# vpariza/open-hummingbird-eval

Hardware: AMD Instinct MI355X
Metric: query-patches/sec (higher is better)
Workload: dtype f32

## Files before the change

### include/hbird_hip.h

```cpp
#ifndef HBIRD_HIP_H
#define HBIRD_HIP_H
#include <stdint.h>
#ifdef __cplusplus
extern "C" {
#endif

typedef struct hb_index hb_index_t;

#define HB_METRIC_IP 0
#define HB_METRIC_L2 1
#define HB_MAX_K 2048
#define HB_MAX_K_AGGREGATE 256
#define HB_BIGK_MAX_PARTS 64

const char* hb_last_error(void);
int hb_device_count(int* n);

int hb_index_create(int d, int metric, int device, hb_index_t** out);
int hb_index_free(hb_index_t* ix);
int hb_index_set_stream(hb_index_t* ix, void* hip_stream);
int hb_index_reserve(hb_index_t* ix, int64_t n_rows);
int hb_index_add(hb_index_t* ix, const float* x, int64_t n, int x_on_device, int normalize);
int hb_index_add_labels(hb_index_t* ix, const float* labels, int64_t n, int c, int on_device);
int hb_index_set_label_denominator(hb_index_t* ix, int P);
// ... 36 lines not shown
int hb_bigk_aggregate(hb_index_t* ix, const float* q, int64_t nq, const int64_t* idx, const float* dist, int k,
                      int64_t id_base, float beta, float* out_label_hat, int io_on_device);
int hb_bigk_aggregate_partial(hb_index_t* ix, const float* q, int64_t nq, const int64_t* idx, const float* dist, int k,
                              int64_t id_base, float beta, const float* norms_all, int64_t n_all, float* out_partial);
int hb_bigk_merge_topk(const float* dist_parts, const int64_t* idx_parts, int parts, int64_t nq, int k, int metric,
                       int64_t* out_idx, float* out_dist, void* hip_stream);
int hb_bigk_merge_topk_packed(const void* packed_parts, int64_t part_bytes, int parts, int64_t nq, int k, int metric,
                              int64_t* out_idx, float* out_dist, void* hip_stream);

typedef struct hb_multi hb_multi_t;
int hb_multi_create(int d, int metric, const int* gpu_ids, int n_gpus, int shard, hb_multi_t** out);
int hb_multi_free(hb_multi_t* m);
int hb_multi_reserve(hb_multi_t* m, int64_t n_rows);
int hb_multi_add(hb_multi_t* m, const float* x, int64_t n, int normalize);
int64_t hb_multi_ntotal(const hb_multi_t* m);
int hb_multi_shard_rows(const hb_multi_t* m, int64_t* rows, int n);
int hb_multi_set_fp16(hb_multi_t* m, int enable);
int hb_multi_search(hb_multi_t* m, const float* q, int64_t nq, int k, int64_t* out_idx, float* out_dist);

int hb_normalize_rows(const float* x, int64_t n, int d, float* out, void* hip_stream);
int hb_patch_label_hist(const int64_t* y, int64_t B, int H, int W, int ps, int C, int map255, float* out,
                        void* hip_stream);
int hb_patch_scores(const float* label, int64_t B, int SS, int C, float* scores, int* nonempty, int* nz_count,
                    void* hip_stream);
int hb_patch_select(const float* scores, const int* nonempty, const float* r, const int64_t* r_off, int64_t B,
                    int SS, int K, int64_t* out_idx, float* out_scores, void* hip_stream);
int hb_gather_rows(const float* src, int64_t src_rows, int width, const int64_t* ids, int64_t n, float* out,
                   void* hip_stream);

int hb_upsample_argmax(const float* label_hat, int64_t B, int S, int C, int h, int w, int64_t* out,
                       void* hip_stream);
int hb_upsample_argmax_confusion(const float* label_hat, int64_t B, int S, int C, int h, int w, const int64_t* gt, int num_gt,
                                 int num_pred, int64_t ignore_index, int has_ignore, uint64_t* conf, int64_t* out_map_opt,
                                 void* hip_stream);
int hb_upsample_accumulate(const float* label_hat, int64_t B, int S, int C, int win_h, int win_w, float* acc, int H,
                           int W, int y0, int x0, void* hip_stream);
int hb_argmax_channels(const float* acc, int64_t n, int C, int64_t* out, void* hip_stream);
int hb_confusion_update(const int64_t* gt, const int64_t* pred, int64_t n, int num_gt, int num_pred,
                        int64_t ignore_index, int has_ignore, uint64_t* conf, void* hip_stream);

int hb_index_set_timing(hb_index_t* ix, int enable);
int hb_index_last_knn_ms(const hb_index_t* ix, double* ms);
int hb_index_set_tuning(hb_index_t* ix, int workgroups, int panel_tiles);
#define HB_FP16_AUTO 3
#define HB_PATH_FP32 0
#define HB_PATH_FP16_CHAIN 1
#define HB_PATH_FP16_WIDE 2
#define HB_WHY_EXPLICIT_FP32 0
#define HB_WHY_EXPLICIT_FP16 1
#define HB_WHY_AUTO 2
#define HB_WHY_K 3
#define HB_WHY_CEILING 4
#define HB_WHY_WORK 5
#define HB_WHY_SMALL 6
#define HB_WHY_PINNED 7
#define HB_WHY_ENV 8
#define HB_WHY_MEMORY 9
#define HB_WHY_OVERFLOW 10
#define HB_WHY_ADAPTIVE 11
int hb_index_set_fp16(hb_index_t* ix, int enable);
int hb_last_search_path(const hb_index_t* ix, int* path, int* reason);
int hb_exact_screen_replay(int setting, int pinned, int env_off, int k, int ceiling, int64_t rows, int64_t nq, int d, int64_t stages_per_wg,
                           int overflow, int have_copy, int declined, uint64_t free_bytes, uint64_t total_bytes, uint64_t bank_bytes,
                           uint64_t copy_bytes, int* why);
int hb_knn_plan_replay(const int64_t* in, int n_in, int64_t* out, int n_out);
int hb_index_last_fp16_fallbacks(const hb_index_t* ix, int64_t* n);
int hb_index_set_fp16_escalation(hb_index_t* ix, int mode);
int hb_index_last_fp16_escalated(const hb_index_t* ix, int64_t* n);
int hb_index_set_variant(hb_index_t* ix, int variant);
int hb_index_set_search_options(hb_index_t* ix, int phases, int64_t small_limit_stages);
int hb_index_set_xcd_weights(hb_index_t* ix, int mode, const double* w8);
int hb_index_xcd_weights(const hb_index_t* ix, int fp16_kernel, double* w8, int* rounds);
int hb_schedule_plan_weighted(int nqt, int nbt, int workgroups, int panel_tiles, int d, int cluster_q, int cluster_b, int shared,
                              const double* xcd_w8, int* segs_out, int64_t max_segs, int64_t stats[8]);
int hb_index_wg_stamps(hb_index_t* ix, uint32_t* out, int max_blocks, int* workgroups);
int hb_index_kernel_clock(hb_index_t* ix, double out[4]);
int hb_index_xcd_stats(const hb_index_t* ix, int fp16_kernel, double out[12]);
void* hb_calibration_new(int fp16_kernel);
void hb_calibration_free(void* h);
int hb_calibration_state(const void* h, double shares8[8], int64_t out[12]);
int hb_calibration_feed(void* h, const uint32_t* stamps, int G, const double run_shares8[8], const int key6[6], int auto_cluster, double frac);
int hb_f16_adapt_replay(int n, const double* f1, const double* f2, int64_t nq, int* out_how);
int hb_set_layout_form(int form);
int hb_index_set_rerank_copy(hb_index_t* ix, int mode);
int hb_index_rerank_copy_bytes(const hb_index_t* ix, int64_t* bytes);
int hb_index_schedule_info(const hb_index_t* ix, int64_t out[8]);
int hb_index_set_cluster(hb_index_t* ix, int cluster_q, int cluster_b, int sync_lag);
int hb_index_set_cluster_sharing(hb_index_t* ix, int mode);
int hb_index_cluster_stats(hb_index_t* ix, int64_t out[4]);

int hb_schedule_plan(int nqt, int nbt, int workgroups, int panel_tiles, int d, int cluster_q, int cluster_b, int* segs_out,
                     int64_t max_segs, int64_t stats[8]);
int hb_schedule_plan_phased(int nqt, int nbt, int workgroups, int panel_tiles, int d, int cluster_q, int cluster_b, int* segs_out,
                            int64_t max_segs, int64_t stats[8], int* clocks_out, int max_cuts, int* n_cuts, int* bounds_out);

int hb_schedule_plan_shared(int nqt, int nbt, int workgroups, int panel_tiles, int d, int cluster_q, int cluster_b, int phased,
                            int* segs_out, int64_t max_segs, int64_t stats[8]);

#include "hbird_hip_centre.h"
#include "hbird_hip_select.h"
#include "hbird_hip_grid.h"

#ifdef __cplusplus
}
#endif
#endif
```

### open-hummingbird-eval_amd/csrc/hbird_capi.hip

```cpp
#include "../../include/hbird_hip.h"
#include "hbird_internal.h"
#include <algorithm>
#include <cmath>
#include <cstdlib>
#include <cstring>
#include <dlfcn.h>
#include <mutex>
#include <set>
#include <utility>

static thread_local std::string g_err;
void hb_set_error(const std::string& msg) { g_err = msg; }
int hb_fail(const std::string& msg) { g_err = msg; return -1; }

namespace {
struct roctx_api {
    int (*push)(const char*) = nullptr;
    int (*pop)() = nullptr;
    roctx_api() {
        for (const char* lib : {"librocprofiler-sdk-roctx.so", "librocprofiler-sdk-roctx.so.1", "libroctx64.so", "libroctx64.so.4"}) {
            void* h = dlopen(lib, RTLD_LAZY | RTLD_GLOBAL);
            if (!h) continue;
            push = reinterpret_cast<int (*)(const char*)>(dlsym(h, "roctxRangePushA"));
            pop = reinterpret_cast<int (*)()>(dlsym(h, "roctxRangePop"));
// ... 116 lines not shown
    if (ix->f16_flag) HB_HIP(hipMemsetAsync(ix->f16_flag, 0, 4, ix->stream));
    hb_centre_drop(ix);
    ix->fp16_centre = on; ix->last_centred = 0;
    ix->f16_adapt = hb_f16_adapt();
    return 0;
}
extern "C" int hb_index_fp16_centre_info(const hb_index_t* ix, double out[8]) {
    if (!ix || !out) return hb_fail("hb_index_fp16_centre_info: NULL pointer");
    for (int i = 0; i < 8; ++i) out[i] = 0.0;
    const hb_centre_state& c = ix->centre;
    HB_HIP(hipSetDevice(ix->device));
    float sc[4] = {0, 0, 0, 0}, bmax = 0.0f;
    HB_HIP(hipStreamSynchronize(ix->stream));
    HB_HIP(hipMemcpy(&bmax, ix->bmax, 4, hipMemcpyDeviceToHost));
    const bool active = ix->fp16_centre && c.active && ix->tiles16 && c.sc;
    if (active) HB_HIP(hipMemcpy(sc, c.sc, 16, hipMemcpyDeviceToHost));
    out[0] = active ? 1.0 : 0.0; out[1] = sc[1]; out[2] = sc[0]; out[3] = bmax; out[4] = sc[3]; out[5] = active ? (double)c.rows : 0.0;
    out[6] = ix->fp16_centre; out[7] = ix->last_centred;
    return 0;
}
extern "C" int hb_last_search_path(const hb_index_t* ix, int* path, int* reason) {
    if (!ix || !path || !reason) return hb_fail("hb_last_search_path: NULL pointer");
    *path = ix->last_path; *reason = ix->last_reason;
    return 0;
}

extern "C" int hb_index_set_fp16_escalation(hb_index_t* ix, int mode) {
    if (!ix) return hb_fail("hb_index_set_fp16_escalation: NULL index handle");
    if (mode < 0 || mode > 1) return hb_fail("hb_index_set_fp16_escalation: mode must be 0 (second fp16 pass before the fp32 kernel) or 1 (straight to the fp32 kernel)");
    ix->fp16_escalation = mode;
    return 0;
}
extern "C" int hb_index_last_fp16_escalated(const hb_index_t* ix, int64_t* n) {
    if (!ix || !n) return hb_fail("hb_index_last_fp16_escalated: NULL pointer");
    *n = ix->last_fp16_escalated;
    return 0;
}
extern "C" int hb_index_last_fp16_fallbacks(const hb_index_t* ix, int64_t* n) {
    if (!ix || !n) return hb_fail("hb_index_last_fp16_fallbacks: NULL pointer");
    *n = ix->last_fp16_fallbacks;
    return 0;
}


extern "C" int hb_index_set_cluster_sharing(hb_index_t* ix, int mode) {
    if (!ix) return hb_fail("hb_index_set_cluster_sharing: NULL index handle");
    if (mode < 0 || mode > 2) return hb_fail("hb_index_set_cluster_sharing: mode must be 0 (automatic), 1 (off) or 2 (on)");
    ix->xcd_share = mode; ix->sched = hb_schedule(); ix->fp32_pinned = 1;
    return 0;
}

extern "C" int hb_index_cluster_stats(hb_index_t* ix, int64_t out[4]) {
    if (!ix || !out) return hb_fail("hb_index_cluster_stats: NULL pointer");
    out[0] = out[1] = out[2] = out[3] = 0;
    if (!ix->cl_stats_dev) return 0;
    HB_HIP(hipSetDevice(ix->device));
    int h[4] = {0, 0, 0, 0};
    HB_HIP(hipMemcpyAsync(h, ix->cl_stats_dev, sizeof(h), hipMemcpyDeviceToHost, ix->stream));
    HB_HIP(hipStreamSynchronize(ix->stream));
    out[0] = h[0]; out[1] = h[1]; out[2] = h[2]; out[3] = h[3];
    return 0;
}

extern "C" int hb_index_set_cluster(hb_index_t* ix, int cluster_q, int cluster_b, int sync_lag) {
    if (!ix) return hb_fail("hb_index_set_cluster: NULL index handle");
    if (cluster_q < 0 || cluster_b < 0 || cluster_q * cluster_b > HB_CLUSTER_MAX)
        return hb_fail("hb_index_set_cluster: cluster shape must be 0 x 0 (automatic), 1 x 1 (off) or q x b with q * b <= " + std::to_string(HB_CLUSTER_MAX));
    ix->force_cq = cluster_q; ix->force_cb = cluster_b; ix->sync_lag = sync_lag; ix->sched = hb_schedule();
    if (cluster_q != 0 || cluster_b != 0) ix->fp32_pinned = 1;
    return 0;
}

extern "C" int hb_index_set_variant(hb_index_t* ix, int variant) {
    if (!ix) return hb_fail("hb_index_set_variant: NULL index handle");
    if (variant < 0 || variant > 6) return hb_fail("hb_index_set_variant: unknown kernel variant");
    if (variant == 1 || variant == 2 || variant == 5)
        return hb_fail("hb_index_set_variant: variants 1 (4-wave fp32 kernel), 2 (first fp16 design) and 5 (16x16x32 fp16 kernel) were removed in round 4 (same bits, not faster)");
    ix->variant = variant; ix->fp32_pinned = 1;
    return 0;
}
extern "C" int hb_index_set_search_options(hb_index_t* ix, int phases, int64_t small_limit_stages) {
    if (!ix) return hb_fail("hb_index_set_search_options: NULL index handle");
    if (small_limit_stages < 0) return hb_fail("hb_index_set_search_options: negative limit");
    ix->phases_on = phases ? 1 : 0; ix->small_limit = small_limit_stages; ix->sched = hb_schedule(); ix->fp32_pinned = 1;
    return 0;
}
extern "C" int hb_index_set_xcd_weights(hb_index_t* ix, int mode, const double* w8) {
    if (!ix) return hb_fail("hb_index_set_xcd_weights: NULL index handle");
    if (mode < 0 || mode > 2) return hb_fail("hb_index_set_xcd_weights: mode must be 0 (calibrated), 1 (equal shares) or 2 (the given shares)");
    if (mode == 2 && !w8) return hb_fail("hb_index_set_xcd_weights: mode 2 needs eight shares");
    for (int x = 0; x < 8; ++x) {
        const double w = mode == 2 ? w8[x] : 1.0;
        if (!(w > 0.25 && w < 4.0)) return hb_fail("hb_index_set_xcd_weights: every share must lie in (0.25, 4)");
        ix->xcal[0].w[x] = w; ix->xcal[1].w[x] = w;
    }
    ix->xcd_balance = mode;
    if (mode != 0) ix->fp32_pinned = 1;
    for (auto& c : ix->xcal) { c.stamp_pending = 0; c.rounds = mode == 0 ? 0 : 1; c.locked = 0; c.cur_n = 0; c.best_span = 0.0; c.perm_moves = 0; }
    ix->sched = hb_schedule();
    return 0;
}
extern "C" int hb_index_xcd_weights(const hb_index_t* ix, int fp16_kernel, double* w8, int* rounds) {
    if (!ix || !w8) return hb_fail("hb_index_xcd_weights: NULL pointer");
    const hb_index::xcd_cal& c = ix->xcal[fp16_kernel ? 1 : 0];
    for (int x = 0; x < 8; ++x) w8[x] = c.w[x];
    if (rounds) *rounds = c.rounds;
    return 0;
}
extern "C" int hb_index_wg_stamps(hb_index_t* ix, uint32_t* out, int max_blocks, int* workgroups) {
    if (!ix || !out || !workgroups) return hb_fail("hb_index_wg_stamps: NULL pointer");
    *workgroups = 0;
    if (!ix->wg_stamp_dev) return 0;
    if (ix->wg_stamp_blocks > max_blocks) return hb_fail("hb_index_wg_stamps: the buffer is too small");
    HB_HIP(hipSetDevice(ix->device));
    std::vector<unsigned> h((size_t)ix->wg_stamp_blocks * 8);
    HB_HIP(hipMemcpyAsync(h.data(), ix->wg_stamp_dev, h.size() * 4, hipMemcpyDeviceToHost, ix->stream));
    HB_HIP(hipStreamSynchronize(ix->stream));
    for (int b = 0; b < ix->wg_stamp_blocks; ++b) { out[4 * b] = h[8 * b]; out[4 * b + 1] = h[8 * b + 4]; out[4 * b + 2] = h[8 * b + 1]; out[4 * b + 3] = 0; }
    *workgroups = ix->wg_stamp_blocks;
    return 0;
}
extern "C" int hb_index_kernel_clock(hb_index_t* ix, double out[4]) {
    if (!ix || !out) return hb_fail("hb_index_kernel_clock: NULL pointer");
    out[0] = out[1] = out[2] = out[3] = 0.0;
    if (!ix->wg_stamp_dev || ix->wg_stamp_blocks <= 0) return 0;
    HB_HIP(hipSetDevice(ix->device));
    const int G = ix->wg_stamp_blocks;
    std::vector<unsigned> h((size_t)G * 8);
    HB_HIP(hipMemcpyAsync(h.data(), ix->wg_stamp_dev, (size_t)G * 32, hipMemcpyDeviceToHost, ix->stream));
    HB_HIP(hipStreamSynchronize(ix->stream));
    std::vector<double> ghz;
    long long first = 0, last = 0;
    bool any = false;
    unsigned origin = 0;
    for (int b = 0; b < G; ++b) {
        const unsigned* sb = h.data() + 8 * (size_t)b;
        const unsigned t0 = sb[0], t1 = sb[4];
        if (t0 == 0u && t1 == 0u) continue;
        if (!any) origin = t0;
        const unsigned d = t1 - t0;
        const long long rs = (long long)(int)(t0 - origin), re = rs + (long long)d;
        if (!any) { first = rs; last = re; any = true; }
        first = std::min(first, rs); last = std::max(last, re);
        const unsigned long long c0 = ((unsigned long long)sb[3] << 32) | sb[2], c1 = ((unsigned long long)sb[7] << 32) | sb[6];
        if (c1 > c0 && d >= 100u && d < 0x7FFFFFFFu) ghz.push_back((double)(c1 - c0) / (double)d * 0.1);
    }
    if (ghz.empty()) return 0;
    std::sort(ghz.begin(), ghz.end());
    out[0] = ghz[ghz.size() / 2]; out[1] = ghz.front(); out[2] = ghz.back(); out[3] = (double)(last - first) * 1e-5;
    return 0;
}
extern "C" int hb_index_xcd_stats(const hb_index_t* ix, int fp16_kernel, double out[12]) {
    if (!ix || !out) return hb_fail("hb_index_xcd_stats: NULL pointer");
    const hb_index::xcd_cal& c = ix->xcal[fp16_kernel ? 1 : 0];
    out[0] = c.rounds; out[1] = c.locked; out[2] = c.reverts; out[3] = c.samples; out[4] = c.rejected;
    out[5] = c.best_span * 1e-5; out[6] = c.cur_span * 1e-5; out[7] = (double)ix->sched_builds;
    out[8] = c.perm_moves; out[9] = c.perm[0];
    out[10] = c.cl_state == 2 ? c.cl_choice : -1; out[11] = (c.cl_span_on - c.cl_span_off) * 1e-5;
    return 0;
}
extern "C" int hb_index_set_rerank_copy(hb_index_t* ix, int mode) {
    if (!ix) return hb_fail("hb_index_set_rerank_copy: NULL index handle");
    if (mode < 0 || mode > 2) return hb_fail("hb_index_set_rerank_copy: mode must be 0 (automatic), 1 (always) or 2 (never)");
    ix->rerank_copy = mode; ix->rows32_declined_cap = -1;
    if (mode == 2 && ix->rows32) {
        (void)hipSetDevice(ix->device);
        HB_HIP(hipStreamSynchronize(ix->stream));
        HB_HIP(hipFree(ix->rows32));
// ... 160 lines not shown
    }
    ix->c = c;
    const size_t esz = ix->label_P ? 2 : 4;
    const size_t ls = (size_t)ix->lab_stride();
    if (ix->nlabels + n > ix->lab_cap) {
        int64_t cap = std::max<int64_t>(ix->nlabels + n, std::max<int64_t>(ix->cap_rows, ix->lab_cap + ix->lab_cap / 2));
        char* nl = nullptr;
        char* old = ix->label_P ? (char*)ix->labels16 : (char*)ix->labels;
        HB_HIP(hipMalloc((void**)&nl, (size_t)cap * ls * esz));
        if (ix->nlabels > 0) HB_HIP(hipMemcpyAsync(nl, old, (size_t)ix->nlabels * ls * esz, hipMemcpyDeviceToDevice, ix->stream));
        HB_HIP(hipStreamSynchronize(ix->stream));
        if (old) HB_HIP(hipFree(old));
        if (ix->label_P) ix->labels16 = (uint16_t*)nl; else ix->labels = (float*)nl;
        ix->lab_cap = cap;
    }
    return 0;
}

extern "C" int hb_index_add_labels(hb_index_t* ix, const float* labels, int64_t n, int c, int on_device) {
    if (!ix) return hb_fail("hb_index_add_labels: NULL index handle");
    if (n < 0 || c <= 0) return hb_fail("hb_index_add_labels: bad shape");
    if (n == 0) return 0;
    HB_HIP(hipSetDevice(ix->device));
    if (ix->c != 0 && ix->c != c && ix->nlabels > 0) return hb_fail("hb_index_add_labels: class count changed");
    if (hb_labels_ensure(ix, c, n)) return -1;
    const size_t ls = (size_t)ix->lab_stride();
    if (ix->label_P) {
        if (!ix->lab_flag) { HB_HIP(hipMalloc((void**)&ix->lab_flag, 4)); HB_HIP(hipMemsetAsync(ix->lab_flag, 0, 4, ix->stream)); }
        const float* src = labels;
        if (!on_device) {
            if (grow((void**)&ix->tmp, &ix->tmp_bytes, (size_t)n * c * 4)) return -1;
            if (stage_in(ix, labels, (size_t)n * c * 4, 0)) return -1;
            src = (const float*)ix->tmp;
        }
        if (hb_launch_labels_to_counts(src, n, c, (int)ls, ix->label_P, ix->labels16 + ix->nlabels * (int64_t)ls, ix->lab_flag, ix->stream)) return -1;
        if (!on_device) HB_HIP(hipStreamSynchronize(ix->stream));
        ix->nlabels += n;
        return 0;
    }
    HB_HIP(hipMemcpyAsync(ix->labels + ix->nlabels * (int64_t)c, labels, (size_t)n * c * 4,
                          on_device ? hipMemcpyDeviceToDevice : hipMemcpyHostToDevice, ix->stream));
    if (!on_device) HB_HIP(hipStreamSynchronize(ix->stream));
    ix->nlabels += n;
    return 0;
}

static inline size_t al256(size_t x) { return (x + 255) / 256 * 256; }

static int search_impl(hb_index* ix, const float* q, int64_t nq, int k, int64_t id_base, float beta, float* out_lab,
                       int64_t* out_idx, float* out_dist, int io_on_device, bool aggregate, bool bigk = false, const hb_grid_spec* grid = nullptr) {
    if (nq < 0) return hb_fail("hb_index_search: negative query count");
    if (k < 1 || k > HB_MAX_K) return hb_fail("hb_index_search: k must be in [1, " + std::to_string(HB_MAX_K) + "] (faiss-gpu's own limit)");
    if (aggregate && !bigk && k > HB_MAX_K_AGGREGATE)
        return hb_fail("hb_index_search_aggregate: k must be in [1, " + std::to_string(HB_MAX_K_AGGREGATE) + "] (plain searches take k up to " + std::to_string(HB_MAX_K) + ")");
    if (nq == 0) return 0;
    if (!q) return hb_fail("hb_index_search: q is NULL");
    hb_range range(aggregate ? "hbird:search_aggregate" : "hbird:search");
    HB_HIP(hipSetDevice(ix->device));
    const int64_t nqp = (nq + HB_QT - 1) / HB_QT * HB_QT;
    if (grow((void**)&ix->q_tiles, &ix->q_tiles_bytes, (size_t)nqp * ix->dp * 4)) return -1;
    if (grow((void**)&ix->q_aux, &ix->q_aux_bytes, (size_t)nq * 2 * 4)) return -1;
    const size_t b_q = io_on_device ? 0 : al256((size_t)nq * ix->d * 4);
    const size_t b_idx = al256((size_t)nq * k * 8), b_dist = al256((size_t)nq * k * 4);
    const size_t lab_bytes = (size_t)nq * ix->c * 4 * (grid ? (size_t)grid->nk * grid->nb : 1);
    const size_t b_lab = (aggregate && !io_on_device) ? al256(lab_bytes) : 0;
    const bool t_idx = !io_on_device || !out_idx, t_dist = !io_on_device || !out_dist;
    const size_t need = b_q + (t_idx ? b_idx : 0) + (t_dist ? b_dist : 0) + b_lab;
    if (need && grow((void**)&ix->tmp, &ix->tmp_bytes, need)) return -1;
    char* cur = ix->tmp;
    const float* qd = q;
    if (!io_on_device) {
        HB_HIP(hipMemcpyAsync(cur, q, (size_t)nq * ix->d * 4, hipMemcpyHostToDevice, ix->stream));
        qd = (const float*)cur;
        cur += b_q;
    }
    int64_t* d_idx = out_idx;
    float* d_dist = out_dist;
    float* d_lab = out_lab;
    if (t_idx) { d_idx = (int64_t*)cur; cur += b_idx; }
    if (t_dist) { d_dist = (float*)cur; cur += b_dist; }
    if (b_lab) { d_lab = (float*)cur; cur += b_lab; }
    {
        hb_range r("hbird:query_tiles");
        if (hb_launch_rows_to_tiles(qd, nq, ix->d, ix->dp, 0, ix->q_tiles, nullptr, nullptr, ix->metric, 0, 0, ix->stream)) return -1;
        if (hb_launch_query_aux(qd, nq, ix->d, ix->q_aux, ix->q_aux + nq, ix->stream)) return -1;
    }
    {
        hb_range r("hbird:knn");
        if (hb_launch_knn(ix, qd, nq, k, id_base, d_idx, d_dist)) return -1;
    }
    if (aggregate) {
        hb_range r("hbird:aggregate");
        if (grid) {
            if (hb_launch_aggregate_grid(ix, ix->q_aux + nq, d_idx, d_dist, nq, k, id_base, *grid, d_lab, ix->stream)) return -1;
        } else if ((bigk ? hb_launch_aggregate_bigk : hb_launch_aggregate)(ix, ix->q_aux + nq, d_idx, d_dist, nq, k, id_base, beta, d_lab, ix->stream, nullptr, 0)) return -1;
    }
    if (!io_on_device) {
        if (out_idx) HB_HIP(hipMemcpyAsync(out_idx, d_idx, (size_t)nq * k * 8, hipMemcpyDeviceToHost, ix->stream));
        if (out_dist) HB_HIP(hipMemcpyAsync(out_dist, d_dist, (size_t)nq * k * 4, hipMemcpyDeviceToHost, ix->stream));
        if (aggregate) HB_HIP(hipMemcpyAsync(out_lab, d_lab, lab_bytes, hipMemcpyDeviceToHost, ix->stream));
        HB_HIP(hipStreamSynchronize(ix->stream));
    }
    return 0;
}

extern "C" int hb_index_search(hb_index_t* ix, const float* q, int64_t nq, int k, int64_t id_base, int64_t* out_idx,
                               float* out_dist, int io_on_device) {
    if (!ix) return hb_fail("hb_index_search: NULL index handle");
    if (nq > 0 && (!out_idx || !out_dist)) return hb_fail("hb_index_search: output pointers are NULL");
    return search_impl(ix, q, nq, k, id_base, 0.f, nullptr, out_idx, out_dist, io_on_device, false);
}

static bool labels_missing(const hb_index* ix) {
    return !ix->ext_labels && !ix->ext_labels16 && ((!ix->labels && !ix->labels16) || ix->nlabels < ix->ntotal);
}

template <typename Launch>
static int aggregate_on_lists(hb_index* ix, const char* range_name, const float* q, int64_t nq, float* zero_if_empty, Launch launch) {
    hb_range range(range_name);
    HB_HIP(hipSetDevice(ix->device));
    if (hb_labels_checked(ix)) return -1;
    if (zero_if_empty && ix->ntotal == 0) {
        HB_HIP(hipMemsetAsync(zero_if_empty, 0, (size_t)nq * ix->c * 4, ix->stream));
        return 0;
    }
    if (grow((void**)&ix->q_aux, &ix->q_aux_bytes, (size_t)nq * 2 * 4)) return -1;
    if (hb_launch_query_aux(q, nq, ix->d, ix->q_aux, ix->q_aux + nq, ix->stream)) return -1;
    return launch(ix->q_aux + nq);
}

extern "C" int hb_index_search_aggregate(hb_index_t* ix, const float* q, int64_t nq, int k, int64_t id_base, float beta,
                                         float* out_label_hat, int64_t* out_idx_opt, float* out_dist_opt,
                                         int io_on_device) {
    if (!ix) return hb_fail("hb_index_search_aggregate: NULL index handle");
    if (nq > 0 && !out_label_hat) return hb_fail("hb_index_search_aggregate: out_label_hat is NULL");
    if (!(beta > 0.f)) return hb_fail("hb_index_search_aggregate: beta must be positive");
    if (labels_missing(ix)) return hb_fail("hb_index_search_aggregate: label rows missing (hb_index_add_labels)");
    if (hb_labels_checked(ix)) return -1;
    return search_impl(ix, q, nq, k, id_base, beta, out_label_hat, out_idx_opt, out_dist_opt, io_on_device, true);
}

extern "C" int hb_index_aggregate(hb_index_t* ix, const float* q, int64_t nq, const int64_t* idx, const float* dist,
                                  int k, int64_t id_base, float beta, float* out_label_hat, int io_on_device) {
    if (!ix) return hb_fail("hb_index_aggregate: NULL index handle");
    if (nq < 0) return hb_fail("hb_index_aggregate: nq is negative");
    if (nq == 0) return 0;
    if (k < 1) return hb_fail("hb_index_aggregate: k must be positive");
    if (!io_on_device) return hb_fail("hb_index_aggregate: host pointers are not supported, pass device memory");
    if (!(beta > 0.f)) return hb_fail("hb_index_aggregate: beta must be positive");
    return aggregate_on_lists(ix, "hbird:aggregate", q, nq, nullptr, [&](const float* qnorm) {
        return hb_launch_aggregate(ix, qnorm, idx, dist, nq, k, id_base, beta, out_label_hat, ix->stream);
    });
}

extern "C" int hb_index_aggregate_grid(hb_index_t* ix, const float* q, int64_t nq, const int64_t* idx, const float* dist, int k_list,
                                       int64_t id_base, const int* ks, int nk, const float* betas, int nb, float* out, int io_on_device) {
    if (!ix) return hb_fail("hb_index_aggregate_grid: NULL index handle");
    if (nq < 0) return hb_fail("hb_index_aggregate_grid: nq is negative");
    hb_grid_spec gs;
    if (hb_grid_check("hb_index_aggregate_grid", ks, nk, betas, nb, k_list, &gs)) return -1;
    if (labels_missing(ix)) return hb_fail("hb_index_aggregate_grid: label rows missing (hb_index_add_labels)");
    if (nq == 0) return 0;
    if (!q || !idx || !dist || !out) return hb_fail("hb_index_aggregate_grid: NULL pointer");
    if (!io_on_device) return hb_fail("hb_index_aggregate_grid: host pointers are not supported, pass device memory");
    return aggregate_on_lists(ix, "hbird:aggregate_grid", q, nq, nullptr, [&](const float* qnorm) {
        return hb_launch_aggregate_grid(ix, qnorm, idx, dist, nq, k_list, id_base, gs, out, ix->stream);
    });
// ... 284 lines not shown
```

### open-hummingbird-eval_amd/csrc/hbird_internal.h

```cpp
#pragma once
#include <hip/hip_runtime.h>
#include <stdint.h>
#include <array>
#include <string>
#include <vector>
#include "hbird_schedule.h"
#include "hbird_calibrate.h"
#include "hbird_f16_centre.h"

#define HB_RT 32
#define HB_THREADS 512
#define HB_WAVES 8
#define HB_BLK 256

#define HB_STAGE_BYTES (16384 + 16384 + 1024)
#define HB_LDS_LISTS (2 * HB_STAGE_BYTES)
#define HB_LDS_SCRATCH (HB_LDS_LISTS + 2 * HB_QT * HB_KL * 4)
#define HB_LDS_TOTAL (HB_LDS_SCRATCH + HB_WAVES * 8 * 64 * 4)

#define HB_ID_NONE 0xFFFFFFFFu

struct hb_range {
    explicit hb_range(const char* name);
    ~hb_range();
// ... 12 lines not shown
    uint16_t* labels16 = nullptr;
    int label_P = 0;
    int* lab_flag = nullptr;
    int64_t lab_checked = 0;
    int c = 0;
    int64_t nlabels = 0, lab_cap = 0;
    int lab_stride() const { return label_P ? (c + 7) & ~7 : c; }
    int num_cu = 256;
    const float* ext_labels = nullptr; const float* ext_bnorm = nullptr; int64_t ext_n = 0, ext_base = 0;
    const uint16_t* ext_labels16 = nullptr; int ext_P = 0;
    float* q_tiles = nullptr; size_t q_tiles_bytes = 0;
    float* q_aux = nullptr; size_t q_aux_bytes = 0;
    char* state = nullptr; size_t state_bytes = 0;
    char* sched_dev = nullptr; size_t sched_bytes = 0;
    char* tmp = nullptr; size_t tmp_bytes = 0;
    hb_schedule sched;
    int force_G = 0, force_panel = 0;
    int force_cq = 0, force_cb = 0;
    int sync_lag = -1;
    int xcd_share = 0;
    struct xcd_cal : hb_xcd_state {
        unsigned* stamp_host = nullptr;
        hipEvent_t stamp_ev = nullptr;
        int stamp_pending = 0;
        double stamp_w[8] = {1, 1, 1, 1, 1, 1, 1, 1};
        double stamp_frac = 1.0;
        std::array<int, 6> stamp_key{{0, 0, 0, 0, 0, 0}};
        int stamp_auto_cluster = 0;
    } xcal[2];
    int64_t sched_builds = 0;
    int xcd_balance = 0;
    const int* cl_stats_dev = nullptr;
    int fp16 = HB_FP16_AUTO, dp16 = 0;
    int fp32_pinned = 0;
    int screen_env_off = 0;
    int64_t f16_declined_cap = -1;
    int last_path = 0, last_reason = 0;
    unsigned* stamp_keep = nullptr; int stamp_keep_blocks = 0;
    void* tiles16 = nullptr; int64_t f16_cap_rows = 0, f16_rows = 0;
    int* f16_flag = nullptr; int f16_overflow = 0;
    float* rows32 = nullptr; int64_t rows32_cap_rows = 0, rows32_rows = 0; int rows32_rs = 0;
    int rerank_copy = 0;
    int64_t rows32_declined_cap = -1;
    int fp16_centre = 0;
    int last_centred = 0;
    hb_centre_state centre;
    void* q16 = nullptr; size_t q16_bytes = 0;
    char* cand = nullptr; size_t cand_bytes = 0;
    float* bmax = nullptr;
    char* mtmp = nullptr; size_t mtmp_bytes = 0;
    char* fb = nullptr; size_t fb_bytes = 0;
    char* fb1 = nullptr; size_t fb1_bytes = 0;
    int64_t last_fp16_fallbacks = 0;
    int64_t last_fp16_escalated = 0;
    int fp16_escalation = 0;
    hb_f16_adapt f16_adapt;
    char* bigk = nullptr; size_t bigk_bytes = 0;
    hb_schedule sched_esc; char* sched_esc_dev = nullptr; size_t sched_esc_bytes = 0;
    int score_output = 0;
    int variant = 0;
    int phases_on = 1;
    const unsigned* wg_stamp_dev = nullptr; int wg_stamp_blocks = 0;
    long long small_limit = 0;
    double last_knn_ms = 0.0;
    hipEvent_t ev0 = nullptr, ev1 = nullptr;
    int time_kernels = 0;
};

void hb_set_error(const std::string& msg);
int hb_fail(const std::string& msg);
#define HB_HIP(call)                                                                         \
    do {                                                                                     \
        hipError_t _e = (call);                                                              \
        if (_e != hipSuccess)                                                                \
            return hb_fail(std::string(#call) + ": " + hipGetErrorString(_e));               \
    } while (0)

int hb_ensure_dyn_lds(const void* kernel, int bytes);

int hb_launch_rows_to_tiles(const float* src, int64_t n_rows, int d, int dp, int64_t row0, float* tiles,
                            float* binit, float* bnorm, int metric, int normalize, int is_bank, hipStream_t s);
int hb_launch_scores_to_l2(const float* qn2, int64_t nq, int k, float* dist_inout, hipStream_t s);
int hb_launch_query_aux(const float* q, int64_t nq, int d, float* qn2, float* qnorm, hipStream_t s);
int hb_launch_tiles_to_rows(const float* tiles, int g8, int d, const int64_t* ids, int64_t n, int64_t id_base, int64_t ntotal,
                            float* out, hipStream_t s);
int hb_launch_knn(hb_index* ix, const float* q_dev, int64_t nq, int k, int64_t id_base, int64_t* out_idx, float* out_dist);
int hb_launch_tiles_to_f16(const float* t32, int g8, _Float16* t16, int g16, int64_t n_row_tiles, int64_t rt0, int* overflow,
                           hipStream_t s);
int hb_launch_tiles_to_rows(const float* t32, int g8, float* rows, int rs, int64_t n_row_tiles, int64_t rt0, hipStream_t s);
int hb_launch_rerank_rows(const float* rows, int rs, const float* binit, int d, const float* q, const float* qn2,
                          const int64_t* cand, const float* cand_score, const float* qnorm, const float* bmax,
                          unsigned char* certified, int kc, int64_t nq, int k, int64_t id_base, int metric, int out_metric,
                          int64_t ntotal, int64_t* out_idx, float* out_dist, hipStream_t s, const float* seed_in = nullptr, float* kth_out = nullptr,
                          float* floor_out = nullptr, const hb_centre_view* cv = nullptr);
int hb_launch_rerank(const float* tiles, const float* binit, int g8, int d, const float* q, const float* qn2,
                     const int64_t* cand, const float* cand_score, const float* qnorm, const float* bmax,
                     unsigned char* certified, int kc, int64_t nq, int k, int64_t id_base, int metric, int out_metric, int64_t ntotal, int64_t* out_idx,
                     float* out_dist, hipStream_t s, const float* seed_in = nullptr, float* kth_out = nullptr, float* floor_out = nullptr,
                     const hb_centre_view* cv = nullptr);
int hb_launch_bnorm_max(const float* bnorm, int64_t n, float* bmax, hipStream_t s);
int hb_launch_scatter_rows(const int64_t* rows, int64_t n, int k, const int64_t* src_idx, const float* src_dist,
                           int64_t* out_idx, float* out_dist, hipStream_t s);
struct knn16_args;
int hb_knn_f16_launch(const knn16_args& args, int grid, hipStream_t s);
int hb_launch_labels_to_counts(const float* src, int64_t rows, int c, int dst_stride, int P, uint16_t* dst, int* flag, hipStream_t s);
int hb_launch_gather_label_counts(const uint16_t* src, int64_t src_rows, int c, int src_stride, int P, const int64_t* ids, int64_t n, float* out, hipStream_t s);
int hb_labels_ensure(hb_index* ix, int c, int64_t n);
int hb_labels_checked(hb_index* ix);
struct hb_k5_table {
    const void* labels; bool u16; int P, ls; int64_t nlabels;
    const float* bnorm; int64_t norm_base, nnorm;
    int64_t id_base;
    int wide;
};
int hb_k5_table_choose(const hb_index* ix, int64_t id_base, const float* norms_all, int64_t n_all, const char* who, hb_k5_table* t);
int hb_launch_aggregate(const hb_index* ix, const float* qnorm, const int64_t* idx, const float* dist, int64_t nq,
                        int k, int64_t id_base, float beta, float* out, hipStream_t s, const float* norms_all = nullptr, int64_t n_all = 0);
int hb_launch_merge_parts(const float* dist_parts, const int64_t* idx_parts, int parts, int64_t nq, int k, int metric,
                          int64_t dist_stride, int64_t idx_stride, int64_t* out_idx, float* out_dist, hipStream_t s);
int hb_launch_aggregate_bigk(const hb_index* ix, const float* qnorm, const int64_t* idx, const float* dist, int64_t nq,
                             int k, int64_t id_base, float beta, float* out, hipStream_t s, const float* norms_all = nullptr, int64_t n_all = 0);
int hb_launch_merge_sorted_parts(const float* dist_parts, const int64_t* idx_parts, int parts, int64_t nq, int k, int metric,
                                 int64_t dist_stride, int64_t idx_stride, int64_t* out_idx, float* out_dist, hipStream_t s);
struct hb_grid_spec { int ks[16]; float betas[16]; int nk, nb; };
int hb_grid_check(const char* who, const int* ks, int nk, const float* betas, int nb, int k_list, hb_grid_spec* gs);
int hb_launch_aggregate_grid(const hb_index* ix, const float* qnorm, const int64_t* idx, const float* dist, int64_t nq, int k_list,
                             int64_t id_base, const hb_grid_spec& gs, float* out, hipStream_t s);
int hb_launch_patch_label_hist(const int64_t* y, int64_t B, int H, int W, int ps, int C, int map255, float* out,
                               hipStream_t s);
int hb_launch_normalize_rows(const float* x, int64_t n, int d, float* out, hipStream_t s);
int hb_launch_gather_rows(const float* src, int64_t src_rows, int width, const int64_t* ids, int64_t n, float* out,
                          hipStream_t s);
int hb_launch_upsample_argmax(const float* label_hat, int64_t B, int S, int C, int h, int w, int64_t* out,
                              hipStream_t s);
int hb_launch_upsample_argmax_confusion(const float* label_hat, int64_t B, int S, int C, int h, int w, int64_t* out, const int64_t* gt,
                                        int num_gt, int num_pred, int64_t ignore, int has_ignore, unsigned long long* conf, hipStream_t s);
int hb_launch_upsample_accumulate(const float* label_hat, int64_t B, int S, int C, int win_h, int win_w, float* acc, int H,
                                  int W, int y0, int x0, hipStream_t s);
int hb_launch_argmax_channels(const float* acc, int64_t n, int C, int64_t* out, hipStream_t s);
int hb_launch_confusion(const int64_t* gt, const int64_t* pred, int64_t n, int num_gt, int num_pred, int64_t ignore,
                        int has_ignore, unsigned long long* conf, hipStream_t s);
```

### open-hummingbird-eval_amd/csrc/hbird_knn.hip

```cpp
#include "hbird_internal.h"
#include "../../include/hbird_hip.h"
#include <algorithm>
#include <array>
#include <mutex>
#include <cstring>
#include <map>

#include "hbird_knn_dev.h"

#define KN_MFMA(T, FR, B, S) acc[T] = __builtin_amdgcn_mfma_f32_32x32x2f32(FR[(T) & 3][S], B[S], acc[T], 0, 0, 0);

template <bool COLD, bool WIDE, bool CL = false, bool CEIL = false>
__global__ __launch_bounds__(HB_THREADS, 2) void knn_fused_kernel(knn_args a) {
    extern __shared__ __attribute__((aligned(16))) char smem[];
    const int tid = threadIdx.x;
    const int lane = tid & 63;
    const int w = __builtin_amdgcn_readfirstlane(tid >> 6);
    const int h = lane >> 5;
    float* lst_s = reinterpret_cast<float*>(smem + KN_LISTS);
    unsigned* lst_i = reinterpret_cast<unsigned*>(smem + KN_LISTS + HB_QT * HB_KL * 4);
    float* sc = reinterpret_cast<float*>(smem + KN_SCRATCH) + w * 256;
    unsigned* qf = reinterpret_cast<unsigned*>(smem + KN_QF) + w * 512;
    int* pcnt = reinterpret_cast<int*>(smem + KN_LISTS);
    const int g8 = a.g8, k = a.k;
// ... 294 lines not shown
    if ((size_t)ng * k * 8 > lim) return hb_fail("hb_index_search: too many partial lists per query tile for the merge kernel");
    const size_t half = (size_t)nqt * ng * HB_QT * klw * 4;
    if (ensure_bytes(&ix->mtmp, &ix->mtmp_bytes, 2 * half)) return -1;
    float* ts = reinterpret_cast<float*>(ix->mtmp);
    unsigned* ti = reinterpret_cast<unsigned*>(ix->mtmp + half);
    knn_merge_kernel<<<dim3((unsigned)nq, (unsigned)ng), dim3(64), (size_t)grp * per * 8, s>>>(state_s, state_i, cnts, pthr, per, qt_off, qt_slots,
                                                                                                0, grp, ng, ts, ti, nq, k, klw, 0, 0,
                                                                                                nullptr, nullptr, nullptr);
    HB_HIP(hipGetLastError());
    knn_merge_kernel<<<dim3((unsigned)nq), dim3(64), (size_t)ng * k * 8, s>>>(ts, ti, nullptr, nullptr, k, nullptr, nullptr, ng, 0, 0, nullptr,
                                                                                nullptr, nq, k, klw, id_base, metric, qn2, out_idx,
                                                                                out_dist);
    HB_HIP(hipGetLastError());
    return 0;
}

__global__ __launch_bounds__(64) void merge_parts_kernel(const float* __restrict__ dist_parts,
                                                         const int64_t* __restrict__ idx_parts, int parts, int64_t nq,
                                                         int k, int metric, int64_t dist_stride, int64_t idx_stride,
                                                         int64_t* __restrict__ out_idx, float* __restrict__ out_dist) {
    extern __shared__ __attribute__((aligned(16))) char smem[];
    const int64_t q = blockIdx.x;
    const int n = parts * k;
    float* cs = reinterpret_cast<float*>(smem);
    int64_t* ci = reinterpret_cast<int64_t*>(smem + ((n * 4 + 15) / 16) * 16);
    const int lane = threadIdx.x;
    for (int c = lane; c < n; c += 64) {
        const size_t off = (size_t)q * k + (c % k);
        float d = dist_parts[(size_t)(c / k) * dist_stride + off];
        cs[c] = metric == 1 ? -d : d;
        ci[c] = idx_parts[(size_t)(c / k) * idx_stride + off];
    }
    __syncthreads();
    for (int c = lane; c < n; c += 64) {
        const float s = cs[c];
        const int64_t id = ci[c];
        int rank = 0;
        for (int j = 0; j < n; ++j) {
            const float sj = cs[j];
            const int64_t ij = ci[j];
            bool better;
            if (ij < 0 || id < 0) better = (ij >= 0 && id < 0) || (ij < 0 && id < 0 && j < c);
            else better = (sj > s) || (sj == s && (ij < id || (ij == id && j < c)));
            rank += better;
        }
        if (rank < k) {
            const int64_t o = q * (int64_t)k + rank;
            out_idx[o] = id < 0 ? -1 : id;
            out_dist[o] = id < 0 ? (metric == 1 ? INFINITY : -INFINITY) : (metric == 1 ? -s : s);
        }
    }
}

int hb_launch_merge_parts(const float* dist_parts, const int64_t* idx_parts, int parts, int64_t nq, int k, int metric,
                          int64_t dist_stride, int64_t idx_stride, int64_t* out_idx, float* out_dist, hipStream_t s) {
    if (nq == 0) return 0;
    const size_t n = (size_t)parts * k;
    const size_t sh = ((n * 4 + 15) / 16) * 16 + n * 8;
    if (sh > 60000) return hb_fail("hb_merge_topk: parts*k too large for the merge kernel");
    merge_parts_kernel<<<dim3((unsigned)nq), dim3(64), sh, s>>>(dist_parts, idx_parts, parts, nq, k, metric, dist_stride, idx_stride,
                                                                 out_idx, out_dist);
    HB_HIP(hipGetLastError());
    return 0;
}


__global__ __launch_bounds__(256) void seed_floors_kernel(const int64_t* __restrict__ idx, const float* __restrict__ score, int64_t nq, int kk,
                                                         unsigned* __restrict__ gthr) {
    const int64_t q = (int64_t)blockIdx.x * 256 + threadIdx.x;
    if (q >= nq) return;
    if (idx[q * kk + kk - 1] >= 0) atomicMax(gthr + q, pool_key(score[q * kk + kk - 1]));
}

__global__ __launch_bounds__(256) void seed_from_scores_kernel(const float* __restrict__ seed, int64_t nq, unsigned* __restrict__ gthr) {
    const int64_t q = (int64_t)blockIdx.x * 256 + threadIdx.x;
    if (q >= nq) return;
    const float v = seed[q];
    if (v > -INFINITY && v < INFINITY) atomicMax(gthr + q, pool_key(v));
}

__global__ __launch_bounds__(256) void pool_floor_kernel(const float* __restrict__ state_s, const int* __restrict__ cnts,
                                                        const float* __restrict__ pthr, const int* __restrict__ qt_off,
                                                        const int* __restrict__ qt_slots, int64_t nq, int kk, int klw, int per_wave,
                                                        unsigned* __restrict__ gthr) {
    extern __shared__ __attribute__((aligned(16))) char smem[];
    const int lane = threadIdx.x & 63, w = threadIdx.x >> 6;
    const int64_t q = (int64_t)blockIdx.x * 4 + w;
    if (q >= nq) return;
    pool_floor_query(state_s, cnts, pthr, qt_off, qt_slots, q, kk, klw, reinterpret_cast<float*>(smem) + (size_t)w * per_wave, gthr, lane);
}

static std::mutex g_xcd_mu;
static std::map<std::pair<int, int>, std::array<double, 8>> g_xcd_known;
static std::map<int, int> g_cl_known;
static void hb_xcd_calibrate(hb_index* ix, int fam) {
    hb_index::xcd_cal& c = ix->xcal[fam];
    if (c.rounds == 0 && !c.stamp_pending) {
        std::lock_guard<std::mutex> lock(g_xcd_mu);
        auto it = g_xcd_known.find({ix->device, fam});
        if (it != g_xcd_known.end()) {
            bool differs = false;
            for (int x = 0; x < 8; ++x) { differs = differs || c.w[x] != it->second[x]; c.w[x] = it->second[x]; }
            if (differs) ix->sched = hb_schedule();
            c.rounds = 1;
        }
        auto cl = g_cl_known.find(ix->device);
        if (fam == 0 && cl != g_cl_known.end() && c.cl_state != 2) { c.cl_state = 2; c.cl_choice = cl->second; ix->sched = hb_schedule(); }
    }
    if (!c.stamp_pending || !c.stamp_ev || !c.stamp_host || hipEventQuery(c.stamp_ev) != hipSuccess) { (void)hipGetLastError(); return; }
    const int G = c.stamp_pending;
    c.stamp_pending = 0;
    hb_stamp_set set;
    set.stamps = c.stamp_host; set.G = G; set.key = c.stamp_key; set.frac = c.stamp_frac; set.auto_cluster = c.stamp_auto_cluster;
    for (int x = 0; x < 8; ++x) set.run_shares[x] = c.stamp_w[x];
    const int flags = hb_xcd_step(c, fam, set);
    if (flags & HB_CAL_REBUILD) ix->sched = hb_schedule();
    if (flags & (HB_CAL_REMEMBER_SHARES | HB_CAL_REMEMBER_CLUSTERS)) {
        std::lock_guard<std::mutex> lock(g_xcd_mu);
        if (flags & HB_CAL_REMEMBER_SHARES) {
            std::array<double, 8> keep;
            for (int x = 0; x < 8; ++x) keep[x] = c.w[x];
            g_xcd_known[{ix->device, fam}] = keep;
        }
        if (flags & HB_CAL_REMEMBER_CLUSTERS) g_cl_known[ix->device] = c.cl_choice;
    }
}
static int hb_xcd_collect(hb_index* ix, int fam, const unsigned* stamps_dev, const hb_schedule& sc, const double* shares, int n_phases, int nqt, int nbt,
                          int k, hipStream_t s, bool auto_cluster = false) {
    hb_index::xcd_cal& c = ix->xcal[fam];
    if (!stamps_dev || sc.G > 1024 || c.stamp_pending) return 0;
    if (!c.stamp_ev) HB_HIP(hipEventCreateWithFlags(&c.stamp_ev, hipEventDisableTiming));
    if (!c.stamp_host) HB_HIP(hipHostMalloc((void**)&c.stamp_host, 1024 * 32, hipHostMallocDefault));
    HB_HIP(hipMemcpyAsync(c.stamp_host, stamps_dev, (size_t)sc.G * 32, hipMemcpyDeviceToHost, s));
    HB_HIP(hipEventRecord(c.stamp_ev, s));
    c.stamp_pending = sc.G;
    for (int x = 0; x < 8; ++x) c.stamp_w[x] = shares[x];
    c.stamp_key = {nqt, nbt, sc.G, n_phases, k, sc.cq * 16 + sc.cb};
    c.stamp_auto_cluster = auto_cluster ? 1 : 0;
    const double per_wg = (double)nqt * (double)nbt / std::max(1, sc.G);
    c.stamp_frac = n_phases > 1 && !sc.cuts_scaled && per_wg > 0.0 ? std::min(1.0, std::max(0.25, 1.0 - (double)sc.phase_clock.back() / per_wg)) : 1.0;
    return 0;
}

__global__ __launch_bounds__(256) void bigk_place_kernel(const int64_t* __restrict__ tmp_idx, const float* __restrict__ tmp_sc, int64_t nq, int kp, int k,
                                                         int col0, int64_t id_base, int out_metric, const float* __restrict__ qn2,
                                                         int64_t* __restrict__ out_idx, float* __restrict__ out_dist, float* __restrict__ ceil_s,
                                                         unsigned* __restrict__ ceil_i) {
    const int64_t t = (int64_t)blockIdx.x * 256 + threadIdx.x;
    if (t >= nq * kp) return;
    const int64_t q = t / kp;
    const int j = (int)(t % kp);
    const int64_t id = tmp_idx[t];
    const float s = tmp_sc[t];
    const int64_t o = q * (int64_t)k + col0 + j;
    if (id < 0) { out_idx[o] = -1; out_dist[o] = out_metric == 1 ? INFINITY : -INFINITY; }
    else {
        out_idx[o] = id + id_base;
        if (out_metric == 1) { const float d2 = fmaf(-2.0f, s, qn2[q]); out_dist[o] = d2 > 0.0f ? d2 : 0.0f; }
        else out_dist[o] = s;
    }
    if (j == kp - 1) {
        ceil_s[q] = id < 0 ? -INFINITY : s;
        ceil_i[q] = id < 0 ? 0xFFFFFFFFu : (unsigned)id;
    }
}

static inline size_t al256(size_t x) { return (x + 255) / 256 * 256; }

struct knn_call {
    int esc = 0;
    const float* seed = nullptr;
    const float* ceil_s = nullptr;
    const unsigned* ceil_i = nullptr;
    int fp16 = 0;
    bool timed = false;
    const float* q_aux = nullptr;
    bool score_out = false;
};
static int knn_search(hb_index* ix, const knn_call& c, const float* q_dev, int64_t nq, int k, int64_t id_base, int64_t* out_idx, float* out_dist);

static int hb_launch_knn_bigk(hb_index* ix, const knn_call& c, const float* q_dev, int64_t nq, int k, int64_t id_base, int64_t* out_idx, float* out_dist) {
    if (nq == 0) return 0;
    hipStream_t s = ix->stream;
    const int64_t nqp = (nq + HB_QT - 1) / HB_QT * HB_QT;
    const size_t o_sc = al256((size_t)nq * 256 * 8), o_cs = o_sc + al256((size_t)nq * 256 * 4), o_ci = o_cs + al256((size_t)nqp * 4), tot = o_ci + al256((size_t)nqp * 4);
    if (ensure_bytes(&ix->bigk, &ix->bigk_bytes, tot)) return -1;
    int64_t* tmp_idx = reinterpret_cast<int64_t*>(ix->bigk);
    float* tmp_sc = reinterpret_cast<float*>(ix->bigk + o_sc);
    float* ceil_s = reinterpret_cast<float*>(ix->bigk + o_cs);
    unsigned* ceil_i = reinterpret_cast<unsigned*>(ix->bigk + o_ci);
    HB_HIP(hipMemsetD32Async((hipDeviceptr_t)ceil_s, 0xFF800000u, (size_t)nqp, s));
    HB_HIP(hipMemsetD32Async((hipDeviceptr_t)ceil_i, 0xFFFFFFFFu, (size_t)nqp, s));
    const int out_metric = c.score_out ? 0 : ix->metric;
    double knn_ms = 0.0;
    int rc = 0;
    for (int col0 = 0; col0 < k && !rc; col0 += 256) {
        const int kp = std::min(256, k - col0);
        knn_call pass = c;
        pass.score_out = true;
        pass.ceil_s = col0 ? ceil_s : nullptr; pass.ceil_i = col0 ? ceil_i : nullptr;
        rc = knn_search(ix, pass, q_dev, nq, kp, 0, tmp_idx, tmp_sc);
        if (rc) break;
        if (c.timed) knn_ms += ix->last_knn_ms;
        bigk_place_kernel<<<dim3((unsigned)((nq * kp + 255) / 256)), dim3(256), 0, s>>>(tmp_idx, tmp_sc, nq, kp, k, col0, id_base, out_metric, c.q_aux,
                                                                                         out_idx, out_dist, ceil_s, ceil_i);
        HB_HIP(hipGetLastError());
    }
    if (c.timed) ix->last_knn_ms = knn_ms;
    return rc;
}

static int knn_drop_tiles16(hb_index* ix) {
    if (ix->tiles16) HB_HIP(hipFree(ix->tiles16));
    ix->tiles16 = nullptr; ix->f16_rows = 0; ix->f16_cap_rows = 0;
    return 0;
}

struct knn_path {
    bool f16 = false;
    int why = HB_WHY_EXPLICIT_FP32;
    bool automatic = false, wide_first = false;
    int how16 = HB_F16_CHAIN;
    bool centred = false;
};
static int knn_choose_path(hb_index* ix, const knn_call& c, int64_t nq, int k, knn_path* out) {
    knn_path& p = *out;
    const bool ceil = c.ceil_s != nullptr;
    const int esc = c.esc;
    hb_screen_in sin;
    sin.setting = c.fp16; sin.pinned = ix->fp32_pinned != 0; sin.env_off = ix->screen_env_off != 0; sin.k = k; sin.ceiling = ceil;
    sin.rows = ix->ntotal; sin.nq = nq; sin.d = ix->d; sin.overflow = ix->f16_overflow != 0;
    sin.stages_per_wg = hb_stages_per_wg((nq + HB_QT - 1) / HB_QT, (ix->ntotal + HB_BT - 1) / HB_BT, hb_knn_workgroups(ix->force_G, ix->num_cu), ix->g8);
    sin.have_copy = ix->tiles16 != nullptr && ix->f16_cap_rows == ix->cap_rows;
    sin.declined = ix->f16_declined_cap == ix->cap_rows;
    sin.bank_b = (uint64_t)ix->cap_rows * ix->dp * 4; sin.copy_b = (uint64_t)ix->cap_rows * ix->dp16 * 2;
    p.automatic = c.fp16 == HB_FP16_AUTO;
    p.f16 = hb_screen_choose(sin, &p.why);
    if (p.f16 && p.automatic && !sin.have_copy && nq > 0 && ix->ntotal > 0) {
        if (knn_drop_tiles16(ix)) return -1;
        size_t free_b = 0, total_b = 0;
        HB_HIP(hipMemGetInfo(&free_b, &total_b));
        sin.mem_known = true; sin.free_b = free_b; sin.total_b = total_b;
        p.f16 = hb_screen_choose(sin, &p.why);
        if (!p.f16) ix->f16_declined_cap = ix->cap_rows;
    }
    bool skipped = false;
    if (p.f16 && esc == 0 && (c.fp16 == 2 || p.automatic) && ix->fp16_escalation == 0) {
        p.how16 = hb_f16_choose(ix->f16_adapt);
        if (p.how16 == HB_F16_FP32) { p.f16 = false; skipped = true; p.why = HB_WHY_ADAPTIVE; }
        else if (p.how16 == HB_F16_WIDE_FIRST) p.wide_first = true;
    }
    if (!p.f16 && esc == 0) { ix->last_fp16_fallbacks = skipped ? nq : 0; ix->last_fp16_escalated = 0; }
    return 0;
}

static int knn_screen_upkeep(hb_index* ix, bool automatic, int esc, int64_t nq, hipStream_t s0, bool& f16, int& why) {
    if (!ix->f16_flag) { HB_HIP(hipMalloc((void**)&ix->f16_flag, 4)); HB_HIP(hipMemsetAsync(ix->f16_flag, 0, 4, s0)); }
    if (ix->f16_cap_rows != ix->cap_rows) {
        if (knn_drop_tiles16(ix)) return -1;
        if (!automatic) HB_HIP(hipMalloc(&ix->tiles16, (size_t)ix->cap_rows * ix->dp16 * 2));
        else if (hipMalloc(&ix->tiles16, (size_t)ix->cap_rows * ix->dp16 * 2) != hipSuccess) {
            (void)hipGetLastError();
            ix->tiles16 = nullptr; ix->f16_declined_cap = ix->cap_rows;
            f16 = false; why = HB_WHY_MEMORY;
            if (esc == 0) { ix->last_fp16_fallbacks = 0; ix->last_fp16_escalated = 0; }
        }
        if (ix->tiles16) {
            HB_HIP(hipMemsetAsync(ix->tiles16, 0, (size_t)ix->cap_rows * ix->dp16 * 2, s0));
            ix->f16_cap_rows = ix->cap_rows;
        }
    }
    if (f16 && ix->f16_rows < ix->ntotal) {
        const int64_t rt0 = ix->f16_rows / 32, need_rt = (ix->ntotal + 31) / 32;
        int centred = 0;
        if (ix->fp16_centre && hb_centre_convert(ix, s0, &centred)) return -1;
        if (!centred && hb_launch_tiles_to_f16(ix->tiles, ix->g8, (_Float16*)ix->tiles16, ix->dp16 / 16, need_rt - rt0, rt0, ix->f16_flag, s0)) return -1;
        ix->f16_rows = ix->ntotal;
        HB_HIP(hipMemcpyAsync(&ix->f16_overflow, ix->f16_flag, 4, hipMemcpyDeviceToHost, s0));
        HB_HIP(hipStreamSynchronize(s0));
    }
    if (f16 && ix->f16_overflow) {
        f16 = false; why = HB_WHY_OVERFLOW;
        if (esc == 0) { ix->last_fp16_fallbacks = nq; ix->last_fp16_escalated = 0; }
        if (automatic && knn_drop_tiles16(ix)) return -1;
    }
    if (f16 && ix->rerank_copy != 2) {
        const int rs = (ix->g8 * 8 + 31) / 32 * 32;
        if (ix->rows32 && (ix->rows32_cap_rows != ix->cap_rows || ix->rows32_rs != rs)) {
            HB_HIP(hipFree(ix->rows32));
            ix->rows32 = nullptr; ix->rows32_cap_rows = 0; ix->rows32_rows = 0;
        }
        if (!ix->rows32 && (ix->rerank_copy == 1 || ix->rows32_declined_cap != ix->cap_rows)) {
            const size_t need = (size_t)ix->cap_rows * rs * 4;
            size_t free_b = 0, total_b = 0;
            HB_HIP(hipMemGetInfo(&free_b, &total_b));
            ix->rows32_declined_cap = ix->cap_rows;
            const size_t bank_b = (size_t)ix->cap_rows * ix->dp * 4;
            if (ix->rerank_copy == 1 || (bank_b <= (size_t)16e9 && bank_b + bank_b / 2 + need <= total_b / 100 * 55 &&
                                         free_b > need + std::max<size_t>(total_b / 16, (size_t)2 << 30))) {
                if (hipMalloc((void**)&ix->rows32, need) == hipSuccess) { ix->rows32_cap_rows = ix->cap_rows; ix->rows32_rs = rs; ix->rows32_rows = 0; ix->rows32_declined_cap = -1; }
                else { (void)hipGetLastError(); ix->rows32 = nullptr; if (ix->rerank_copy == 1) return hb_fail("hb_index_search: no memory for the re-rank copy of the bank"); }
            }
        }
        if (ix->rows32 && ix->rows32_rows < ix->ntotal) {
            const int64_t rt0 = ix->rows32_rows / 32, need_rt = (ix->ntotal + 31) / 32;
            if (hb_launch_tiles_to_rows(ix->tiles, ix->g8, ix->rows32, rs, need_rt - rt0, rt0, s0)) return -1;
            ix->rows32_rows = ix->ntotal;
        }
    }
    return 0;
}

struct knn_work_list {
    const hb_schedule* sc = nullptr;
    double shares[8] = {1, 1, 1, 1, 1, 1, 1, 1};
    const hb_seg* segs = nullptr;
    const int *wg_off = nullptr, *qt_off = nullptr, *qt_slots = nullptr, *wg_member = nullptr, *phase_bounds = nullptr;
    int n_phases = 1;
    const int* phase_begin(int p) const { return p == 0 ? wg_off : phase_bounds + (size_t)(p - 1) * sc->G; }
    const int* phase_end(int p) const { return p == n_phases - 1 ? wg_off + 1 : phase_bounds + (size_t)p * sc->G; }
};
static int knn_get_work_list(hb_index* ix, int esc, const hb_knn_plan& p, hipStream_t s, knn_work_list* out) {
    knn_work_list& wl = *out;
    static const double equal_shares[8] = {1, 1, 1, 1, 1, 1, 1, 1};
    if (p.balance) {
        double shares_n[8];
        double mean = 0.0;
        bool uneven = false;
        const hb_index::xcd_cal& xc = ix->xcal[p.fam];
        for (int x = 0; x < 8; ++x) mean += xc.w[x] / 8.0;
        for (int g = 0; g < 8; ++g) { shares_n[g] = xc.w[ix->xcd_balance == 0 ? xc.perm[g] : g] / mean; uneven = uneven || std::fabs(shares_n[g] - 1.0) > 1e-9; }
        if (uneven) std::copy(shares_n, shares_n + 8, wl.shares);
    }
    const double* shares = wl.shares;
    hb_schedule& sc = esc == 0 ? ix->sched : ix->sched_esc;
    char*& sched_dev = esc == 0 ? ix->sched_dev : ix->sched_esc_dev;
    size_t& sched_bytes = esc == 0 ? ix->sched_bytes : ix->sched_esc_bytes;
    const int nqt = p.nqt, nbt = p.nbt, G = p.G;
    const bool rebuilt = !(sc.nqt == nqt && sc.nbt == nbt && sc.panel == p.panel && sc.cq == p.cq && sc.cb == p.cb && sc.phased == p.phased &&
                           sc.xcd_share == p.xs && (sc.G == G || (long long)nqt * nbt < G) &&
                           (sc.xcd_w.empty() ? std::equal(shares, shares + 8, equal_shares) : std::equal(shares, shares + 8, sc.xcd_w.begin())));
    if (rebuilt) { hb_build_schedule(nqt, nbt, G, p.panel, sc, p.cq, p.cb, p.phased, p.xs, shares); ++ix->sched_builds; }
    const struct { const void* data; size_t bytes; } part[6] = {{sc.segs.data(), sc.segs.size() * sizeof(hb_seg)}, {sc.wg_off.data(), sc.wg_off.size() * 4},
        {sc.qt_off.data(), sc.qt_off.size() * 4}, {sc.qt_slots.data(), sc.qt_slots.size() * 4}, {sc.wg_member.data(), sc.wg_member.size() * 4},
        {sc.phase_bounds.data(), sc.phase_bounds.size() * 4}};
    size_t off[7] = {0};
    for (int i = 0; i < 6; ++i) off[i + 1] = off[i] + al256(part[i].bytes);
    const bool need_upload = rebuilt || sched_bytes < off[6];
    if (ensure_bytes(&sched_dev, &sched_bytes, off[6])) return -1;
    if (need_upload) {
        for (int i = 0; i < 6; ++i) HB_HIP(hipMemcpyAsync(sched_dev + off[i], part[i].data, part[i].bytes, hipMemcpyHostToDevice, s));
        HB_HIP(hipStreamSynchronize(s));
    }
    auto ints = [&](int i) { return reinterpret_cast<const int*>(sched_dev + off[i]); };
    wl.sc = &sc; wl.segs = reinterpret_cast<const hb_seg*>(sched_dev);
    wl.wg_off = ints(1); wl.qt_off = ints(2); wl.qt_slots = ints(3); wl.wg_member = ints(4); wl.phase_bounds = ints(5);
    wl.n_phases = (int)sc.phase_clock.size() + 1;
    return 0;
}

struct knn_workspace {
    knn_args a;
    size_t state_aux = 0;
    size_t prog_bytes = 0, stamp_bytes = 0;
};
static int knn_carve_workspace(hb_index* ix, const knn_call& c, const hb_knn_plan& p, const knn_work_list& wl, int64_t nq, int k, hipStream_t s,
                               knn_workspace* out) {
    const hb_schedule& sc = *wl.sc;
    const int nqt = p.nqt, klw = p.klw, esc = c.esc;
    const size_t state_half = (size_t)sc.n_slots * HB_QT * klw * 4;
    const size_t state_aux = p.wide ? (size_t)sc.n_slots * HB_QT * 4 : 0;
    const size_t floor_bytes = (size_t)nqt * HB_QT * 4 * 17;
    const size_t prog_bytes = ((size_t)std::max(1, sc.n_clusters) * HB_CLUSTER_MAX + 1) * HB_CLUSTER_LINE * 4;
    const size_t stamp_bytes = (size_t)sc.G * 32;
    if (ensure_bytes(&ix->state, &ix->state_bytes, 2 * state_half + 2 * state_aux + floor_bytes + prog_bytes + stamp_bytes)) return -1;
    out->state_aux = state_aux; out->prog_bytes = prog_bytes; out->stamp_bytes = stamp_bytes;
    char* const floors = ix->state + 2 * state_half + 2 * state_aux;
    knn_args& a = out->a;
    a.wg_stamp = esc == 0 && (c.timed || p.calibrated) ? reinterpret_cast<unsigned*>(floors + floor_bytes + prog_bytes) : nullptr;
    if (esc == 0) { ix->wg_stamp_dev = a.wg_stamp; ix->wg_stamp_blocks = sc.G; }
    if (a.wg_stamp) HB_HIP(hipMemsetAsync(a.wg_stamp, 0, stamp_bytes, s));
    a.bank_tiles = ix->tiles; a.binit = ix->binit; a.q_tiles = ix->q_tiles;
    a.ceil_s = c.ceil_s; a.ceil_i = c.ceil_i; a.segs = wl.segs; a.wg_off = wl.wg_off; a.wg_end = a.wg_off + 1;
    a.state_s = reinterpret_cast<float*>(ix->state);
    a.state_i = reinterpret_cast<unsigned*>(ix->state + state_half);
    a.g8 = ix->g8; a.k = k; a.klw = klw;
    a.state_cnt = reinterpret_cast<int*>(ix->state + 2 * state_half);
    a.state_thr = reinterpret_cast<float*>(ix->state + 2 * state_half + state_aux);
    a.gthr = reinterpret_cast<unsigned*>(floors);
    a.qfl = a.gthr + (size_t)nqt * HB_QT;
    HB_HIP(hipMemsetD32Async((hipDeviceptr_t)a.gthr, 0x007FFFFF, (size_t)nqt * HB_QT * 17, s));
    if (nq < (int64_t)nqt * HB_QT) HB_HIP(hipMemsetD32Async((hipDeviceptr_t)(a.gthr + nq), 0xFF800000u, (size_t)((int64_t)nqt * HB_QT - nq), s));
    if (esc != 0 && c.seed) {
        seed_from_scores_kernel<<<dim3((unsigned)((nq + 255) / 256)), dim3(256), 0, s>>>(c.seed, nq, a.gthr);
        HB_HIP(hipGetLastError());
    }
    a.wg_member = wl.wg_member; a.prog = reinterpret_cast<int*>(floors + floor_bytes);
    a.cl = sc.cq * sc.cb; a.lag = p.lag;
    a.cl_stats = a.prog + (size_t)std::max(1, sc.n_clusters) * HB_CLUSTER_MAX * HB_CLUSTER_LINE;
    ix->cl_stats_dev = a.cl > 1 ? a.cl_stats : nullptr;
    if (a.cl > 1) HB_HIP(hipMemsetAsync(a.prog, 0, prog_bytes, s));
    return 0;
}

static int knn_seed_floors(hb_index* ix, const knn_args& a, const knn_work_list& wl, int nqt, int klw, int64_t nq, int kk, int64_t* scratch_idx,
                           float* scratch_dist, hipStream_t s) {
    const hb_schedule& sc = *wl.sc;
    const size_t per_wave = (size_t)sc.max_slots_per_qt * klw;
    if (per_wave * 16 <= 144 * 1024) {
        if (per_wave * 16 > 48 * 1024 && hb_ensure_dyn_lds((const void*)pool_floor_kernel, 144 * 1024)) return -1;
        pool_floor_kernel<<<dim3((unsigned)((nq + 3) / 4)), dim3(256), per_wave * 16, s>>>(a.state_s, a.state_cnt, a.state_thr, wl.qt_off, wl.qt_slots, nq, kk,
                                                                                           klw, (int)per_wave, a.gthr);
        HB_HIP(hipGetLastError());
        return 0;
    }
    if (launch_merge(ix, a.state_s, a.state_i, a.state_cnt, a.state_thr, wl.qt_off, wl.qt_slots, sc.max_slots_per_qt, nqt, nq, kk, klw, 0, 0, nullptr,
                     scratch_idx, scratch_dist, s)) return -1;
    seed_floors_kernel<<<dim3((unsigned)((nq + 255) / 256)), dim3(256), 0, s>>>(scratch_idx, scratch_dist, nq, kk, a.gthr);
    HB_HIP(hipGetLastError());
    return 0;
}

template <class Launch>
static int knn_run_phases(hb_index* ix, const knn_call& c, const hb_knn_plan& p, const knn_work_list& wl, const knn_workspace& ws, int64_t nq, int kk,
                          int64_t* scratch_idx, float* scratch_dist, hipStream_t s, Launch launch) {
    const knn_args& a = ws.a;
    if (c.timed) HB_HIP(hipEventRecord(ix->ev0, s));
    if (wl.n_phases > 1) {
        HB_HIP(hipMemsetAsync(a.state_cnt, 0, ws.state_aux, s));
        HB_HIP(hipMemsetD32Async((hipDeviceptr_t)a.state_thr, 0xFF800000u, ws.state_aux / 4, s));
    }
    for (int ph = 0; ph < wl.n_phases; ++ph) {
        if (launch(wl.phase_begin(ph), wl.phase_end(ph))) return -1;
        if (ph + 1 < wl.n_phases) {
            if (knn_seed_floors(ix, a, wl, p.nqt, p.klw, nq, kk, scratch_idx, scratch_dist, s)) return -1;
            if (a.cl > 1) HB_HIP(hipMemsetAsync(a.prog, 0, ws.prog_bytes - HB_CLUSTER_LINE * 4, s));
        }
    }
    if (c.timed) HB_HIP(hipEventRecord(ix->ev1, s));
    if (p.calibrated && c.esc == 0 && hb_xcd_collect(ix, p.fam, a.wg_stamp, *wl.sc, wl.shares, wl.n_phases, p.nqt, p.nbt, kk, s, p.auto_cluster)) return -1;
    return 0;
}
static int knn_read_time(hb_index* ix, const knn_call& c) {
    if (!c.timed) return 0;
    HB_HIP(hipEventSynchronize(ix->ev1));
    float ms = 0.f;
    HB_HIP(hipEventElapsedTime(&ms, ix->ev0, ix->ev1));
    ix->last_knn_ms = ms;
    return 0;
}

struct knn_level_buf {
    char*& buf; size_t& bytes;
    size_t o_kth, o_flo, o_rows;
    knn_level_buf(hb_index* ix, int esc, int64_t nq) : buf(esc == 0 ? ix->fb : ix->fb1), bytes(esc == 0 ? ix->fb_bytes : ix->fb1_bytes), o_kth(al256((size_t)nq + 64)),
                                                       o_flo(o_kth + al256((size_t)nq * 4)), o_rows(o_flo + al256((size_t)nq * 4)) {}
    float* kth() const { return reinterpret_cast<float*>(buf + o_kth); }
    float* flo() const { return reinterpret_cast<float*>(buf + o_flo); }
};

static int knn_research_failures(hb_index* ix, const knn_call& c, const knn_path& path, const hb_knn_plan& p, const knn_work_list& wl, const knn_workspace& ws,
                                 const std::vector<int64_t>& bad, const float* q_dev, int64_t nq, int k, int64_t id_base, int64_t* out_idx, float* out_dist,
                                 hipStream_t s) {
    const int esc = c.esc;
    const int64_t nf = (int64_t)bad.size();
    const knn_level_buf lv(ix, esc, nq);
    char*& fbuf = lv.buf;
    size_t& fbuf_bytes = lv.bytes;
    const size_t o_rows = lv.o_rows;
    const bool again16 = esc == 0 && ix->fp16_escalation == 0 && p.kc < 256 && ix->ntotal >= 4096;
    const size_t o_q = o_rows + al256((size_t)nf * 8), o_aux = o_q + al256((size_t)nf * ix->d * 4), o_seed = o_aux + al256((size_t)nf * 8),
                 o_idx = o_seed + al256((size_t)nf * 4), o_dist = o_idx + al256((size_t)nf * k * 8), tot2 = o_dist + al256((size_t)nf * k * 4);
    if (fbuf_bytes < tot2) {
        char* nb = nullptr;
        HB_HIP(hipMalloc((void**)&nb, tot2 + tot2 / 4));
        HB_HIP(hipMemcpyAsync(nb, fbuf, o_rows, hipMemcpyDeviceToDevice, s));
        HB_HIP(hipStreamSynchronize(s));
        HB_HIP(hipFree(fbuf));
        fbuf = nb; fbuf_bytes = tot2 + tot2 / 4;
    }
    const float *kth = lv.kth(), *flo = lv.flo();
    int64_t* d_rows = reinterpret_cast<int64_t*>(fbuf + o_rows);
    float* d_q = reinterpret_cast<float*>(fbuf + o_q);
    float* d_aux = reinterpret_cast<float*>(fbuf + o_aux);
    float* d_seed = reinterpret_cast<float*>(fbuf + o_seed);
    int64_t* d_fi = reinterpret_cast<int64_t*>(fbuf + o_idx);
    float* d_fd = reinterpret_cast<float*>(fbuf + o_dist);
    HB_HIP(hipMemcpyAsync(d_rows, bad.data(), (size_t)nf * 8, hipMemcpyHostToDevice, s));
    if (hb_launch_gather_rows(q_dev, nq, ix->d, d_rows, nf, d_q, s)) return -1;
    if (hb_launch_gather_rows(again16 ? flo : kth, nq, 1, d_rows, nf, d_seed, s)) return -1;
    if (hb_launch_rows_to_tiles(d_q, nf, ix->d, ix->dp, 0, ix->q_tiles, nullptr, nullptr, ix->metric, 0, 0, s)) return -1;
    if (esc == 0 && ws.a.wg_stamp) {
        const hb_schedule& sc = *wl.sc;
        const size_t stamp_bytes = ws.stamp_bytes;
        if (ix->stamp_keep_blocks < sc.G) {
            if (ix->stamp_keep) HB_HIP(hipFree(ix->stamp_keep));
            ix->stamp_keep = nullptr; ix->stamp_keep_blocks = 0;
            HB_HIP(hipMalloc((void**)&ix->stamp_keep, stamp_bytes));
            ix->stamp_keep_blocks = sc.G;
        }
        HB_HIP(hipMemcpyAsync(ix->stamp_keep, ws.a.wg_stamp, ws.stamp_bytes, hipMemcpyDeviceToDevice, s));
        ix->wg_stamp_dev = ix->stamp_keep;
    }
    int rc = hb_launch_query_aux(d_q, nf, ix->d, d_aux, d_aux + nf, s);
    knn_call nested;
    nested.esc = again16 ? 1 : 2; nested.seed = d_seed;
    nested.fp16 = again16 ? 1 : 0; nested.timed = false; nested.q_aux = d_aux; nested.score_out = c.score_out;
    if (!again16) ix->last_fp16_fallbacks = nf;
    if (!rc) rc = knn_search(ix, nested, d_q, nf, k, id_base, d_fi, d_fd);
    if (esc == 0) { ix->last_fp16_escalated = nf; hb_f16_observe(ix->f16_adapt, path.how16, nq, nf, ix->last_fp16_fallbacks); }
    if (rc) return -1;
    if (hb_launch_scatter_rows(d_rows, nf, k, d_fi, d_fd, out_idx, out_dist, s)) return -1;
    HB_HIP(hipStreamSynchronize(s));
    return 0;
}

static int knn_search_f16(hb_index* ix, const knn_call& c, const knn_path& path, const hb_knn_plan& p, const knn_work_list& wl, const knn_workspace& ws,
                          const float* q_dev, int64_t nq, int k, int64_t id_base, int out_metric, int64_t* out_idx, float* out_dist,
                          hipStream_t s) {
    const knn_args& a = ws.a;
    const hb_schedule& sc = *wl.sc;
    const int esc = c.esc, kc = p.kc, klw = p.klw, nqt = p.nqt;
    const bool centred = path.centred;
    const int64_t nqp = (int64_t)nqt * HB_QT;
    if (ensure_bytes((char**)&ix->q16, &ix->q16_bytes, (size_t)nqp * ix->dp16 * 2)) return -1;
    hb_centre_view cview{nullptr, nullptr, nullptr};
    if (centred) { if (hb_centre_queries(ix, nq, esc == 0, (_Float16*)ix->q16, &cview, s)) return -1; }
    else if (hb_launch_tiles_to_f16(ix->q_tiles, ix->g8, (_Float16*)ix->q16, ix->dp16 / 16, nqp / 32, 0, nullptr, s)) return -1;
    const hb_centre_view* cv = centred ? &cview : nullptr;
    if (ensure_bytes(&ix->cand, &ix->cand_bytes, (size_t)nq * kc * 12)) return -1;
    int64_t* cand_idx = reinterpret_cast<int64_t*>(ix->cand);
    float* cand_dist = reinterpret_cast<float*>(ix->cand + (size_t)nq * kc * 8);
    knn16_args h;
    h.wg_stamp = a.wg_stamp;
    h.bank16 = reinterpret_cast<const _Float16*>(ix->tiles16); h.binit = centred ? ix->centre.init16 : ix->binit; h.q16 = reinterpret_cast<const _Float16*>(ix->q16); h.segs = a.segs; h.wg_off = a.wg_off; h.wg_end = a.wg_end;
    h.state_s = a.state_s; h.state_i = a.state_i; h.g16 = ix->dp16 / 16; h.k = kc; h.klw = klw;
    h.state_cnt = a.state_cnt; h.state_thr = a.state_thr; h.gthr = a.gthr;
    h.wg_member = a.wg_member; h.prog = a.prog; h.cl = a.cl; h.lag = a.lag; h.cl_stats = a.cl_stats;
    if (knn_run_phases(ix, c, p, wl, ws, nq, kc, cand_idx, cand_dist, s, [&](const int* begin, const int* end) {
            h.wg_off = begin; h.wg_end = end;
            return hb_knn_f16_launch(h, sc.G, s);
        })) return -1;
    if (launch_merge(ix, a.state_s, a.state_i, a.state_cnt, a.state_thr, wl.qt_off, wl.qt_slots, sc.max_slots_per_qt, nqt, nq, kc, klw, 0, 0, nullptr,
                     cand_idx, cand_dist, s)) return -1;
    const knn_level_buf lv(ix, esc, nq);
    if (ensure_bytes(&lv.buf, &lv.bytes, lv.o_rows)) return -1;
    unsigned char* cert = reinterpret_cast<unsigned char*>(lv.buf);
    float *kth = lv.kth(), *flo = lv.flo();
    HB_HIP(hipMemsetD32Async((hipDeviceptr_t)kth, 0xFF800000u, (lv.o_rows - lv.o_kth) / 4, s));
    const float* seed_in = esc == 1 ? c.seed : nullptr;
    const float* q_aux = c.q_aux;
    if (ix->rows32 && ix->rerank_copy != 2 && ix->rows32_rows >= ix->ntotal) {
        if (hb_launch_rerank_rows(ix->rows32, ix->rows32_rs, ix->binit, ix->d, q_dev, q_aux, cand_idx, cand_dist, q_aux + nq, ix->bmax,
                                  cert, kc, nq, k, id_base, ix->metric, out_metric, ix->ntotal, out_idx, out_dist, s, seed_in, kth, flo, cv)) return -1;
    } else if (hb_launch_rerank(ix->tiles, ix->binit, ix->g8, ix->d, q_dev, q_aux, cand_idx, cand_dist, q_aux + nq, ix->bmax,
                                cert, kc, nq, k, id_base, ix->metric, out_metric, ix->ntotal, out_idx, out_dist, s, seed_in, kth, flo, cv)) return -1;
    if (knn_read_time(ix, c)) return -1;
    std::vector<unsigned char> hc((size_t)nq);
    HB_HIP(hipMemcpyAsync(hc.data(), cert, (size_t)nq, hipMemcpyDeviceToHost, s));
    HB_HIP(hipStreamSynchronize(s));
    std::vector<int64_t> bad;
    for (int64_t i = 0; i < nq; ++i) if (!hc[i]) bad.push_back(i);
    const int64_t nf = (int64_t)bad.size();
    if (esc == 0) { ix->last_fp16_escalated = 0; ix->last_fp16_fallbacks = 0; }
    if (esc == 0 && nf == 0) hb_f16_observe(ix->f16_adapt, path.how16, nq, 0, 0);
    if (nf > 0 && knn_research_failures(ix, c, path, p, wl, ws, bad, q_dev, nq, k, id_base, out_idx, out_dist, s)) return -1;
    return 0;
}

static int knn_search_f32(hb_index* ix, const knn_call& c, const hb_knn_plan& p, const knn_work_list& wl, const knn_workspace& ws, int64_t nq, int k,
                          int64_t id_base, int out_metric, int64_t* out_idx, float* out_dist, hipStream_t s) {
    const hb_schedule& sc = *wl.sc;
    typedef void (*knn_fn)(knn_args);
    knn_fn fn = nullptr;
    int lds_bytes = KN_LDS_TOTAL;
    switch (p.kernel) {
        case HB_KERNEL_LISTS: fn = knn_fused_kernel<false, false>; break;
        case HB_KERNEL_LISTS_COLD: fn = knn_fused_kernel<true, false>; lds_bytes = KN_LDS_TOTAL_COLD; break;
        case HB_KERNEL_POOLS: fn = knn_fused_kernel<false, true>; break;
        case HB_KERNEL_LISTS_CL: fn = knn_fused_kernel<false, false, true>; break;
        case HB_KERNEL_POOLS_CL: fn = knn_fused_kernel<false, true, true>; break;
        case HB_KERNEL_CEIL: fn = knn_fused_kernel<false, true, false, true>; break;
        default:
            fn = hb_knn_bd_kernel(p.wide, ws.a.cl > 1, p.small);
            lds_bytes = hb_knn_bd_lds_bytes(p.small && !p.wide);
    }
    if (hb_ensure_dyn_lds((const void*)fn, lds_bytes)) return -1;
    knn_args a = ws.a;
    if (knn_run_phases(ix, c, p, wl, ws, nq, k, out_idx, out_dist, s, [&](const int* begin, const int* end) {
            a.wg_off = begin; a.wg_end = end;
            fn<<<dim3((unsigned)sc.G), dim3(HB_THREADS), lds_bytes, s>>>(a);
            HB_HIP(hipGetLastError());
            return 0;
        })) return -1;
    const float* qn2 = c.q_aux;
    const int* pool_cnt = p.wide ? a.state_cnt : nullptr;
    if (launch_merge(ix, a.state_s, a.state_i, pool_cnt, pool_cnt ? a.state_thr : nullptr, wl.qt_off, wl.qt_slots, sc.max_slots_per_qt, p.nqt, nq, k, p.klw,
                     id_base, out_metric, qn2, out_idx, out_dist, s)) return -1;
    return knn_read_time(ix, c);
}

static int knn_search(hb_index* ix, const knn_call& c, const float* q_dev, int64_t nq, int k, int64_t id_base, int64_t* out_idx, float* out_dist) {
    if (k < 1 || k > HB_MAX_K) return hb_fail("hb_index_search: k must be in [1, " + std::to_string(HB_MAX_K) + "] (faiss-gpu's limit, search_faiss.py:84-85)");
    if (k > 256) return hb_launch_knn_bigk(ix, c, q_dev, nq, k, id_base, out_idx, out_dist);
    hipStream_t s = ix->stream;
    const int esc = c.esc;
    knn_path path;
    if (knn_choose_path(ix, c, nq, k, &path)) return -1;
    if (path.f16 && nq > 0 && ix->ntotal > 0 && knn_screen_upkeep(ix, path.automatic, esc, nq, s, path.f16, path.why)) return -1;
    path.centred = path.f16 && ix->fp16_centre && ix->centre.active;
    if (esc == 0) { ix->last_path = !path.f16 ? HB_PATH_FP32 : path.wide_first ? HB_PATH_FP16_WIDE : HB_PATH_FP16_CHAIN; ix->last_reason = path.why; ix->last_centred = path.centred ? 1 : 0; }
    if (nq == 0) return 0;
    const int out_metric = c.score_out ? 0 : ix->metric;
    if (ix->ntotal == 0) {
        std::vector<int64_t> hi((size_t)nq * k, -1);
        std::vector<float> hd((size_t)nq * k, out_metric == 1 ? INFINITY : -INFINITY);
        HB_HIP(hipMemcpyAsync(out_idx, hi.data(), hi.size() * 8, hipMemcpyHostToDevice, s));
        HB_HIP(hipMemcpyAsync(out_dist, hd.data(), hd.size() * 4, hipMemcpyHostToDevice, s));
        HB_HIP(hipStreamSynchronize(s));
        return 0;
    }
    hb_knn_plan_in pin;
    pin.f16 = path.f16; pin.wide_first = path.wide_first; pin.esc = esc; pin.ceil = c.ceil_s != nullptr;
    pin.k = k; pin.nq = nq; pin.ntotal = ix->ntotal; pin.g8 = ix->g8; pin.dp = ix->dp; pin.dp16 = ix->dp16; pin.num_cu = ix->num_cu;
    pin.force_G = ix->force_G; pin.force_panel = ix->force_panel; pin.force_cq = ix->force_cq; pin.force_cb = ix->force_cb; pin.variant = ix->variant;
    pin.small_limit = ix->small_limit; pin.phases_on = ix->phases_on; pin.xcd_balance = ix->xcd_balance; pin.xcd_share = ix->xcd_share; pin.sync_lag = ix->sync_lag;
    hb_knn_plan p;
    hb_knn_plan_shape(pin, p);
    if (p.calibrated && esc == 0) hb_xcd_calibrate(ix, p.fam);
    pin.cl_state = ix->xcal[0].cl_state; pin.cl_choice = ix->xcal[0].cl_choice;
    hb_knn_plan_clusters(pin, p);
    knn_work_list wl;
    if (knn_get_work_list(ix, esc, p, s, &wl)) return -1;
    hb_knn_plan_kernel(pin, wl.sc->G, p);
    knn_workspace ws;
    if (knn_carve_workspace(ix, c, p, wl, nq, k, s, &ws)) return -1;
    if (path.f16) return knn_search_f16(ix, c, path, p, wl, ws, q_dev, nq, k, id_base, out_metric, out_idx, out_dist, s);
    return knn_search_f32(ix, c, p, wl, ws, nq, k, id_base, out_metric, out_idx, out_dist, s);
}

int hb_launch_knn(hb_index* ix, const float* q_dev, int64_t nq, int k, int64_t id_base, int64_t* out_idx, float* out_dist) {
    knn_call c;
    c.fp16 = ix->fp16; c.timed = ix->time_kernels != 0; c.q_aux = ix->q_aux; c.score_out = ix->score_output != 0;
    return knn_search(ix, c, q_dev, nq, k, id_base, out_idx, out_dist);
}
```

### open-hummingbird-eval_amd/csrc/hbird_knn_f16.hip

```cpp
#include "hbird_knn_dev.h"
#include <algorithm>

typedef _Float16 f16x8 __attribute__((ext_vector_type(8)));


__global__ __launch_bounds__(256) void tiles_to_f16_kernel(const float* __restrict__ t32, int g8, _Float16* __restrict__ t16,
                                                           int g16, int64_t n_row_tiles, int64_t rt0, int* __restrict__ overflow) {
    const int64_t gid = (int64_t)blockIdx.x * 256 + threadIdx.x;
    const int64_t total = n_row_tiles * g16 * 64;
    if (gid >= total) return;
    const int i = (int)(gid & 31), h = (int)((gid >> 5) & 1);
    const int64_t blk = gid >> 6;
    const int g = (int)(blk % g16);
    const int64_t rt = rt0 + blk / g16;
    f16x8 out;
#pragma unroll
    for (int j = 0; j < 8; ++j) {
        const int k = 16 * g + 8 * h + j;
        const int gg = k >> 3, kk = k & 7;
        float v = 0.0f;
        if (gg < g8) v = t32[((rt * g8) + gg) * HB_BLK + ((kk & 1) * 32 + i) * 4 + (kk >> 1)];
        out[j] = (_Float16)v;
        if (overflow && fabsf(v) > 65504.0f && fabsf(v) < INFINITY) *overflow = 1;
    }
// ... 95 lines not shown
            _Pragma("unroll") for (int t = 0; t < 8; ++t)                                                                    \
                _Pragma("unroll") for (int g = 0; g < 4; ++g) {                                                              \
                    const f32x4 v = bi_[8 * t + 2 * g + h];                                                                  \
                    acc[t][4 * g + 0] = v[0]; acc[t][4 * g + 1] = v[1]; acc[t][4 * g + 2] = v[2]; acc[t][4 * g + 3] = v[3]; \
                }                                                                                                            \
        }
        {
            const f16x8* A = reinterpret_cast<const f16x8*>(smem) + lane;
#pragma unroll
            for (int t = 0; t < 8; ++t) fa[t] = A[(t * 2) * 64];
        }
        F2_INIT_TILE()
#define F2_MM(T, B) acc[T] = __builtin_amdgcn_mfma_f32_32x32x16_f16(fa[T], B, acc[T], 0, 0, 0);
#define F2_STAGE(U)                                                                                                          \
        {                                                                                                                    \
            const f16x8* Ac = reinterpret_cast<const f16x8*>(smem + slot_c) + lane;                                          \
            const unsigned slot_n = (slot_c + F2_SLOT) & (F2_RING * F2_SLOT - 1);                                            \
            const f16x8* An = reinterpret_cast<const f16x8*>(smem + slot_n) + lane;                                          \
                                       \
            KN_FENCE F2_MM(0, bq[U][0]) KN_FENCE fa[0] = Ac[(0 * 2 + 1) * 64]; F2_REQ_B1((U + 3) & 3)                           \
            KN_FENCE F2_MM(1, bq[U][0]) KN_FENCE fa[1] = Ac[(1 * 2 + 1) * 64];                                                  \
            KN_FENCE F2_MM(2, bq[U][0]) KN_FENCE fa[2] = Ac[(2 * 2 + 1) * 64];                                                  \
            KN_FENCE F2_MM(3, bq[U][0]) KN_FENCE fa[3] = Ac[(3 * 2 + 1) * 64];                                                  \
            KN_FENCE F2_MM(4, bq[U][0]) KN_FENCE fa[4] = Ac[(4 * 2 + 1) * 64];                                                  \
            KN_FENCE F2_MM(5, bq[U][0]) KN_FENCE fa[5] = Ac[(5 * 2 + 1) * 64];                                                  \
            KN_FENCE F2_MM(6, bq[U][0]) KN_FENCE fa[6] = Ac[(6 * 2 + 1) * 64];                                                  \
            KN_FENCE F2_MM(7, bq[U][0]) KN_FENCE fa[7] = Ac[(7 * 2 + 1) * 64];                                                  \
            KN_FENCE                                                                                                         \
                                \
            asm volatile("s_waitcnt vmcnt(8)" : "+v"(bq[(U + 1) & 3][0]), "+v"(bq[(U + 1) & 3][1]), "+v"(bq[U][1]) :: "memory"); \
            __builtin_amdgcn_s_barrier();      \
                 \
            if ((U) == 0 && w == 0) cl_tick(cs, clock0 + st, lane);    \
            KN_FENCE F2_MM(0, bq[U][1]) KN_FENCE fa[0] = An[(0 * 2) * 64]; F2_REQ_B0(U)                                         \
            KN_FENCE F2_MM(1, bq[U][1]) KN_FENCE fa[1] = An[(1 * 2) * 64];                                                      \
            KN_FENCE F2_MM(2, bq[U][1]) KN_FENCE fa[2] = An[(2 * 2) * 64]; F2_REQ_C(0)                                          \
            KN_FENCE F2_MM(3, bq[U][1]) KN_FENCE fa[3] = An[(3 * 2) * 64];                                                      \
            KN_FENCE F2_MM(4, bq[U][1]) KN_FENCE fa[4] = An[(4 * 2) * 64]; F2_REQ_C(1)                                          \
            KN_FENCE F2_MM(5, bq[U][1]) KN_FENCE fa[5] = An[(5 * 2) * 64];                                                      \
            KN_FENCE F2_MM(6, bq[U][1]) KN_FENCE fa[6] = An[(6 * 2) * 64];                                                      \
            KN_FENCE F2_MM(7, bq[U][1]) KN_FENCE fa[7] = An[(7 * 2) * 64];                                                      \
            KN_FENCE                                                                                                         \
            F2_ADVANCE()                                                                                                     \
            KN_FENCE                                                                                                         \
            slot_c = slot_n;                                                                                                 \
        }
        for (int st = 0; st < total; st += 4) {
            F2_STAGE(0) F2_STAGE(1) F2_STAGE(2) F2_STAGE(3)
            ks += 4;
            if (ks == NS) {
                if (seg.first && bt == seg.b_tile0 && cold_start_needed(thr)) thr = fmaxf(thr, cold_start_threshold(acc, k));
                pool_epilogue_scan<EMAX>(acc, thr, wl_s, wl_i, sc, w * 32, lane, k, (unsigned)bt, klw, pcnt, bulk);
                ks = 0; bt += seg.stride; cpar ^= 1;
                F2_INIT_TILE()
                {
                    const f16x8* A = reinterpret_cast<const f16x8*>(smem + slot_c) + lane;
#pragma unroll
                    for (int t = 0; t < 8; ++t) fa[t] = A[(t * 2) * 64];
                }
            }
        }
        asm volatile("s_waitcnt vmcnt(0)" : "+v"(bq[0][0]), "+v"(bq[0][1]), "+v"(bq[1][0]), "+v"(bq[1][1]), "+v"(bq[2][0]), "+v"(bq[2][1]),
                     "+v"(bq[3][0]), "+v"(bq[3][1]) :: "memory");
#undef F2_STAGE
#undef F2_MM
#undef F2_INIT_TILE
#undef F2_ADVANCE
#undef F2_REQ_B0
#undef F2_REQ_B1
#undef F2_REQ_C
        if (w == 0) cl_publish(cs, seg.next_tile0 == 0x7FFFFFFF ? 0x7FFFFFFF : seg.next_tile0 * NS, lane);
        {
            const knn_args_pool_view pv{HB_KARG(knn16_args, state_cnt), HB_KARG(knn16_args, state_thr)};
            pool_end(pv, seg.slot, pcnt, thr, myq, lane);
        }
        if (lane < 32) floor_publish(HB_KARG(knn16_args, gthr), seg.q_tile * HB_QT + myq, thr);
        asm volatile("s_waitcnt vmcnt(0)" ::: "memory");
        __syncthreads();
    }
    cl_finish(cs, a.cl_stats, w == 0, lane);
    wg_stamp<knn16_args>(1);
}

struct hb_rerank_seeds { const float* seed_in; float* kth_out; float* floor_out; };
template <bool CENTRED>
__device__ __forceinline__ bool hb_rerank_finish(const hb_rerank_seeds& sd, int64_t qi, bool ok, bool list_not_full, bool have_kth, float s, float E, float cq) {
    if (sd.seed_in && list_not_full && have_kth && !ok) ok = CENTRED ? s > sd.seed_in[qi] + cq + E : s > sd.seed_in[qi] + E;
    if (sd.kth_out) {
        const bool fin = have_kth && E < INFINITY && fabsf(s) < INFINITY && (!CENTRED || fabsf(cq) < INFINITY);
        float f = CENTRED ? s - cq - 1.001f * E : s - 1.001f * E;
        f = f - fabsf(f) * 2.4e-7f - 1e-37f;
        sd.kth_out[qi] = fin ? s : -INFINITY;
        sd.floor_out[qi] = fin ? f : -INFINITY;
    }
    return ok;
}

__device__ __forceinline__ float hb_centred_E(const hb_centre_view& cv, int64_t qi, float qn, float bmax, int d, int metric) {
    const float cmax = cv.sc[0], mun = cv.sc[1], at = fabsf(cv.sc[3]), qc = cv.qcn[qi];
    const float du = (float)(d + 4) * 1.2e-7f;
    return qc * cmax * (1.05f / 1024.0f + du)
           + du * (qn * bmax + qn * mun + 2.0f * at * mun * cmax + (metric == 1 ? bmax * bmax : 0.0f))
           + (qc + cmax) * sqrtf((float)d) * 6e-8f
           + 1e-30f;
}

template <bool CENTRED>
__global__ __launch_bounds__(256) void rerank_kernel(const float* __restrict__ tiles, const float* __restrict__ binit, int g8,
                                                     int d, const float* __restrict__ q, const float* __restrict__ qn2,
                                                     const int64_t* __restrict__ cand, const float* __restrict__ cand_score,
                                                     const float* __restrict__ qnorm, const float* __restrict__ bmax,
                                                     unsigned char* __restrict__ certified, int kc, int64_t nq, int k,
                                                     int64_t id_base, int metric, int out_metric, int64_t ntotal,
                                                     int64_t* __restrict__ out_idx, float* __restrict__ out_dist, hb_rerank_seeds sd, hb_centre_view cv) {
    __shared__ float s_sc[4][256];
    __shared__ int64_t s_id[4][256];
    const int lane = threadIdx.x & 63, wv = threadIdx.x >> 6;
    const int64_t qi = (int64_t)blockIdx.x * 4 + wv;
    if (qi >= nq) return;
    const float* qr = q + qi * (int64_t)d;
    const float E = CENTRED ? hb_centred_E(cv, qi, qnorm[qi], bmax[0], d, metric)
                            : qnorm[qi] * bmax[0] * (1.05f / 1024.0f + (float)d * 2.4e-7f)
                              + (qnorm[qi] + bmax[0]) * sqrtf((float)d) * 6e-8f
                              + (metric == 1 ? (float)d * 1.2e-7f * 0.5f * bmax[0] * bmax[0] : 0.0f)
                              + 1e-30f;
    const float cq = CENTRED ? cv.cq[qi] : 0.0f;
    const float cut = (k <= kc && cand[qi * (int64_t)kc + (k - 1)] >= 0) ? cand_score[qi * (int64_t)kc + (k - 1)] - 2.0f * E : -INFINITY;
    for (int c = lane; c < kc; c += 64) {
        const int64_t row = cand[qi * (int64_t)kc + c];
        float acc = -INFINITY;
        if (row >= 0 && !(c >= k && cand_score[qi * (int64_t)kc + c] < cut)) {
            acc = binit[row];
            const float* base = tiles + ((row >> 5) * (int64_t)g8) * HB_BLK + (int)(row & 31) * 4;
            for (int g = 0; g < g8; ++g) {
                const f32x4 e = *reinterpret_cast<const f32x4*>(base + (int64_t)g * HB_BLK);
                const f32x4 o = *reinterpret_cast<const f32x4*>(base + (int64_t)g * HB_BLK + 128);
                const int k0 = 8 * g;
#pragma unroll
                for (int j = 0; j < 4; ++j) {
                    if (k0 + 2 * j < d) acc = fmaf(qr[k0 + 2 * j], e[j], acc);
                    if (k0 + 2 * j + 1 < d) acc = fmaf(qr[k0 + 2 * j + 1], o[j], acc);
                }
            }
        }
        s_sc[wv][c] = acc;
        s_id[wv][c] = row;
    }
    __builtin_amdgcn_s_waitcnt(0xc07f);
    for (int c = lane; c < kc; c += 64) {
        const float s = s_sc[wv][c];
        const int64_t id = s_id[wv][c];
        int rank = 0;
        for (int j = 0; j < kc; ++j) {
            const float sj = s_sc[wv][j];
            const int64_t ij = s_id[wv][j];
            bool better;
            if (ij < 0 || id < 0) better = (ij >= 0 && id < 0) || (ij < 0 && id < 0 && j < c);
            else better = (sj > s) || (sj == s && (ij < id || (ij == id && j < c)));
            rank += better;
        }
        if (rank == k - 1) {
            const int64_t last = cand[qi * (int64_t)kc + kc - 1];
            const bool finite_q = CENTRED ? (cv.qcn[qi] <= 65504.0f && qnorm[qi] < INFINITY && fabsf(cq) < INFINITY) : qnorm[qi] <= 65504.0f;
            bool ok = last < 0 && ntotal < kc && finite_q;
            if (last >= 0 && id >= 0 && finite_q) {
                ok = CENTRED ? s > cand_score[qi * (int64_t)kc + kc - 1] + cq + E : s > cand_score[qi * (int64_t)kc + kc - 1] + E;
            }
            ok = hb_rerank_finish<CENTRED>(sd, qi, ok, last < 0, id >= 0 && finite_q, s, E, cq);
            certified[qi] = ok ? 1 : 0;
        }
        if (rank < k) {
            const int64_t o = qi * (int64_t)k + rank;
            if (id < 0) { out_idx[o] = -1; out_dist[o] = out_metric == 1 ? INFINITY : -INFINITY; }
            else {
                out_idx[o] = id + id_base;
                if (out_metric == 1) { const float d2 = fmaf(-2.0f, s, qn2[qi]); out_dist[o] = d2 > 0.0f ? d2 : 0.0f; }
                else out_dist[o] = s;
            }
        }
    }
}

int hb_launch_rerank(const float* tiles, const float* binit, int g8, int d, const float* q, const float* qn2,
                     const int64_t* cand, const float* cand_score, const float* qnorm, const float* bmax,
                     unsigned char* certified, int kc, int64_t nq, int k, int64_t id_base, int metric, int out_metric,
                     int64_t ntotal, int64_t* out_idx, float* out_dist, hipStream_t s, const float* seed_in, float* kth_out, float* floor_out,
                     const hb_centre_view* cv) {
    if (nq == 0) return 0;
    if (kc > 256) return hb_fail("hb_index_search: too many candidates for the re-rank kernel");
    auto fn = cv ? rerank_kernel<true> : rerank_kernel<false>;
    fn<<<dim3((unsigned)((nq + 3) / 4)), dim3(256), 0, s>>>(tiles, binit, g8, d, q, qn2, cand, cand_score, qnorm, bmax,
                                                          certified, kc, nq, k, id_base, metric, out_metric, ntotal, out_idx, out_dist,
                                                          hb_rerank_seeds{seed_in, kth_out, floor_out}, cv ? *cv : hb_centre_view{nullptr, nullptr, nullptr});
    HB_HIP(hipGetLastError());
    return 0;
}

__global__ __launch_bounds__(256) void tiles_to_rows_kernel(const float* __restrict__ t32, int g8, float* __restrict__ rows, int rs,
                                                            int64_t rt0) {
    __shared__ float s[4 * HB_BLK];
    const int64_t rt = rt0 + blockIdx.x;
    const int g0 = blockIdx.y * 4, ng = min(4, g8 - g0);
    const int t = threadIdx.x;
    if (t < ng * 64) reinterpret_cast<f32x4*>(s)[t] = reinterpret_cast<const f32x4*>(t32 + (rt * g8 + g0) * HB_BLK)[t];
    __syncthreads();
    const int i = t >> 3, c = t & 7;
    f32x4 out;
#pragma unroll
    for (int j = 0; j < 4; ++j) {
        const int kq = 4 * c + j, gl = kq >> 3, kk = kq & 7;
        out[j] = gl < ng ? s[gl * HB_BLK + ((kk & 1) * 32 + i) * 4 + (kk >> 1)] : 0.0f;
    }
    if (8 * g0 + 4 * c < rs) *reinterpret_cast<f32x4*>(rows + (rt * 32 + i) * (int64_t)rs + 8 * g0 + 4 * c) = out;
}

int hb_launch_tiles_to_rows(const float* t32, int g8, float* rows, int rs, int64_t n_row_tiles, int64_t rt0, hipStream_t s) {
    if (n_row_tiles <= 0) return 0;
    tiles_to_rows_kernel<<<dim3((unsigned)n_row_tiles, (unsigned)((rs / 8 + 3) / 4)), dim3(256), 0, s>>>(t32, g8, rows, rs, rt0);
    HB_HIP(hipGetLastError());
    return 0;
}

#define RRW_NONE 0xFFFFFFFFu
#define RRW_STRIDE 36
template <bool CENTRED>
__global__ __launch_bounds__(256) void rerank_rows_kernel(const float* __restrict__ rows, int rs, const float* __restrict__ binit,
                                                          int d, const float* __restrict__ q, const float* __restrict__ qn2,
                                                          const int64_t* __restrict__ cand, const float* __restrict__ cand_score,
                                                          const float* __restrict__ qnorm, const float* __restrict__ bmax,
                                                          unsigned char* __restrict__ certified, int kc, int64_t nq, int k,
                                                          int64_t id_base, int metric, int out_metric, int64_t ntotal,
                                                          int64_t* __restrict__ out_idx, float* __restrict__ out_dist, hb_rerank_seeds sd, hb_centre_view cv) {
    __shared__ float s_sc[4][256];
    __shared__ unsigned s_id[4][256];
    __shared__ int s_act[4][256];
    __shared__ __attribute__((aligned(16))) float s_img[4][66 * RRW_STRIDE];
    const int lane = threadIdx.x & 63, wv = threadIdx.x >> 6;
    const int64_t qi = (int64_t)blockIdx.x * 4 + wv;
    if (qi >= nq) return;
    const float* qr = q + qi * (int64_t)d;
    const float E = CENTRED ? hb_centred_E(cv, qi, qnorm[qi], bmax[0], d, metric)
                            : qnorm[qi] * bmax[0] * (1.05f / 1024.0f + (float)d * 2.4e-7f)
                              + (qnorm[qi] + bmax[0]) * sqrtf((float)d) * 6e-8f
                              + (metric == 1 ? (float)d * 1.2e-7f * 0.5f * bmax[0] * bmax[0] : 0.0f)
                              + 1e-30f;
    const float cq = CENTRED ? cv.cq[qi] : 0.0f;
    const float cut = (k <= kc && cand[qi * (int64_t)kc + (k - 1)] >= 0) ? cand_score[qi * (int64_t)kc + (k - 1)] - 2.0f * E : -INFINITY;
    int n_act = 0;
    for (int c0 = 0; c0 < kc; c0 += 64) {
        const int c = c0 + lane;
        int64_t row = -1;
        bool act = false;
        if (c < kc) {
            row = cand[qi * (int64_t)kc + c];
            act = row >= 0 && !(c >= k && cand_score[qi * (int64_t)kc + c] < cut);
            s_sc[wv][c] = -INFINITY;
            s_id[wv][c] = row >= 0 ? (unsigned)row : RRW_NONE;
        }
        const unsigned long long m = __ballot(act);
        if (act) s_act[wv][n_act + __popcll(m & ((1ull << lane) - 1ull))] = c;
        n_act += __popcll(m);
    }
    __builtin_amdgcn_s_waitcnt(0xc07f);
    __builtin_amdgcn_wave_barrier();
    float* img = s_img[wv];
    const int rr = lane >> 3, chn = lane & 7;
    const int nch = (d + 31) >> 5;
    for (int b0 = 0; b0 < n_act; b0 += 64) {
        const int nb = min(64, n_act - b0);
        const int nj = (nb + 1 + 7) >> 3;
        const int c = lane < nb ? s_act[wv][b0 + lane] : -1;
        float acc = c >= 0 ? binit[s_id[wv][c]] : 0.0f;
        const float* src[9];
#pragma unroll
        for (int j = 0; j < 9; ++j) {
            const int li = 8 * j + rr;
            src[j] = li < nb ? rows + (int64_t)s_id[wv][s_act[wv][b0 + li]] * rs + 4 * chn : (li == nb ? qr + 4 * chn : nullptr);
        }
        f32x4 R[9];
#define RRW_LOAD(CH)                                                                                                         \
        _Pragma("unroll") for (int j = 0; j < 9; ++j) {                                                                      \
            if (j < nj) {                                                                                                    \
                R[j] = f32x4{0.f, 0.f, 0.f, 0.f};                                                                            \
                if (src[j]) {                                                                                                \
                    const int k0 = 32 * (CH) + 4 * chn;                                                                      \
                    if (8 * j + rr < nb || k0 + 4 <= d) R[j] = *reinterpret_cast<const f32x4*>(src[j] + 32 * (CH));          \
                    else { _Pragma("unroll") for (int e = 0; e < 4; ++e) if (k0 + e < d) R[j][e] = src[j][32 * (CH) + e]; }   \
                }                                                                                                            \
            }                                                                                                                \
        }
        RRW_LOAD(0)
        for (int ch = 0; ch < nch; ++ch) {
#pragma unroll
            for (int j = 0; j < 9; ++j)
                if (j < nj && 8 * j + rr <= nb) *reinterpret_cast<f32x4*>(img + (8 * j + rr) * RRW_STRIDE + 4 * chn) = R[j];
            if (ch + 1 < nch) { RRW_LOAD(ch + 1) }
            __builtin_amdgcn_s_waitcnt(0xc07f);
            __builtin_amdgcn_wave_barrier();
            if (c >= 0) {
                const f32x4* xr = reinterpret_cast<const f32x4*>(img + lane * RRW_STRIDE);
                const f32x4* qv = reinterpret_cast<const f32x4*>(img + nb * RRW_STRIDE);
                if (32 * ch + 32 <= d) {
#pragma unroll
                    for (int i = 0; i < 8; ++i) {
                        const f32x4 x = xr[i], y = qv[i];
                        acc = fmaf(y[0], x[0], acc); acc = fmaf(y[1], x[1], acc); acc = fmaf(y[2], x[2], acc); acc = fmaf(y[3], x[3], acc);
                    }
                } else {
                    for (int i = 0; 32 * ch + i < d; ++i) acc = fmaf(img[nb * RRW_STRIDE + i], img[lane * RRW_STRIDE + i], acc);
                }
            }
            __builtin_amdgcn_wave_barrier();
        }
#undef RRW_LOAD
        if (c >= 0) s_sc[wv][c] = acc;
    }
    __builtin_amdgcn_s_waitcnt(0xc07f);
    __builtin_amdgcn_wave_barrier();
    for (int c = lane; c < kc; c += 64) {
        const float s = s_sc[wv][c];
        const int64_t id = s_id[wv][c] == RRW_NONE ? -1 : (int64_t)s_id[wv][c];
        int rank = 0;
        for (int j = 0; j < kc; ++j) {
            const float sj = s_sc[wv][j];
            const int64_t ij = s_id[wv][j] == RRW_NONE ? -1 : (int64_t)s_id[wv][j];
            bool better;
            if (ij < 0 || id < 0) better = (ij >= 0 && id < 0) || (ij < 0 && id < 0 && j < c);
            else better = (sj > s) || (sj == s && (ij < id || (ij == id && j < c)));
            rank += better;
        }
        if (rank == k - 1) {
            const int64_t last = cand[qi * (int64_t)kc + kc - 1];
            const bool finite_q = CENTRED ? (cv.qcn[qi] <= 65504.0f && qnorm[qi] < INFINITY && fabsf(cq) < INFINITY) : qnorm[qi] <= 65504.0f;
            bool ok = last < 0 && ntotal < kc && finite_q;
            if (last >= 0 && id >= 0 && finite_q) ok = CENTRED ? s > cand_score[qi * (int64_t)kc + kc - 1] + cq + E : s > cand_score[qi * (int64_t)kc + kc - 1] + E;
            ok = hb_rerank_finish<CENTRED>(sd, qi, ok, last < 0, id >= 0 && finite_q, s, E, cq);
            certified[qi] = ok ? 1 : 0;
        }
        if (rank < k) {
            const int64_t o = qi * (int64_t)k + rank;
            if (id < 0) { out_idx[o] = -1; out_dist[o] = out_metric == 1 ? INFINITY : -INFINITY; }
            else {
                out_idx[o] = id + id_base;
                if (out_metric == 1) { const float d2 = fmaf(-2.0f, s, qn2[qi]); out_dist[o] = d2 > 0.0f ? d2 : 0.0f; }
                else out_dist[o] = s;
            }
        }
    }
}

int hb_launch_rerank_rows(const float* rows, int rs, const float* binit, int d, const float* q, const float* qn2,
                          const int64_t* cand, const float* cand_score, const float* qnorm, const float* bmax,
                          unsigned char* certified, int kc, int64_t nq, int k, int64_t id_base, int metric, int out_metric,
                          int64_t ntotal, int64_t* out_idx, float* out_dist, hipStream_t s, const float* seed_in, float* kth_out, float* floor_out,
                          const hb_centre_view* cv) {
    if (nq == 0) return 0;
    if (kc > 256) return hb_fail("hb_index_search: too many candidates for the re-rank kernel");
    auto fn = cv ? rerank_rows_kernel<true> : rerank_rows_kernel<false>;
    fn<<<dim3((unsigned)((nq + 3) / 4)), dim3(256), 0, s>>>(rows, rs, binit, d, q, qn2, cand, cand_score, qnorm, bmax,
                                                          certified, kc, nq, k, id_base, metric, out_metric, ntotal, out_idx, out_dist,
                                                          hb_rerank_seeds{seed_in, kth_out, floor_out}, cv ? *cv : hb_centre_view{nullptr, nullptr, nullptr});
    HB_HIP(hipGetLastError());
    return 0;
}

int hb_knn_f16_launch(const knn16_args& args, int grid, hipStream_t s) {
    void (*fn)(knn16_args) = args.klw <= 256 ? knn_f16v2_kernel<4> : knn_f16v2_kernel<8>;
    if (args.klw > 512) return hb_fail("hb_index_search: candidate pools beyond 512 entries");
    if (hb_ensure_dyn_lds((const void*)fn, F2_LDS_TOTAL)) return -1;
    fn<<<dim3((unsigned)grid), dim3(HB_THREADS), F2_LDS_TOTAL, s>>>(args);
    HB_HIP(hipGetLastError());
    return 0;
}

__global__ __launch_bounds__(256) void bnorm_max_kernel(const float* __restrict__ bnorm, int64_t n, float* __restrict__ bmax) {
    float m = 0.0f;
    for (int64_t i = (int64_t)blockIdx.x * 256 + threadIdx.x; i < n; i += (int64_t)gridDim.x * 256) m = fmaxf(m, bnorm[i]);
    for (int o = 32; o > 0; o >>= 1) m = fmaxf(m, __shfl_xor(m, o));
    if ((threadIdx.x & 63) == 0) atomicMax(reinterpret_cast<int*>(bmax), __float_as_int(m));
}

int hb_launch_bnorm_max(const float* bnorm, int64_t n, float* bmax, hipStream_t s) {
    if (n == 0) return 0;
    const int64_t blocks = std::min<int64_t>((n + 255) / 256, 1024);
    bnorm_max_kernel<<<dim3((unsigned)blocks), dim3(256), 0, s>>>(bnorm, n, bmax);
    HB_HIP(hipGetLastError());
    return 0;
}

__global__ __launch_bounds__(256) void scatter_rows_kernel(const int64_t* __restrict__ rows, int64_t n, int k,
                                                           const int64_t* __restrict__ src_idx, const float* __restrict__ src_dist,
                                                           int64_t* __restrict__ out_idx, float* __restrict__ out_dist) {
    const int64_t t = (int64_t)blockIdx.x * 256 + threadIdx.x;
    if (t >= n * k) return;
    const int64_t i = t / k;
    const int j = (int)(t % k);
    out_idx[rows[i] * k + j] = src_idx[t];
    out_dist[rows[i] * k + j] = src_dist[t];
}

int hb_launch_scatter_rows(const int64_t* rows, int64_t n, int k, const int64_t* src_idx, const float* src_dist,
                           int64_t* out_idx, float* out_dist, hipStream_t s) {
    if (n == 0) return 0;
    scatter_rows_kernel<<<dim3((unsigned)((n * k + 255) / 256)), dim3(256), 0, s>>>(rows, n, k, src_idx, src_dist, out_idx, out_dist);
    HB_HIP(hipGetLastError());
    return 0;
}
```

### open-hummingbird-eval_amd/csrc/hbird_layout.hip

```cpp
#include "hbird_internal.h"
#include <algorithm>

__device__ __forceinline__ double wave8_sum(double v) {
    v += __shfl_xor(v, 1);
    v += __shfl_xor(v, 2);
    v += __shfl_xor(v, 4);
    return v;
}

template <bool NORMALIZE, bool IS_BANK>
__global__ __launch_bounds__(256) void rows_to_tiles_kernel(const float* __restrict__ src, int64_t n_valid,
                                                            int64_t n_cover, int d, int dp, int64_t row0,
                                                            float* __restrict__ tiles, float* __restrict__ binit,
                                                            float* __restrict__ bnorm, int metric) {
    __shared__ float s_scale[32];
    const int tid = threadIdx.x;
    const int64_t r_base = (int64_t)blockIdx.x * 32;
    const int g8 = dp >> 3;

    {
        const int i = tid >> 3, sub = tid & 7;
        const int64_t r = r_base + i;
        double acc = 0.0;
        if ((NORMALIZE || IS_BANK) && r < n_valid) {
// ... 169 lines not shown

static int g_layout_form = 0;
static int g_layout_rows = 0;
extern "C" int hb_set_layout_form(int form) {
    if (form != 0 && form != 1 && form != 8 && form != 16 && form != 32) return hb_fail("hb_set_layout_form: 0 (automatic), 1 (the first form) or 8 / 16 / 32 (rows per workgroup of the LDS form)");
    g_layout_form = form == 1 ? 1 : 0;
    g_layout_rows = form > 1 ? form : 0;
    return 0;
}

int hb_launch_rows_to_tiles(const float* src, int64_t n_rows, int d, int dp, int64_t row0, float* tiles, float* binit,
                            float* bnorm, int metric, int normalize, int is_bank, hipStream_t s) {
    int64_t n_cover = is_bank ? n_rows : ((n_rows + HB_QT - 1) / HB_QT) * HB_QT;
    if (n_cover == 0) return 0;
    dim3 grid((unsigned)((n_cover + 31) / 32)), block(256);
    if (g_layout_form == 0 && d % 16 == 0 && d == dp && d <= K1L_MAX_D && (reinterpret_cast<uintptr_t>(src) & 15) == 0) {
        const int rows = g_layout_rows > 0 ? g_layout_rows : (d <= 192 ? 32 : d <= 828 ? 16 : 8);
        const int lds = rows * (d + 4) * 4;
        typedef void (*k1_fn)(const float*, int64_t, int64_t, int, int64_t, float*, float*, float*, int);
        k1_fn fn;
        if (rows == 32) fn = is_bank ? (normalize ? (k1_fn)rows_to_tiles_lds_kernel<true, true, 32> : (k1_fn)rows_to_tiles_lds_kernel<false, true, 32>) : (k1_fn)rows_to_tiles_lds_kernel<false, false, 32>;
        else if (rows == 16) fn = is_bank ? (normalize ? (k1_fn)rows_to_tiles_lds_kernel<true, true, 16> : (k1_fn)rows_to_tiles_lds_kernel<false, true, 16>) : (k1_fn)rows_to_tiles_lds_kernel<false, false, 16>;
        else fn = is_bank ? (normalize ? (k1_fn)rows_to_tiles_lds_kernel<true, true, 8> : (k1_fn)rows_to_tiles_lds_kernel<false, true, 8>) : (k1_fn)rows_to_tiles_lds_kernel<false, false, 8>;
        if (hb_ensure_dyn_lds((const void*)fn, lds)) return -1;
        fn<<<dim3((unsigned)((n_cover + rows - 1) / rows)), block, lds, s>>>(src, n_rows, n_cover, d, row0, tiles, binit, bnorm, metric);
        HB_HIP(hipGetLastError());
        return 0;
    }
    if (is_bank) {
        if (normalize) rows_to_tiles_kernel<true, true><<<grid, block, 0, s>>>(src, n_rows, n_cover, d, dp, row0, tiles, binit, bnorm, metric);
        else rows_to_tiles_kernel<false, true><<<grid, block, 0, s>>>(src, n_rows, n_cover, d, dp, row0, tiles, binit, bnorm, metric);
    } else {
        rows_to_tiles_kernel<false, false><<<grid, block, 0, s>>>(src, n_rows, n_cover, d, dp, row0, tiles, nullptr, nullptr, metric);
    }
    HB_HIP(hipGetLastError());
    return 0;
}

__global__ __launch_bounds__(64) void query_aux_kernel(const float* __restrict__ q, int64_t nq, int d,
                                                       float* __restrict__ qn2, float* __restrict__ qnorm) {
    const int64_t r = (int64_t)blockIdx.x * 64 + threadIdx.x;
    if (r >= nq) return;
    const float* row = q + r * (int64_t)d;
    float acc = 0.0f;
    double a2 = 0.0;
    int k = 0;
    if ((d & 3) == 0 && (reinterpret_cast<uintptr_t>(q) & 15) == 0) {
#pragma unroll 4
        for (; k < d; k += 4) {
            const float4 v4 = *reinterpret_cast<const float4*>(row + k); const float v[4] = {v4.x, v4.y, v4.z, v4.w};
#pragma unroll
            for (int j = 0; j < 4; ++j) { acc = fmaf(v[j], v[j], acc); a2 += (double)v[j] * v[j]; }
        }
    }
    for (; k < d; ++k) { const float v = row[k]; acc = fmaf(v, v, acc); a2 += (double)v * v; }
    qn2[r] = acc;
    qnorm[r] = (float)sqrt(a2);
}

__global__ __launch_bounds__(256) void scores_to_l2_kernel(const float* __restrict__ qn2, int64_t n, int k, float* __restrict__ dist) {
    const int64_t i = (int64_t)blockIdx.x * 256 + threadIdx.x;
    if (i >= n) return;
    const float s = dist[i];
    if (s == -INFINITY) { dist[i] = INFINITY; return; }
    const float d2 = fmaf(-2.0f, s, qn2[i / k]);
    dist[i] = d2 > 0.0f ? d2 : 0.0f;
}

int hb_launch_scores_to_l2(const float* qn2, int64_t nq, int k, float* dist_inout, hipStream_t s) {
    const int64_t n = nq * k;
    if (n == 0) return 0;
    scores_to_l2_kernel<<<dim3((unsigned)((n + 255) / 256)), dim3(256), 0, s>>>(qn2, n, k, dist_inout);
    HB_HIP(hipGetLastError());
    return 0;
}

int hb_launch_query_aux(const float* q, int64_t nq, int d, float* qn2, float* qnorm, hipStream_t s) {
    if (nq == 0) return 0;
    query_aux_kernel<<<dim3((unsigned)((nq + 63) / 64)), dim3(64), 0, s>>>(q, nq, d, qn2, qnorm);
    HB_HIP(hipGetLastError());
    return 0;
}

__global__ __launch_bounds__(256) void tiles_to_rows_kernel(const float* __restrict__ tiles, int g8, int d,
                                                            const int64_t* __restrict__ ids, int64_t n,
                                                            int64_t id_base, int64_t ntotal, float* __restrict__ out) {
    const int lane = threadIdx.x & 63;
    const int64_t o = (int64_t)blockIdx.x * 4 + (threadIdx.x >> 6);
    if (o >= n) return;
    const int64_t gid = ids[o];
    float* dst = out + o * (int64_t)d;
    if (gid < 0 || gid < id_base || (uint64_t)gid - (uint64_t)id_base >= (uint64_t)ntotal) { for (int k = lane; k < d; k += 64) dst[k] = 0.0f; return; }
    const int64_t r = (int64_t)((uint64_t)gid - (uint64_t)id_base);
    const float* base = tiles + ((r >> 5) * (int64_t)g8) * HB_BLK;
    const int i = (int)(r & 31);
    for (int k = lane; k < d; k += 64) {
        const int g = k >> 3, kk = k & 7;
        dst[k] = base[(int64_t)g * HB_BLK + ((kk & 1) * 32 + i) * 4 + (kk >> 1)];
    }
}

int hb_launch_tiles_to_rows(const float* tiles, int g8, int d, const int64_t* ids, int64_t n, int64_t id_base, int64_t ntotal,
                            float* out, hipStream_t s) {
    if (n == 0) return 0;
    tiles_to_rows_kernel<<<dim3((unsigned)((n + 3) / 4)), dim3(256), 0, s>>>(tiles, g8, d, ids, n, id_base, ntotal, out);
    HB_HIP(hipGetLastError());
    return 0;
}

__global__ __launch_bounds__(256) void normalize_rows_kernel(const float* __restrict__ x, int64_t n, int d,
                                                             float* __restrict__ out) {
    const int lane = threadIdx.x & 63;
    const int64_t r = (int64_t)blockIdx.x * 4 + (threadIdx.x >> 6);
    if (r >= n) return;
    const float* row = x + r * (int64_t)d;
    double acc = 0.0;
    for (int k = lane; k < d; k += 64) { float v = row[k]; acc += (double)v * v; }
    for (int o = 32; o > 0; o >>= 1) acc += __shfl_xor(acc, o);
    const float nrm = (float)sqrt(acc);
    for (int k = lane; k < d; k += 64) out[r * (int64_t)d + k] = row[k] / nrm;
}

int hb_launch_normalize_rows(const float* x, int64_t n, int d, float* out, hipStream_t s) {
    if (n == 0) return 0;
    normalize_rows_kernel<<<dim3((unsigned)((n + 3) / 4)), dim3(256), 0, s>>>(x, n, d, out);
    HB_HIP(hipGetLastError());
    return 0;
}

__global__ __launch_bounds__(256) void gather_rows_kernel(const float* __restrict__ src, int64_t src_rows, int width,
                                                          const int64_t* __restrict__ ids, int64_t n,
                                                          float* __restrict__ out) {
    const int lane = threadIdx.x & 63;
    const int64_t o = (int64_t)blockIdx.x * 4 + (threadIdx.x >> 6);
    if (o >= n) return;
    const int64_t r = ids[o];
    const bool ok = r >= 0 && r < src_rows;
    for (int c = lane; c < width; c += 64) out[o * (int64_t)width + c] = ok ? src[r * (int64_t)width + c] : 0.0f;
}

int hb_launch_gather_rows(const float* src, int64_t src_rows, int width, const int64_t* ids, int64_t n, float* out,
                          hipStream_t s) {
    if (n == 0) return 0;
    gather_rows_kernel<<<dim3((unsigned)((n + 3) / 4)), dim3(256), 0, s>>>(src, src_rows, width, ids, n, out);
    HB_HIP(hipGetLastError());
    return 0;
}
```

### open-hummingbird-eval_amd/csrc/hbird_schedule.cpp

```cpp
#include "hbird_schedule.h"
#include <algorithm>
#include <cmath>
#include <map>

#ifdef HB_PLAN_STANDALONE
static thread_local std::string g_plan_err;
int hb_fail(const std::string& msg) { g_plan_err = msg; return -1; }
extern "C" const char* hb_last_error(void) { return g_plan_err.c_str(); }
#endif

static int hb_gcd(int x, int y) { while (y) { int t = x % y; x = y; y = t; } return x; }

int hb_default_panel(int nqt, int G, size_t tile_bytes, int cq, int cb) {
    int p0;
    if (cq * cb > 1) {
        const int NC = std::max(1, G / (cq * cb)), NQG = (nqt + cq - 1) / cq;
        p0 = cb * (NC / hb_gcd(NQG, NC));
    } else p0 = G / hb_gcd(nqt, G);
    size_t budget = (size_t)96 << 20;
    int j = (int)std::max<size_t>(1, budget / (tile_bytes * (size_t)p0));
    return p0 * j;
}

void hb_default_cluster(int nqt, int nbt, int G, bool fp32_kernel, int* cq, int* cb) {
// ... 88 lines not shown
    return cum;
}
static long long hb_share_bound(long long W, const std::vector<double>& cum, int i, int workers, int panel_index) {
    if (i <= 0) return 0;
    if (i >= workers) return W;
    const double phi = std::fmod(0.5 + 0.6180339887498949 * panel_index, 1.0);
    return std::min<long long>(W, std::max<long long>(0, (long long)std::floor((double)W * cum[i] + phi)));
}

static void hb_build_clustered(int nqt, int nbt, int G, int panel, int cq, int cb, hb_schedule& out, bool xcd_share) {
    const int CS = cq * cb, NC = G / CS, NQG = (nqt + cq - 1) / cq;
    out.cq = cq; out.cb = cb; out.n_clusters = NC; out.xcd_share = xcd_share;
    std::vector<std::vector<hb_seg>> per_wg(G);
    std::vector<int> slot_of((size_t)G * nqt, -1);
    std::vector<std::vector<int>> slots_of_qt(nqt);
    std::vector<int> clock(NC, 0);
    auto deal = [&](int c, int b0, int pp, int qg, int j0, int cnt) {
        for (int m = 0; m < CS; ++m) {
            const int ia = m / cb, ib = m % cb, q = qg * cq + ia, w = c * CS + m;
            int n = cnt;
            if ((j0 + cnt - 1) * cb + ib >= pp) --n;
            if (q >= nqt || n <= 0) continue;
            hb_seg sg;
            sg.q_tile = q; sg.b_tile0 = b0 + j0 * cb + ib; sg.n_tiles = n; sg.stride = cb; sg.tile0 = clock[c]; sg.next_tile0 = 0;
            int& known = slot_of[(size_t)w * nqt + q];
            if (known < 0) {
                sg.slot = out.n_slots++; sg.first = 1;
                known = sg.slot;
                slots_of_qt[q].push_back(sg.slot);
            } else { sg.slot = known; sg.first = 0; }
            per_wg[w].push_back(sg);
        }
        clock[c] += cnt;
    };
    const int per_xcd_c = NC / 8;
    int rot = 0;
    const std::vector<double> cum = (!out.xcd_w.empty() && !xcd_share && NC % 8 == 0) ? hb_cum_shares(NC, NC / 8, out.xcd_w) : std::vector<double>();
    const std::vector<double> cumx = (!out.xcd_w.empty() && xcd_share) ? hb_cum_shares(8, 1, out.xcd_w) : std::vector<double>();
    for (int b0 = 0; b0 < nbt; b0 += panel) {
        const int pp = std::min(panel, nbt - b0);
        const int UB = (pp + cb - 1) / cb;
        const long long U = (long long)NQG * UB;
        if (xcd_share) {
            for (int x = 0; x < 8; ++x) {
                long long e = (U * x) / 8;
                long long e1 = (U * (x + 1)) / 8;
                if (!cumx.empty()) { e = hb_share_bound(U, cumx, x, 8, b0 / panel); e1 = hb_share_bound(U, cumx, x + 1, 8, b0 / panel); }
                while (e < e1) {
                    const int qg = (int)(e / UB), j0 = (int)(e % UB);
                    const int L = (int)std::min<long long>(UB - j0, e1 - e);
                    for (int i = 0; i < per_xcd_c; ++i) {
                        const int a0 = (int)((long long)L * i / per_xcd_c), a1 = (int)((long long)L * (i + 1) / per_xcd_c);
                        if (a1 > a0) deal(x * per_xcd_c + (i + rot) % per_xcd_c, b0, pp, qg, j0 + a0, a1 - a0);
                    }
                    ++rot;
                    e += L;
                }
            }
            continue;
        }
        for (int c = 0; c < NC; ++c) {
            long long e0 = (U * c) / NC, e1 = (U * (c + 1)) / NC;
            if (!cum.empty()) { e0 = hb_share_bound(U, cum, c, NC, b0 / panel); e1 = hb_share_bound(U, cum, c + 1, NC, b0 / panel); }
            while (e0 < e1) {
                const int qg = (int)(e0 / UB), j0 = (int)(e0 % UB);
                const int cnt = (int)std::min<long long>(UB - j0, e1 - e0);
                deal(c, b0, pp, qg, j0, cnt);
                e0 += cnt;
            }
        }
    }
    std::vector<int> logical_of_block(G);
    out.wg_member.assign(G, -1);
    const int per_xcd = NC / 8;
    for (int c = 0; c < NC; ++c)
        for (int m = 0; m < CS; ++m) {
            const int block = c / per_xcd + 8 * ((c % per_xcd) * CS + m);
            logical_of_block[block] = c * CS + m;
            out.wg_member[block] = c * HB_CLUSTER_LINE + m;
        }
    hb_finish_schedule(out, per_wg, logical_of_block, slots_of_qt);
}

void hb_build_schedule(int nqt, int nbt, int G, int panel, hb_schedule& out, int cq, int cb, bool phased, bool xcd_share, const double* xcd_w) {
    out = hb_schedule();
    out.nqt = nqt; out.nbt = nbt; out.panel = panel; out.phased = phased;
    if (xcd_w) {
        bool ok = true, equal = true;
        for (int x = 0; x < 8; ++x) { ok = ok && xcd_w[x] > 0.25 && xcd_w[x] < 4.0; equal = equal && xcd_w[x] == xcd_w[0]; }
        if (ok && !equal) out.xcd_w.assign(xcd_w, xcd_w + 8);
    }
    const long long total_pairs = (long long)nqt * nbt;
    if (total_pairs < G) G = (int)std::max<long long>(1, total_pairs);
    out.G = G;
    if (phased) {
        const long long per_wg_tiles = total_pairs / G;
        long long t = 0, step = 1;
        while (out.phase_clock.size() < HB_PHASE_CUTS) {
            t += step;
            if (t * 2 > per_wg_tiles) break;
            out.phase_clock.push_back((int)t);
            step = std::max<long long>(step + 1, per_wg_tiles <= 64 ? step * 3 : step < 128 ? step * 3 / 2 : step * 2);
        }
    }
    if (cq < 1 || cb < 1 || cq * cb > HB_CLUSTER_MAX || G % (8 * cq * cb) != 0) { cq = 1; cb = 1; }
    if (cq * cb > 1) { hb_build_clustered(nqt, nbt, G, panel, cq, cb, out, xcd_share); return; }
    std::vector<std::vector<hb_seg>> per_wg(G);
    std::vector<int> slot_of((size_t)G * nqt, -1);
    std::vector<std::vector<int>> slots_of_qt(nqt);
    std::vector<int> clock(G, 0);
    const std::vector<double> cum = (!out.xcd_w.empty() && G % 8 == 0) ? hb_cum_shares(G, G / 8, out.xcd_w) : std::vector<double>();
    for (int b0 = 0; b0 < nbt; b0 += panel) {
        const int pp = std::min(panel, nbt - b0);
        const long long W = (long long)nqt * pp;
        for (int w = 0; w < G; ++w) {
            long long e0 = (W * w) / G, e1 = (W * (w + 1)) / G;
            if (!cum.empty()) { e0 = hb_share_bound(W, cum, w, G, b0 / panel); e1 = hb_share_bound(W, cum, w + 1, G, b0 / panel); }
            while (e0 < e1) {
                const int q = (int)(e0 / pp), b = (int)(e0 % pp);
                const int cnt = (int)std::min<long long>(pp - b, e1 - e0);
                int& known = slot_of[(size_t)w * nqt + q];
                hb_seg sg;
                sg.q_tile = q; sg.b_tile0 = b0 + b; sg.n_tiles = cnt; sg.stride = 1; sg.tile0 = clock[w]; sg.next_tile0 = 0;
                clock[w] += cnt;
                if (known < 0) {
                    sg.slot = out.n_slots++; sg.first = 1;
                    known = sg.slot;
                    slots_of_qt[q].push_back(sg.slot);
                } else { sg.slot = known; sg.first = 0; }
                if (!per_wg[w].empty()) {
                    hb_seg& pv = per_wg[w].back();
                    if (pv.slot == sg.slot && pv.b_tile0 + pv.n_tiles == sg.b_tile0) { pv.n_tiles += cnt; e0 += cnt; continue; }
                }
                per_wg[w].push_back(sg);
                e0 += cnt;
            }
        }
    }
    std::vector<int> logical_of_block(G);
    for (int b = 0; b < G; ++b) {
        if (G % 8 == 0) logical_of_block[b] = (b % 8) * (G / 8) + b / 8;
        else {
            const int q = G / 8, r = G % 8, x = b % 8;
            logical_of_block[b] = (x < r ? x * (q + 1) : r * (q + 1) + (x - r) * q) + b / 8;
        }
    }
    out.wg_member.assign(G, -1);
    hb_finish_schedule(out, per_wg, logical_of_block, slots_of_qt);
}


static int schedule_plan(int nqt, int nbt, int workgroups, int panel_tiles, int d, int cluster_q, int cluster_b, bool phased,
                         int* segs_out, int64_t max_segs, int64_t stats[8], hb_schedule& sc, bool xcd_share = false, const double* xcd_w = nullptr) {
    if (!stats) return hb_fail("hb_schedule_plan: stats is NULL");
    if (nqt <= 0 || nbt <= 0 || workgroups <= 0 || d <= 0) return hb_fail("hb_schedule_plan: bad arguments");
    const int dp = (d + HB_KC - 1) / HB_KC * HB_KC;
    const int G = (int)std::min<long long>(workgroups, (long long)nqt * nbt);
    int cq = cluster_q, cb = cluster_b;
    if (cq < 0 || cb < 0) hb_default_cluster(nqt, nbt, G, cq == -2, &cq, &cb);
    if (cq < 1 || cb < 1 || (long long)nqt * nbt < workgroups || cq * cb > HB_CLUSTER_MAX || G % (8 * cq * cb) != 0) { cq = 1; cb = 1; }
    const int panel = panel_tiles > 0 ? panel_tiles : hb_default_panel(nqt, G, (size_t)HB_BT * dp * 4, cq, cb);
    hb_build_schedule(nqt, nbt, workgroups, panel, sc, cq, cb, phased, xcd_share && cq * cb > 1, xcd_w);
    stats[0] = sc.G; stats[1] = (int64_t)sc.segs.size(); stats[2] = sc.n_slots; stats[3] = sc.panel;
    stats[4] = sc.max_slots_per_qt; stats[5] = sc.nqt; stats[6] = sc.nbt; stats[7] = sc.cq * 16 + sc.cb;
    if (segs_out) {
        int64_t n = 0;
        for (int b = 0; b < sc.G; ++b)
            for (int i = sc.wg_off[b]; i < sc.wg_off[b + 1] && n < max_segs; ++i, ++n) {
                const hb_seg& g = sc.segs[i];
                int* o = segs_out + n * 10;
                o[0] = b; o[1] = g.q_tile; o[2] = g.b_tile0; o[3] = g.n_tiles; o[4] = g.slot; o[5] = g.first;
                o[6] = g.stride; o[7] = g.tile0; o[8] = g.next_tile0; o[9] = sc.wg_member[b];
            }
    }
    return 0;
}

extern "C" int hb_schedule_plan(int nqt, int nbt, int workgroups, int panel_tiles, int d, int cluster_q, int cluster_b,
                                int* segs_out, int64_t max_segs, int64_t stats[8]) {
    hb_schedule sc;
    return schedule_plan(nqt, nbt, workgroups, panel_tiles, d, cluster_q, cluster_b, false, segs_out, max_segs, stats, sc);
}

extern "C" int hb_schedule_plan_phased(int nqt, int nbt, int workgroups, int panel_tiles, int d, int cluster_q, int cluster_b,
                                       int* segs_out, int64_t max_segs, int64_t stats[8], int* clocks_out, int max_cuts, int* n_cuts,
                                       int* bounds_out) {
    if (!n_cuts) return hb_fail("hb_schedule_plan_phased: n_cuts is NULL");
    hb_schedule sc;
    if (schedule_plan(nqt, nbt, workgroups, panel_tiles, d, cluster_q, cluster_b, true, segs_out, max_segs, stats, sc)) return -1;
    *n_cuts = (int)sc.phase_clock.size();
    for (int p = 0; p < *n_cuts && p < max_cuts; ++p) {
        if (clocks_out) clocks_out[p] = sc.phase_clock[p];
        if (bounds_out)
            for (int b = 0; b < sc.G; ++b) bounds_out[(size_t)p * sc.G + b] = sc.phase_bounds[(size_t)p * sc.G + b] - sc.wg_off[b];
    }
    return 0;
}

extern "C" int hb_schedule_plan_weighted(int nqt, int nbt, int workgroups, int panel_tiles, int d, int cluster_q, int cluster_b, int shared,
                                         const double* xcd_w8, int* segs_out, int64_t max_segs, int64_t stats[8]) {
    hb_schedule sc;
    return schedule_plan(nqt, nbt, workgroups, panel_tiles, d, cluster_q, cluster_b, (shared & 2) != 0, segs_out, max_segs, stats, sc, (shared & 1) != 0, xcd_w8);
}

extern "C" int hb_schedule_plan_shared(int nqt, int nbt, int workgroups, int panel_tiles, int d, int cluster_q, int cluster_b, int phased,
                                       int* segs_out, int64_t max_segs, int64_t stats[8]) {
    hb_schedule sc;
    return schedule_plan(nqt, nbt, workgroups, panel_tiles, d, cluster_q, cluster_b, phased != 0, segs_out, max_segs, stats, sc, true);
}
```

### open-hummingbird-eval_amd/csrc/hbird_schedule.h

```cpp
#pragma once
#include <stddef.h>
#include <stdint.h>
#include <string>
#include <vector>

#define HB_QT 256
#define HB_BT 256
#define HB_KC 16

struct hb_seg {
    int q_tile;
    int b_tile0;
    int n_tiles;
    int slot;
    int first;
    int stride;
    int tile0;
    int next_tile0;
    int ord;
    int nsl;
};

#define HB_PHASE_CUTS 24
#define HB_CLUSTER_MAX 8
#define HB_CLUSTER_LINE 32

struct hb_schedule {
    int nqt = 0, nbt = 0, G = 0, panel = 0;
    int cq = 1, cb = 1;
    bool xcd_share = false;
    std::vector<double> xcd_w;
    std::vector<hb_seg> segs;
    std::vector<int> wg_off;
    std::vector<int> wg_member;
    bool phased = false;
    std::vector<int> phase_clock;
    bool cuts_scaled = false;
    std::vector<int> phase_bounds;
    std::vector<int> qt_off;
    std::vector<int> qt_slots;
    int n_slots = 0;
    int max_slots_per_qt = 0;
    int n_clusters = 0;
};

void hb_build_schedule(int nqt, int nbt, int G, int panel_tiles, hb_schedule& out, int cq = 1, int cb = 1, bool phased = false,
                       bool xcd_share = false, const double* xcd_w = nullptr);
int hb_default_panel(int nqt, int G, size_t tile_bytes, int cq = 1, int cb = 1);
void hb_default_cluster(int nqt, int nbt, int G, bool fp32_kernel, int* cq, int* cb);

int hb_fail(const std::string& msg);
```

### open-hummingbird-eval_amd/hbird_mi/_lib.py

```python
from __future__ import annotations

import ctypes
import os
from ctypes import POINTER, c_char_p, c_double, c_float, c_int, c_int64, c_uint64, c_void_p

_PKG_ROOT = os.path.dirname(os.path.dirname(os.path.abspath(__file__)))
LIB_PATH = os.environ.get("HBIRD_HIP_LIB") or os.path.join(_PKG_ROOT, "lib", "libhbird_hip.so")
CSRC_DIR = os.path.join(_PKG_ROOT, "csrc")

_lib = None

SIGNATURES = {
    "hb_last_error": (c_char_p, []),
    "hb_device_count": (c_int, [POINTER(c_int)]),
    "hb_index_create": (c_int, [c_int, c_int, c_int, POINTER(c_void_p)]),
    "hb_index_free": (c_int, [c_void_p]),
    "hb_index_set_stream": (c_int, [c_void_p, c_void_p]),
    "hb_index_reserve": (c_int, [c_void_p, c_int64]),
    "hb_index_add": (c_int, [c_void_p, c_void_p, c_int64, c_int, c_int]),
    "hb_index_add_labels": (c_int, [c_void_p, c_void_p, c_int64, c_int, c_int]),
    "hb_index_ntotal": (c_int64, [c_void_p]),
    "hb_index_nlabels": (c_int64, [c_void_p]),
    "hb_index_reset": (c_int, [c_void_p]),
    "hb_index_search": (c_int, [c_void_p, c_void_p, c_int64, c_int, c_int64, c_void_p, c_void_p, c_int]),
    "hb_index_search_aggregate": (c_int, [c_void_p, c_void_p, c_int64, c_int, c_int64, c_float, c_void_p, c_void_p,
                                          c_void_p, c_int]),
    "hb_index_aggregate": (c_int, [c_void_p, c_void_p, c_int64, c_void_p, c_void_p, c_int, c_int64, c_float,
                                   c_void_p, c_int]),
    "hb_index_aggregate_partial": (c_int, [c_void_p, c_void_p, c_int64, c_void_p, c_void_p, c_int, c_int64, c_float, c_void_p, c_int64,
                                           c_void_p]),
    "hb_index_reconstruct": (c_int, [c_void_p, c_void_p, c_int64, c_int64, c_void_p, c_int]),
    "hb_index_gather_labels": (c_int, [c_void_p, c_void_p, c_int64, c_int64, c_void_p, c_int]),
    "hb_index_set_label_table": (c_int, [c_void_p, c_void_p, c_void_p, c_int64, c_int, c_int64]),
    "hb_index_copy_norms": (c_int, [c_void_p, c_void_p, c_int]),
    "hb_index_set_score_output": (c_int, [c_void_p, c_int]),
    "hb_index_distances_from_scores": (c_int, [c_void_p, c_void_p, c_int64, c_int, c_void_p]),
    "hb_merge_topk": (c_int, [c_void_p, c_void_p, c_int, c_int64, c_int, c_int, c_void_p, c_void_p, c_void_p]),
    "hb_packed_list_bytes": (c_int64, [c_int64, c_int]),
    "hb_merge_topk_packed": (c_int, [c_void_p, c_int64, c_int, c_int64, c_int, c_int, c_void_p, c_void_p, c_void_p]),
    "hb_bigk_search_aggregate": (c_int, [c_void_p, c_void_p, c_int64, c_int, c_int64, c_float, c_void_p, c_void_p,
                                         c_void_p, c_int]),
    "hb_bigk_aggregate": (c_int, [c_void_p, c_void_p, c_int64, c_void_p, c_void_p, c_int, c_int64, c_float,
                                  c_void_p, c_int]),
    "hb_bigk_aggregate_partial": (c_int, [c_void_p, c_void_p, c_int64, c_void_p, c_void_p, c_int, c_int64, c_float, c_void_p, c_int64,
                                          c_void_p]),
    "hb_bigk_merge_topk": (c_int, [c_void_p, c_void_p, c_int, c_int64, c_int, c_int, c_void_p, c_void_p, c_void_p]),
    "hb_bigk_merge_topk_packed": (c_int, [c_void_p, c_int64, c_int, c_int64, c_int, c_int, c_void_p, c_void_p, c_void_p]),
    "hb_multi_create": (c_int, [c_int, c_int, POINTER(c_int), c_int, c_int, POINTER(c_void_p)]),
    "hb_multi_free": (c_int, [c_void_p]),
    "hb_multi_reserve": (c_int, [c_void_p, c_int64]),
    "hb_multi_add": (c_int, [c_void_p, c_void_p, c_int64, c_int]),
    "hb_multi_ntotal": (c_int64, [c_void_p]),
    "hb_multi_shard_rows": (c_int, [c_void_p, POINTER(c_int64), c_int]),
    "hb_multi_set_fp16": (c_int, [c_void_p, c_int]),
    "hb_multi_search": (c_int, [c_void_p, c_void_p, c_int64, c_int, c_void_p, c_void_p]),
    "hb_normalize_rows": (c_int, [c_void_p, c_int64, c_int, c_void_p, c_void_p]),
    "hb_patch_label_hist": (c_int, [c_void_p, c_int64, c_int, c_int, c_int, c_int, c_int, c_void_p, c_void_p]),
    "hb_patch_scores": (c_int, [c_void_p, c_int64, c_int, c_int, c_void_p, c_void_p, c_void_p, c_void_p]),
    "hb_patch_select": (c_int, [c_void_p, c_void_p, c_void_p, c_void_p, c_int64, c_int, c_int, c_void_p, c_void_p,
                                c_void_p]),
    "hb_gather_rows": (c_int, [c_void_p, c_int64, c_int, c_void_p, c_int64, c_void_p, c_void_p]),
    "hb_upsample_argmax": (c_int, [c_void_p, c_int64, c_int, c_int, c_int, c_int, c_void_p, c_void_p]),
    "hb_upsample_argmax_confusion": (c_int, [c_void_p, c_int64, c_int, c_int, c_int, c_int, c_void_p, c_int, c_int, c_int64, c_int,
                                             c_void_p, c_void_p, c_void_p]),
    "hb_upsample_accumulate": (c_int, [c_void_p, c_int64, c_int, c_int, c_int, c_int, c_void_p, c_int, c_int, c_int, c_int,
                                       c_void_p]),
    "hb_argmax_channels": (c_int, [c_void_p, c_int64, c_int, c_void_p, c_void_p]),
    "hb_confusion_update": (c_int, [c_void_p, c_void_p, c_int64, c_int, c_int, c_int64, c_int, c_void_p, c_void_p]),
    "hb_index_set_timing": (c_int, [c_void_p, c_int]),
    "hb_index_last_knn_ms": (c_int, [c_void_p, POINTER(c_double)]),
    "hb_index_set_tuning": (c_int, [c_void_p, c_int, c_int]),
    "hb_index_set_fp16": (c_int, [c_void_p, c_int]),
    "hb_index_last_fp16_fallbacks": (c_int, [c_void_p, POINTER(c_int64)]),
    "hb_last_search_path": (c_int, [c_void_p, POINTER(c_int), POINTER(c_int)]),
    "hb_index_set_fp16_escalation": (c_int, [c_void_p, c_int]),
    "hb_index_last_fp16_escalated": (c_int, [c_void_p, POINTER(c_int64)]),
    "hb_schedule_plan": (c_int, [c_int, c_int, c_int, c_int, c_int, c_int, c_int, c_void_p, c_int64, POINTER(c_int64)]),
    "hb_schedule_plan_phased": (c_int, [c_int, c_int, c_int, c_int, c_int, c_int, c_int, c_void_p, c_int64, POINTER(c_int64),
                                        c_void_p, c_int, POINTER(c_int), c_void_p]),
    "hb_schedule_plan_shared": (c_int, [c_int, c_int, c_int, c_int, c_int, c_int, c_int, c_int, c_void_p, c_int64, POINTER(c_int64)]),
    "hb_index_set_cluster": (c_int, [c_void_p, c_int, c_int, c_int]),
    "hb_index_set_cluster_sharing": (c_int, [c_void_p, c_int]),
    "hb_index_set_label_denominator": (c_int, [c_void_p, c_int]),
    "hb_index_labels_to_fp32": (c_int, [c_void_p]),
    "hb_index_label_denominator": (c_int, [c_void_p, POINTER(c_int)]),
    "hb_index_copy_label_counts": (c_int, [c_void_p, c_void_p, c_int]),
    "hb_index_set_label_count_table": (c_int, [c_void_p, c_void_p, c_void_p, c_int64, c_int, c_int, c_int64]),
    "hb_index_cluster_stats": (c_int, [c_void_p, POINTER(c_int64)]),
    "hb_index_set_variant": (c_int, [c_void_p, c_int]),
    "hb_index_set_search_options": (c_int, [c_void_p, c_int, c_int64]),
    "hb_index_wg_stamps": (c_int, [c_void_p, c_void_p, c_int, POINTER(c_int)]),
    "hb_index_set_xcd_weights": (c_int, [c_void_p, c_int, POINTER(c_double)]),
    "hb_index_xcd_weights": (c_int, [c_void_p, c_int, POINTER(c_double), POINTER(c_int)]),
    "hb_schedule_plan_weighted": (c_int, [c_int, c_int, c_int, c_int, c_int, c_int, c_int, c_int, POINTER(c_double), c_void_p, c_int64, POINTER(c_int64)]),
    "hb_index_kernel_clock": (c_int, [c_void_p, POINTER(c_double)]),
    "hb_index_xcd_stats": (c_int, [c_void_p, c_int, POINTER(c_double)]),
    "hb_calibration_new": (c_void_p, [c_int]),
    "hb_calibration_free": (None, [c_void_p]),
    "hb_calibration_state": (c_int, [c_void_p, POINTER(c_double), POINTER(c_int64)]),
    "hb_calibration_feed": (c_int, [c_void_p, c_void_p, c_int, POINTER(c_double), POINTER(c_int), c_int, c_double]),
    "hb_f16_adapt_replay": (c_int, [c_int, POINTER(c_double), POINTER(c_double), c_int64, POINTER(c_int)]),
    "hb_exact_screen_replay": (c_int, [c_int, c_int, c_int, c_int, c_int, c_int64, c_int64, c_int, c_int64, c_int, c_int, c_int,
                                       c_uint64, c_uint64, c_uint64, c_uint64, POINTER(c_int)]),
    "hb_knn_plan_replay": (c_int, [POINTER(c_int64), c_int, POINTER(c_int64), c_int]),
    "hb_set_layout_form": (c_int, [c_int]),
    "hb_index_set_rerank_copy": (c_int, [c_void_p, c_int]),
    "hb_index_rerank_copy_bytes": (c_int, [c_void_p, POINTER(c_int64)]),
    "hb_index_schedule_info": (c_int, [c_void_p, POINTER(c_int64)]),
}

SIGNATURES_CENTRE = {
    "hb_index_set_fp16_centre": (c_int, [c_void_p, c_int]),
    "hb_index_fp16_centre_info": (c_int, [c_void_p, POINTER(c_double)]),
    "hb_multi_set_fp16_centre": (c_int, [c_void_p, c_int]),
}

SIGNATURES_SELECT = {
    "hb_index_add_from": (c_int, [c_void_p, c_void_p, c_void_p, c_int64, c_int]),
    "hb_index_select_rows": (c_int, [c_void_p, c_void_p, c_int64, c_int, POINTER(c_void_p)]),
}

GRID_MAX_CONFIGS = 16
SIGNATURES_GRID = {
    "hb_index_aggregate_grid": (c_int, [c_void_p, c_void_p, c_int64, c_void_p, c_void_p, c_int, c_int64, POINTER(c_int), c_int,
                                        POINTER(c_float), c_int, c_void_p, c_int]),
    "hb_index_search_aggregate_grid": (c_int, [c_void_p, c_void_p, c_int64, c_int64, POINTER(c_int), c_int, POINTER(c_float), c_int,
                                               c_void_p, c_void_p, c_void_p, c_int]),
}


class HbirdHipError(RuntimeError):
    pass


class HbirdClassRangeError(HbirdHipError, ValueError):
    """A mask holds a class id outside [0, num_classes): F.one_hot of the reference raises for it (hbird_eval.py:319)."""


def lib() -> ctypes.CDLL:
    global _lib
    if _lib is None:
        if not os.path.exists(LIB_PATH):
            raise HbirdHipError(
                f"{LIB_PATH} is missing: build the HIP extension first (python -c 'import __graft_entry__ as g; "
                f"g.build()' or make -C {CSRC_DIR}). There is no CPU fallback.")
        L = ctypes.CDLL(LIB_PATH)
        plan_only = os.environ.get("HBIRD_PLAN_ONLY") == "1"
        for name, (res, args) in list(SIGNATURES.items()) + list(SIGNATURES_CENTRE.items()) + list(SIGNATURES_SELECT.items()) + list(SIGNATURES_GRID.items()):
            if plan_only and not (name.startswith("hb_schedule_plan") or name.startswith("hb_calibration_") or name in ("hb_f16_adapt_replay", "hb_exact_screen_replay", "hb_knn_plan_replay") or name == "hb_last_error"):
                continue
            fn = getattr(L, name)
            fn.restype = res
            fn.argtypes = args
        _lib = L
    return _lib


def last_error() -> str:
    msg = lib().hb_last_error()
    return msg.decode() if msg else ""


def check(rc: int, exc=HbirdHipError):
    if rc != 0:
        raise exc(last_error() or f"libhbird_hip call failed with status {rc}")


def device_count() -> int:
    n = c_int(0)
    lib().hb_device_count(ctypes.byref(n))
    return int(n.value)
```

Baseline: 77880.

## Batch workspace memsets into one init kernel and fuse query f16 tiling

Several separate hipMemsetAsync/MemsetD32 calls on the search workspace (floors, stamps, progress counters, phase state, level buffers) are gathered into one range list and cleared by a single state-init launch. The progress reset between phases is folded into pool_floor_kernel. Query fp32 tiling moves into the kNN path so it runs only where it is needed, and a direct rows-to-f16-tiles kernel is added. This cuts launch and queue overhead per search, at the cost of more coupling between the workspace setup and the kernels. It also adds a first-clock option for phased schedules and a failure counter for rerank.

```diff
diff --git a/include/hbird_hip.h b/include/hbird_hip.h
--- a/include/hbird_hip.h
+++ b/include/hbird_hip.h
@@ -142,6 +142,7 @@
 int hb_calibration_feed(void* h, const uint32_t* stamps, int G, const double run_shares8[8], const int key6[6], int auto_cluster, double frac);
 int hb_f16_adapt_replay(int n, const double* f1, const double* f2, int64_t nq, int* out_how);
 int hb_set_layout_form(int form);
+int hb_query_tiles_f16(const float* q_dev, int64_t nq, int d, int direct, void* out_dev, int64_t out_bytes, void* stream);
 int hb_index_set_rerank_copy(hb_index_t* ix, int mode);
 int hb_index_rerank_copy_bytes(const hb_index_t* ix, int64_t* bytes);
 int hb_index_schedule_info(const hb_index_t* ix, int64_t out[8]);
@@ -154,6 +155,9 @@
 int hb_schedule_plan_phased(int nqt, int nbt, int workgroups, int panel_tiles, int d, int cluster_q, int cluster_b, int* segs_out,
                             int64_t max_segs, int64_t stats[8], int* clocks_out, int max_cuts, int* n_cuts, int* bounds_out);
 
+int hb_schedule_plan_phased_from(int nqt, int nbt, int workgroups, int panel_tiles, int d, int cluster_q, int cluster_b, int first_clock,
+                                 int* segs_out, int64_t max_segs, int64_t stats[8], int* clocks_out, int max_cuts, int* n_cuts, int* bounds_out);
+
 int hb_schedule_plan_shared(int nqt, int nbt, int workgroups, int panel_tiles, int d, int cluster_q, int cluster_b, int phased,
                             int* segs_out, int64_t max_segs, int64_t stats[8]);
 
diff --git a/open-hummingbird-eval_amd/csrc/hbird_capi.hip b/open-hummingbird-eval_amd/csrc/hbird_capi.hip
--- a/open-hummingbird-eval_amd/csrc/hbird_capi.hip
+++ b/open-hummingbird-eval_amd/csrc/hbird_capi.hip
@@ -222,8 +222,25 @@
 extern "C" int hb_index_set_search_options(hb_index_t* ix, int phases, int64_t small_limit_stages) {
     if (!ix) return hb_fail("hb_index_set_search_options: NULL index handle");
     if (small_limit_stages < 0) return hb_fail("hb_index_set_search_options: negative limit");
-    ix->phases_on = phases ? 1 : 0; ix->small_limit = small_limit_stages; ix->sched = hb_schedule(); ix->fp32_pinned = 1;
-    return 0;
+    if (phases < 0) return hb_fail("hb_index_set_search_options: phases must be 0 (off), 1 (on) or the first cut clock of an A/B run (> 1)");
+    ix->phases_on = phases; ix->small_limit = small_limit_stages; ix->sched = hb_schedule(); ix->fp32_pinned = 1;
+    return 0;
+}
+extern "C" int hb_query_tiles_f16(const float* q_dev, int64_t nq, int d, int direct, void* out_dev, int64_t out_bytes, void* stream) {
+    if (!q_dev || !out_dev || nq < 1 || d < 1) return hb_fail("hb_query_tiles_f16: bad arguments");
+    const int dp = (d + HB_KC - 1) / HB_KC * HB_KC, dp16 = (d + 127) / 128 * 128;
+    const int64_t nqp = (nq + HB_QT - 1) / HB_QT * HB_QT;
+    if (out_bytes < nqp * dp16 * 2) return hb_fail("hb_query_tiles_f16: the output holds fewer than ceil(nq / 256) * 256 rows of ceil(d / 128) * 128 halves");
+    hipStream_t s = (hipStream_t)stream;
+    if (direct) return hb_launch_rows_to_f16_tiles(q_dev, nq, d, (_Float16*)out_dev, dp16 / 16, s);
+    float* t32 = nullptr;
+    HB_HIP(hipMalloc((void**)&t32, (size_t)nqp * dp * 4));
+    int rc = hb_launch_rows_to_tiles(q_dev, nq, d, dp, 0, t32, nullptr, nullptr, 0, 0, 0, s);
+    if (!rc) rc = hb_launch_tiles_to_f16(t32, dp / 8, (_Float16*)out_dev, dp16 / 16, nqp / 32, 0, nullptr, s);
+    const hipError_t e = hipStreamSynchronize(s);
+    (void)hipFree(t32);
+    if (!rc && e != hipSuccess) return hb_fail(std::string("hb_query_tiles_f16: ") + hipGetErrorString(e));
+    return rc;
 }
 extern "C" int hb_index_set_xcd_weights(hb_index_t* ix, int mode, const double* w8) {
     if (!ix) return hb_fail("hb_index_set_xcd_weights: NULL index handle");
@@ -550,7 +567,6 @@
     if (b_lab) { d_lab = (float*)cur; cur += b_lab; }
     {
         hb_range r("hbird:query_tiles");
-        if (hb_launch_rows_to_tiles(qd, nq, ix->d, ix->dp, 0, ix->q_tiles, nullptr, nullptr, ix->metric, 0, 0, ix->stream)) return -1;
         if (hb_launch_query_aux(qd, nq, ix->d, ix->q_aux, ix->q_aux + nq, ix->stream)) return -1;
     }
     {
diff --git a/open-hummingbird-eval_amd/csrc/hbird_internal.h b/open-hummingbird-eval_amd/csrc/hbird_internal.h
--- a/open-hummingbird-eval_amd/csrc/hbird_internal.h
+++ b/open-hummingbird-eval_amd/csrc/hbird_internal.h
@@ -118,22 +118,33 @@
                             float* binit, float* bnorm, int metric, int normalize, int is_bank, hipStream_t s);
 int hb_launch_scores_to_l2(const float* qn2, int64_t nq, int k, float* dist_inout, hipStream_t s);
 int hb_launch_query_aux(const float* q, int64_t nq, int d, float* qn2, float* qnorm, hipStream_t s);
+#define HB_INIT_RANGES 10
+struct hb_init_ranges {
+    unsigned* p[HB_INIT_RANGES]; unsigned long long n[HB_INIT_RANGES]; unsigned v[HB_INIT_RANGES]; int count = 0, dropped = 0;
+    void add(void* ptr, size_t words, unsigned value) {
+        if (!words) return;
+        if (count == HB_INIT_RANGES) { ++dropped; return; }
+        p[count] = static_cast<unsigned*>(ptr); n[count] = words; v[count] = value; ++count;
+    }
+};
+int hb_launch_state_init(const hb_init_ranges& r, hipStream_t s);
 int hb_launch_tiles_to_rows(const float* tiles, int g8, int d, const int64_t* ids, int64_t n, int64_t id_base, int64_t ntotal,
                             float* out, hipStream_t s);
 int hb_launch_knn(hb_index* ix, const float* q_dev, int64_t nq, int k, int64_t id_base, int64_t* out_idx, float* out_dist);
 int hb_launch_tiles_to_f16(const float* t32, int g8, _Float16* t16, int g16, int64_t n_row_tiles, int64_t rt0, int* overflow,
                            hipStream_t s);
+int hb_launch_rows_to_f16_tiles(const float* src, int64_t n_rows, int d, _Float16* t16, int g16, hipStream_t s);
 int hb_launch_tiles_to_rows(const float* t32, int g8, float* rows, int rs, int64_t n_row_tiles, int64_t rt0, hipStream_t s);
 int hb_launch_rerank_rows(const float* rows, int rs, const float* binit, int d, const float* q, const float* qn2,
                           const int64_t* cand, const float* cand_score, const float* qnorm, const float* bmax,
                           unsigned char* certified, int kc, int64_t nq, int k, int64_t id_base, int metric, int out_metric,
                           int64_t ntotal, int64_t* out_idx, float* out_dist, hipStream_t s, const float* seed_in = nullptr, float* kth_out = nullptr,
-                          float* floor_out = nullptr, const hb_centre_view* cv = nullptr);
+                          float* floor_out = nullptr, const hb_centre_view* cv = nullptr, unsigned* n_failed = nullptr);
 int hb_launch_rerank(const float* tiles, const float* binit, int g8, int d, const float* q, const float* qn2,
                      const int64_t* cand, const float* cand_score, const float* qnorm, const float* bmax,
                      unsigned char* certified, int kc, int64_t nq, int k, int64_t id_base, int metric, int out_metric, int64_t ntotal, int64_t* out_idx,
                      float* out_dist, hipStream_t s, const float* seed_in = nullptr, float* kth_out = nullptr, float* floor_out = nullptr,
-                     const hb_centre_view* cv = nullptr);
+                     const hb_centre_view* cv = nullptr, unsigned* n_failed = nullptr);
 int hb_launch_bnorm_max(const float* bnorm, int64_t n, float* bmax, hipStream_t s);
 int hb_launch_scatter_rows(const int64_t* rows, int64_t n, int k, const int64_t* src_idx, const float* src_dist,
                            int64_t* out_idx, float* out_dist, hipStream_t s);
diff --git a/open-hummingbird-eval_amd/csrc/hbird_knn.hip b/open-hummingbird-eval_amd/csrc/hbird_knn.hip
--- a/open-hummingbird-eval_amd/csrc/hbird_knn.hip
+++ b/open-hummingbird-eval_amd/csrc/hbird_knn.hip
@@ -400,9 +400,10 @@
 __global__ __launch_bounds__(256) void pool_floor_kernel(const float* __restrict__ state_s, const int* __restrict__ cnts,
                                                         const float* __restrict__ pthr, const int* __restrict__ qt_off,
                                                         const int* __restrict__ qt_slots, int64_t nq, int kk, int klw, int per_wave,
-                                                        unsigned* __restrict__ gthr) {
+                                                        unsigned* __restrict__ gthr, int* __restrict__ prog, int prog_words) {
     extern __shared__ __attribute__((aligned(16))) char smem[];
     const int lane = threadIdx.x & 63, w = threadIdx.x >> 6;
+    if (prog) for (int64_t e = (int64_t)blockIdx.x * 256 + threadIdx.x; e < prog_words; e += (int64_t)gridDim.x * 256) prog[e] = 0;
     const int64_t q = (int64_t)blockIdx.x * 4 + w;
     if (q >= nq) return;
     pool_floor_query(state_s, cnts, pthr, qt_off, qt_slots, q, kk, klw, reinterpret_cast<float*>(smem) + (size_t)w * per_wave, gthr, lane);
@@ -494,6 +495,7 @@
     bool timed = false;
     const float* q_aux = nullptr;
     bool score_out = false;
+    bool q32_tiled = false;
 };
 static int knn_search(hb_index* ix, const knn_call& c, const float* q_dev, int64_t nq, int k, int64_t id_base, int64_t* out_idx, float* out_dist);
 
@@ -512,9 +514,11 @@
     const int out_metric = c.score_out ? 0 : ix->metric;
     double knn_ms = 0.0;
     int rc = 0;
+    if (!c.q32_tiled && hb_launch_rows_to_tiles(q_dev, nq, ix->d, ix->dp, 0, ix->q_tiles, nullptr, nullptr, ix->metric, 0, 0, s)) return -1;
     for (int col0 = 0; col0 < k && !rc; col0 += 256) {
         const int kp = std::min(256, k - col0);
         knn_call pass = c;
+        pass.q32_tiled = true;
         pass.score_out = true;
         pass.ceil_s = col0 ? ceil_s : nullptr; pass.ceil_i = col0 ? ceil_i : nullptr;
         rc = knn_search(ix, pass, q_dev, nq, kp, 0, tmp_idx, tmp_sc);
@@ -658,7 +662,7 @@
     const bool rebuilt = !(sc.nqt == nqt && sc.nbt == nbt && sc.panel == p.panel && sc.cq == p.cq && sc.cb == p.cb && sc.phased == p.phased &&
                            sc.xcd_share == p.xs && (sc.G == G || (long long)nqt * nbt < G) &&
                            (sc.xcd_w.empty() ? std::equal(shares, shares + 8, equal_shares) : std::equal(shares, shares + 8, sc.xcd_w.begin())));
-    if (rebuilt) { hb_build_schedule(nqt, nbt, G, p.panel, sc, p.cq, p.cb, p.phased, p.xs, shares); ++ix->sched_builds; }
+    if (rebuilt) { hb_build_schedule(nqt, nbt, G, p.panel, sc, p.cq, p.cb, p.phased, p.xs, shares, ix->phases_on > 1 ? ix->phases_on : 0); ++ix->sched_builds; }
     const struct { const void* data; size_t bytes; } part[6] = {{sc.segs.data(), sc.segs.size() * sizeof(hb_seg)}, {sc.wg_off.data(), sc.wg_off.size() * 4},
         {sc.qt_off.data(), sc.qt_off.size() * 4}, {sc.qt_slots.data(), sc.qt_slots.size() * 4}, {sc.wg_member.data(), sc.wg_member.size() * 4},
         {sc.phase_bounds.data(), sc.phase_bounds.size() * 4}};
@@ -683,7 +687,7 @@
     size_t prog_bytes = 0, stamp_bytes = 0;
 };
 static int knn_carve_workspace(hb_index* ix, const knn_call& c, const hb_knn_plan& p, const knn_work_list& wl, int64_t nq, int k, hipStream_t s,
-                               knn_workspace* out) {
+                               const hb_init_ranges& tail, knn_workspace* out) {
     const hb_schedule& sc = *wl.sc;
     const int nqt = p.nqt, klw = p.klw, esc = c.esc;
     const size_t state_half = (size_t)sc.n_slots * HB_QT * klw * 4;
@@ -697,7 +701,8 @@
     knn_args& a = out->a;
     a.wg_stamp = esc == 0 && (c.timed || p.calibrated) ? reinterpret_cast<unsigned*>(floors + floor_bytes + prog_bytes) : nullptr;
     if (esc == 0) { ix->wg_stamp_dev = a.wg_stamp; ix->wg_stamp_blocks = sc.G; }
-    if (a.wg_stamp) HB_HIP(hipMemsetAsync(a.wg_stamp, 0, stamp_bytes, s));
+    hb_init_ranges init = tail;
+    if (a.wg_stamp) init.add(a.wg_stamp, stamp_bytes / 4, 0u);
     a.bank_tiles = ix->tiles; a.binit = ix->binit; a.q_tiles = ix->q_tiles;
     a.ceil_s = c.ceil_s; a.ceil_i = c.ceil_i; a.segs = wl.segs; a.wg_off = wl.wg_off; a.wg_end = a.wg_off + 1;
     a.state_s = reinterpret_cast<float*>(ix->state);
@@ -707,31 +712,39 @@
     a.state_thr = reinterpret_cast<float*>(ix->state + 2 * state_half + state_aux);
     a.gthr = reinterpret_cast<unsigned*>(floors);
     a.qfl = a.gthr + (size_t)nqt * HB_QT;
-    HB_HIP(hipMemsetD32Async((hipDeviceptr_t)a.gthr, 0x007FFFFF, (size_t)nqt * HB_QT * 17, s));
-    if (nq < (int64_t)nqt * HB_QT) HB_HIP(hipMemsetD32Async((hipDeviceptr_t)(a.gthr + nq), 0xFF800000u, (size_t)((int64_t)nqt * HB_QT - nq), s));
-    if (esc != 0 && c.seed) {
-        seed_from_scores_kernel<<<dim3((unsigned)((nq + 255) / 256)), dim3(256), 0, s>>>(c.seed, nq, a.gthr);
-        HB_HIP(hipGetLastError());
-    }
+    const size_t nqp = (size_t)nqt * HB_QT;
+    init.add(a.gthr, (size_t)nq, 0x007FFFFFu);
+    init.add(a.gthr + nqp, nqp * 16, 0x007FFFFFu);
+    init.add(a.gthr + nq, nqp - (size_t)nq, 0xFF800000u);
     a.wg_member = wl.wg_member; a.prog = reinterpret_cast<int*>(floors + floor_bytes);
     a.cl = sc.cq * sc.cb; a.lag = p.lag;
     a.cl_stats = a.prog + (size_t)std::max(1, sc.n_clusters) * HB_CLUSTER_MAX * HB_CLUSTER_LINE;
     ix->cl_stats_dev = a.cl > 1 ? a.cl_stats : nullptr;
-    if (a.cl > 1) HB_HIP(hipMemsetAsync(a.prog, 0, prog_bytes, s));
+    if (a.cl > 1) init.add(a.prog, prog_bytes / 4, 0u);
+    if (wl.n_phases > 1) {
+        init.add(a.state_cnt, state_aux / 4, 0u);
+        init.add(a.state_thr, state_aux / 4, 0xFF800000u);
+    }
+    if (hb_launch_state_init(init, s)) return -1;
+    if (esc != 0 && c.seed) {
+        seed_from_scores_kernel<<<dim3((unsigned)((nq + 255) / 256)), dim3(256), 0, s>>>(c.seed, nq, a.gthr);
+        HB_HIP(hipGetLastError());
+    }
     return 0;
 }
 
 static int knn_seed_floors(hb_index* ix, const knn_args& a, const knn_work_list& wl, int nqt, int klw, int64_t nq, int kk, int64_t* scratch_idx,
-                           float* scratch_dist, hipStream_t s) {
+                           float* scratch_dist, int prog_words, hipStream_t s) {
     const hb_schedule& sc = *wl.sc;
     const size_t per_wave = (size_t)sc.max_slots_per_qt * klw;
     if (per_wave * 16 <= 144 * 1024) {
         if (per_wave * 16 > 48 * 1024 && hb_ensure_dyn_lds((const void*)pool_floor_kernel, 144 * 1024)) return -1;
         pool_floor_kernel<<<dim3((unsigned)((nq + 3) / 4)), dim3(256), per_wave * 16, s>>>(a.state_s, a.state_cnt, a.state_thr, wl.qt_off, wl.qt_slots, nq, kk,
-                                                                                           klw, (int)per_wave, a.gthr);
+                                                                                           klw, (int)per_wave, a.gthr, prog_words > 0 ? a.prog : nullptr, prog_words);
         HB_HIP(hipGetLastError());
         return 0;
     }
+    if (prog_words > 0) HB_HIP(hipMemsetAsync(a.prog, 0, (size_t)prog_words * 4, s));
     if (launch_merge(ix, a.state_s, a.state_i, a.state_cnt, a.state_thr, wl.qt_off, wl.qt_slots, sc.max_slots_per_qt, nqt, nq, kk, klw, 0, 0, nullptr,
                      scratch_idx, scratch_dist, s)) return -1;
     seed_floors_kernel<<<dim3((unsigned)((nq + 255) / 256)), dim3(256), 0, s>>>(scratch_idx, scratch_dist, nq, kk, a.gthr);
@@ -744,15 +757,10 @@
                           int64_t* scratch_idx, float* scratch_dist, hipStream_t s, Launch launch) {
     const knn_args& a = ws.a;
     if (c.timed) HB_HIP(hipEventRecord(ix->ev0, s));
-    if (wl.n_phases > 1) {
-        HB_HIP(hipMemsetAsync(a.state_cnt, 0, ws.state_aux, s));
-        HB_HIP(hipMemsetD32Async((hipDeviceptr_t)a.state_thr, 0xFF800000u, ws.state_aux / 4, s));
-    }
     for (int ph = 0; ph < wl.n_phases; ++ph) {
         if (launch(wl.phase_begin(ph), wl.phase_end(ph))) return -1;
         if (ph + 1 < wl.n_phases) {
-            if (knn_seed_floors(ix, a, wl, p.nqt, p.klw, nq, kk, scratch_idx, scratch_dist, s)) return -1;
-            if (a.cl > 1) HB_HIP(hipMemsetAsync(a.prog, 0, ws.prog_bytes - HB_CLUSTER_LINE * 4, s));
+            if (knn_seed_floors(ix, a, wl, p.nqt, p.klw, nq, kk, scratch_idx, scratch_dist, a.cl > 1 ? (int)(ws.prog_bytes / 4) - HB_CLUSTER_LINE : 0, s)) return -1;
         }
     }
     if (c.timed) HB_HIP(hipEventRecord(ix->ev1, s));
@@ -773,9 +781,18 @@
     size_t o_kth, o_flo, o_rows;
     knn_level_buf(hb_index* ix, int esc, int64_t nq) : buf(esc == 0 ? ix->fb : ix->fb1), bytes(esc == 0 ? ix->fb_bytes : ix->fb1_bytes), o_kth(al256((size_t)nq + 64)),
                                                        o_flo(o_kth + al256((size_t)nq * 4)), o_rows(o_flo + al256((size_t)nq * 4)) {}
+    unsigned* n_failed() const { return reinterpret_cast<unsigned*>(buf + o_kth - 64); }
     float* kth() const { return reinterpret_cast<float*>(buf + o_kth); }
     float* flo() const { return reinterpret_cast<float*>(buf + o_flo); }
 };
+
+static int knn_level_init(hb_index* ix, int esc, int64_t nq, hb_init_ranges* init) {
+    const knn_level_buf lv(ix, esc, nq);
+    if (ensure_bytes(&lv.buf, &lv.bytes, lv.o_rows)) return -1;
+    init->add(lv.kth(), (lv.o_rows - lv.o_kth) / 4, 0xFF800000u);
+    init->add(lv.n_failed(), 1, 0u);
+    return 0;
+}
 
 static int knn_research_failures(hb_index* ix, const knn_call& c, const knn_path& path, const hb_knn_plan& p, const knn_work_list& wl, const knn_workspace& ws,
                                  const std::vector<int64_t>& bad, const float* q_dev, int64_t nq, int k, int64_t id_base, int64_t* out_idx, float* out_dist,
@@ -807,7 +824,6 @@
     HB_HIP(hipMemcpyAsync(d_rows, bad.data(), (size_t)nf * 8, hipMemcpyHostToDevice, s));
     if (hb_launch_gather_rows(q_dev, nq, ix->d, d_rows, nf, d_q, s)) return -1;
     if (hb_launch_gather_rows(again16 ? flo : kth, nq, 1, d_rows, nf, d_seed, s)) return -1;
-    if (hb_launch_rows_to_tiles(d_q, nf, ix->d, ix->dp, 0, ix->q_tiles, nullptr, nullptr, ix->metric, 0, 0, s)) return -1;
     if (esc == 0 && ws.a.wg_stamp) {
         const hb_schedule& sc = *wl.sc;
         const size_t stamp_bytes = ws.stamp_bytes;
@@ -844,7 +860,7 @@
     if (ensure_bytes((char**)&ix->q16, &ix->q16_bytes, (size_t)nqp * ix->dp16 * 2)) return -1;
     hb_centre_view cview{nullptr, nullptr, nullptr};
     if (centred) { if (hb_centre_queries(ix, nq, esc == 0, (_Float16*)ix->q16, &cview, s)) return -1; }
-    else if (hb_launch_tiles_to_f16(ix->q_tiles, ix->g8, (_Float16*)ix->q16, ix->dp16 / 16, nqp / 32, 0, nullptr, s)) return -1;
+    else if (hb_launch_rows_to_f16_tiles(q_dev, nq, ix->d, (_Float16*)ix->q16, ix->dp16 / 16, s)) return -1;
     const hb_centre_view* cv = centred ? &cview : nullptr;
     if (ensure_bytes(&ix->cand, &ix->cand_bytes, (size_t)nq * kc * 12)) return -1;
     int64_t* cand_idx = reinterpret_cast<int64_t*>(ix->cand);
@@ -862,23 +878,26 @@
     if (launch_merge(ix, a.state_s, a.state_i, a.state_cnt, a.state_thr, wl.qt_off, wl.qt_slots, sc.max_slots_per_qt, nqt, nq, kc, klw, 0, 0, nullptr,
                      cand_idx, cand_dist, s)) return -1;
     const knn_level_buf lv(ix, esc, nq);
-    if (ensure_bytes(&lv.buf, &lv.bytes, lv.o_rows)) return -1;
     unsigned char* cert = reinterpret_cast<unsigned char*>(lv.buf);
     float *kth = lv.kth(), *flo = lv.flo();
-    HB_HIP(hipMemsetD32Async((hipDeviceptr_t)kth, 0xFF800000u, (lv.o_rows - lv.o_kth) / 4, s));
     const float* seed_in = esc == 1 ? c.seed : nullptr;
     const float* q_aux = c.q_aux;
     if (ix->rows32 && ix->rerank_copy != 2 && ix->rows32_rows >= ix->ntotal) {
         if (hb_launch_rerank_rows(ix->rows32, ix->rows32_rs, ix->binit, ix->d, q_dev, q_aux, cand_idx, cand_dist, q_aux + nq, ix->bmax,
-                                  cert, kc, nq, k, id_base, ix->metric, out_metric, ix->ntotal, out_idx, out_dist, s, seed_in, kth, flo, cv)) return -1;
+                                  cert, kc, nq, k, id_base, ix->metric, out_metric, ix->ntotal, out_idx, out_dist, s, seed_in, kth, flo, cv, lv.n_failed())) return -1;
     } else if (hb_launch_rerank(ix->tiles, ix->binit, ix->g8, ix->d, q_dev, q_aux, cand_idx, cand_dist, q_aux + nq, ix->bmax,
-                                cert, kc, nq, k, id_base, ix->metric, out_metric, ix->ntotal, out_idx, out_dist, s, seed_in, kth, flo, cv)) return -1;
+                                cert, kc, nq, k, id_base, ix->metric, out_metric, ix->ntotal, out_idx, out_dist, s, seed_in, kth, flo, cv, lv.n_failed())) return -1;
     if (knn_read_time(ix, c)) return -1;
-    std::vector<unsigned char> hc((size_t)nq);
-    HB_HIP(hipMemcpyAsync(hc.data(), cert, (size_t)nq, hipMemcpyDeviceToHost, s));
+    unsigned n_failed = 0;
+    HB_HIP(hipMemcpyAsync(&n_failed, lv.n_failed(), 4, hipMemcpyDeviceToHost, s));
     HB_HIP(hipStreamSynchronize(s));
     std::vector<int64_t> bad;
-    for (int64_t i = 0; i < nq; ++i) if (!hc[i]) bad.push_back(i);
+    if (n_failed) {
+        std::vector<unsigned char> hc((size_t)nq);
+        HB_HIP(hipMemcpyAsync(hc.data(), cert, (size_t)nq, hipMemcpyDeviceToHost, s));
+        HB_HIP(hipStreamSynchronize(s));
+        for (int64_t i = 0; i < nq; ++i) if (!hc[i]) bad.push_back(i);
+    }
     const int64_t nf = (int64_t)bad.size();
     if (esc == 0) { ix->last_fp16_escalated = 0; ix->last_fp16_fallbacks = 0; }
     if (esc == 0 && nf == 0) hb_f16_observe(ix->f16_adapt, path.how16, nq, 0, 0);
@@ -938,6 +957,8 @@
         HB_HIP(hipStreamSynchronize(s));
         return 0;
     }
+    if (!c.q32_tiled && (!path.f16 || path.centred) &&
+        hb_launch_rows_to_tiles(q_dev, nq, ix->d, ix->dp, 0, ix->q_tiles, nullptr, nullptr, ix->metric, 0, 0, s)) return -1;
     hb_knn_plan_in pin;
     pin.f16 = path.f16; pin.wide_first = path.wide_first; pin.esc = esc; pin.ceil = c.ceil_s != nullptr;
     pin.k = k; pin.nq = nq; pin.ntotal = ix->ntotal; pin.g8 = ix->g8; pin.dp = ix->dp; pin.dp16 = ix->dp16; pin.num_cu = ix->num_cu;
@@ -952,7 +973,9 @@
     if (knn_get_work_list(ix, esc, p, s, &wl)) return -1;
     hb_knn_plan_kernel(pin, wl.sc->G, p);
     knn_workspace ws;
-    if (knn_carve_workspace(ix, c, p, wl, nq, k, s, &ws)) return -1;
+    hb_init_ranges tail;
+    if (path.f16 && knn_level_init(ix, esc, nq, &tail)) return -1;
+    if (knn_carve_workspace(ix, c, p, wl, nq, k, s, tail, &ws)) return -1;
     if (path.f16) return knn_search_f16(ix, c, path, p, wl, ws, q_dev, nq, k, id_base, out_metric, out_idx, out_dist, s);
     return knn_search_f32(ix, c, p, wl, ws, nq, k, id_base, out_metric, out_idx, out_dist, s);
 }
diff --git a/open-hummingbird-eval_amd/csrc/hbird_knn_f16.hip b/open-hummingbird-eval_amd/csrc/hbird_knn_f16.hip
--- a/open-hummingbird-eval_amd/csrc/hbird_knn_f16.hip
+++ b/open-hummingbird-eval_amd/csrc/hbird_knn_f16.hip
@@ -201,7 +201,7 @@
     wg_stamp<knn16_args>(1);
 }
 
-struct hb_rerank_seeds { const float* seed_in; float* kth_out; float* floor_out; };
+struct hb_rerank_seeds { const float* seed_in; float* kth_out; float* floor_out; unsigned* n_failed; };
 template <bool CENTRED>
 __device__ __forceinline__ bool hb_rerank_finish(const hb_rerank_seeds& sd, int64_t qi, bool ok, bool list_not_full, bool have_kth, float s, float E, float cq) {
     if (sd.seed_in && list_not_full && have_kth && !ok) ok = CENTRED ? s > sd.seed_in[qi] + cq + E : s > sd.seed_in[qi] + E;
@@ -212,6 +212,7 @@
         sd.kth_out[qi] = fin ? s : -INFINITY;
         sd.floor_out[qi] = fin ? f : -INFINITY;
     }
+    if (sd.n_failed && !ok) atomicAdd(sd.n_failed, 1u);
     return ok;
 }
 
@@ -304,13 +305,13 @@
                      const int64_t* cand, const float* cand_score, const float* qnorm, const float* bmax,
                      unsigned char* certified, int kc, int64_t nq, int k, int64_t id_base, int metric, int out_metric,
                      int64_t ntotal, int64_t* out_idx, float* out_dist, hipStream_t s, const float* seed_in, float* kth_out, float* floor_out,
-                     const hb_centre_view* cv) {
+                     const hb_centre_view* cv, unsigned* n_failed) {
     if (nq == 0) return 0;
     if (kc > 256) return hb_fail("hb_index_search: too many candidates for the re-rank kernel");
     auto fn = cv ? rerank_kernel<true> : rerank_kernel<false>;
     fn<<<dim3((unsigned)((nq + 3) / 4)), dim3(256), 0, s>>>(tiles, binit, g8, d, q, qn2, cand, cand_score, qnorm, bmax,
                                                           certified, kc, nq, k, id_base, metric, out_metric, ntotal, out_idx, out_dist,
-                                                          hb_rerank_seeds{seed_in, kth_out, floor_out}, cv ? *cv : hb_centre_view{nullptr, nullptr, nullptr});
+                                                          hb_rerank_seeds{seed_in, kth_out, floor_out, n_failed}, cv ? *cv : hb_centre_view{nullptr, nullptr, nullptr});
     HB_HIP(hipGetLastError());
     return 0;
 }
@@ -472,13 +473,13 @@
                           const int64_t* cand, const float* cand_score, const float* qnorm, const float* bmax,
                           unsigned char* certified, int kc, int64_t nq, int k, int64_t id_base, int metric, int out_metric,
                           int64_t ntotal, int64_t* out_idx, float* out_dist, hipStream_t s, const float* seed_in, float* kth_out, float* floor_out,
-                          const hb_centre_view* cv) {
+                          const hb_centre_view* cv, unsigned* n_failed) {
     if (nq == 0) return 0;
     if (kc > 256) return hb_fail("hb_index_search: too many candidates for the re-rank kernel");
     auto fn = cv ? rerank_rows_kernel<true> : rerank_rows_kernel<false>;
     fn<<<dim3((unsigned)((nq + 3) / 4)), dim3(256), 0, s>>>(rows, rs, binit, d, q, qn2, cand, cand_score, qnorm, bmax,
                                                           certified, kc, nq, k, id_base, metric, out_metric, ntotal, out_idx, out_dist,
-                                                          hb_rerank_seeds{seed_in, kth_out, floor_out}, cv ? *cv : hb_centre_view{nullptr, nullptr, nullptr});
+                                                          hb_rerank_seeds{seed_in, kth_out, floor_out, n_failed}, cv ? *cv : hb_centre_view{nullptr, nullptr, nullptr});
     HB_HIP(hipGetLastError());
     return 0;
 }
diff --git a/open-hummingbird-eval_amd/csrc/hbird_layout.hip b/open-hummingbird-eval_amd/csrc/hbird_layout.hip
--- a/open-hummingbird-eval_amd/csrc/hbird_layout.hip
+++ b/open-hummingbird-eval_amd/csrc/hbird_layout.hip
@@ -275,6 +275,68 @@
     return 0;
 }
 
+__global__ __launch_bounds__(256) void search_state_init_kernel(hb_init_ranges r) {
+    const int g = blockIdx.y;
+    unsigned* const p = r.p[g];
+    const size_t n = r.n[g];
+    const unsigned v = r.v[g];
+    const size_t head = std::min<size_t>(n, ((16 - (reinterpret_cast<uintptr_t>(p) & 15)) & 15) / 4);
+    const size_t n4 = (n - head) / 4, tail0 = head + 4 * n4;
+    const size_t t = (size_t)blockIdx.x * 256 + threadIdx.x, stride = (size_t)gridDim.x * 256;
+    uint4* const p4 = reinterpret_cast<uint4*>(p + head);
+    for (size_t i = t; i < n4; i += stride) p4[i] = make_uint4(v, v, v, v);
+    if (t < head) p[t] = v;
+    if (t < n - tail0) p[tail0 + t] = v;
+}
+
+int hb_launch_state_init(const hb_init_ranges& r, hipStream_t s) {
+    if (r.dropped) return hb_fail("hb_launch_state_init: more than HB_INIT_RANGES ranges");
+    if (r.count == 0) return 0;
+    size_t most = 0;
+    for (int g = 0; g < r.count; ++g) most = std::max<size_t>(most, r.n[g]);
+    const unsigned bx = (unsigned)std::min<size_t>(512, std::max<size_t>(1, (most / 4 + 255) / 256));
+    search_state_init_kernel<<<dim3(bx, (unsigned)r.count), dim3(256), 0, s>>>(r);
+    HB_HIP(hipGetLastError());
+    return 0;
+}
+
+__global__ __launch_bounds__(256) void rows_to_f16_tiles_kernel(const float* __restrict__ src, int64_t n_valid, int d, _Float16* __restrict__ t16,
+                                                                int g16, int64_t n_row_tiles, int aligned) {
+    typedef _Float16 f16x8 __attribute__((ext_vector_type(8)));
+    const int64_t gid = (int64_t)blockIdx.x * 256 + threadIdx.x;
+    if (gid >= n_row_tiles * g16 * 64) return;
+    const int i = (int)(gid & 31), h = (int)((gid >> 5) & 1);
+    const int64_t blk = gid >> 6;
+    const int g = (int)(blk % g16);
+    const int64_t r = (blk / g16) * 32 + i;
+    const int k0 = 16 * g + 8 * h;
+    float v[8] = {0.f, 0.f, 0.f, 0.f, 0.f, 0.f, 0.f, 0.f};
+    if (r < n_valid) {
+        const float* row = src + r * (int64_t)d;
+        if (aligned && k0 + 8 <= d) {
+            const float4 a = *reinterpret_cast<const float4*>(row + k0), b = *reinterpret_cast<const float4*>(row + k0 + 4);
+            v[0] = a.x; v[1] = a.y; v[2] = a.z; v[3] = a.w; v[4] = b.x; v[5] = b.y; v[6] = b.z; v[7] = b.w;
+        } else {
+#pragma unroll
+            for (int j = 0; j < 8; ++j) if (k0 + j < d) v[j] = row[k0 + j];
+        }
+    }
+    f16x8 out;
+#pragma unroll
+    for (int j = 0; j < 8; ++j) out[j] = (_Float16)v[j];
+    reinterpret_cast<f16x8*>(t16)[gid] = out;
+}
+
+int hb_launch_rows_to_f16_tiles(const float* src, int64_t n_rows, int d, _Float16* t16, int g16, hipStream_t s) {
+    const int64_t n_row_tiles = (n_rows + HB_QT - 1) / HB_QT * (HB_QT / 32);
+    const int64_t total = n_row_tiles * g16 * 64;
+    if (total == 0) return 0;
+    const int aligned = (d & 3) == 0 && (reinterpret_cast<uintptr_t>(src) & 15) == 0;
+    rows_to_f16_tiles_kernel<<<dim3((unsigned)((total + 255) / 256)), dim3(256), 0, s>>>(src, n_rows, d, t16, g16, n_row_tiles, aligned);
+    HB_HIP(hipGetLastError());
+    return 0;
+}
+
 __global__ __launch_bounds__(256) void tiles_to_rows_kernel(const float* __restrict__ tiles, int g8, int d,
                                                             const int64_t* __restrict__ ids, int64_t n,
                                                             int64_t id_base, int64_t ntotal, float* __restrict__ out) {
diff --git a/open-hummingbird-eval_amd/csrc/hbird_schedule.cpp b/open-hummingbird-eval_amd/csrc/hbird_schedule.cpp
--- a/open-hummingbird-eval_amd/csrc/hbird_schedule.cpp
+++ b/open-hummingbird-eval_amd/csrc/hbird_schedule.cpp
@@ -194,7 +194,7 @@
     hb_finish_schedule(out, per_wg, logical_of_block, slots_of_qt);
 }
 
-void hb_build_schedule(int nqt, int nbt, int G, int panel, hb_schedule& out, int cq, int cb, bool phased, bool xcd_share, const double* xcd_w) {
+void hb_build_schedule(int nqt, int nbt, int G, int panel, hb_schedule& out, int cq, int cb, bool phased, bool xcd_share, const double* xcd_w, int first_clock) {
     out = hb_schedule();
     out.nqt = nqt; out.nbt = nbt; out.panel = panel; out.phased = phased;
     if (xcd_w) {
@@ -207,11 +207,12 @@
     out.G = G;
     if (phased) {
         const long long per_wg_tiles = total_pairs / G;
+        const long long first = std::max(1, first_clock);
         long long t = 0, step = 1;
-        while (out.phase_clock.size() < HB_PHASE_CUTS) {
+        for (int n = 0; n < HB_PHASE_CUTS; ++n) {
             t += step;
             if (t * 2 > per_wg_tiles) break;
-            out.phase_clock.push_back((int)t);
+            if (t >= first) out.phase_clock.push_back((int)t);
             step = std::max<long long>(step + 1, per_wg_tiles <= 64 ? step * 3 : step < 128 ? step * 3 / 2 : step * 2);
         }
     }
@@ -263,7 +264,8 @@
 
 
 static int schedule_plan(int nqt, int nbt, int workgroups, int panel_tiles, int d, int cluster_q, int cluster_b, bool phased,
-                         int* segs_out, int64_t max_segs, int64_t stats[8], hb_schedule& sc, bool xcd_share = false, const double* xcd_w = nullptr) {
+                         int* segs_out, int64_t max_segs, int64_t stats[8], hb_schedule& sc, bool xcd_share = false, const double* xcd_w = nullptr,
+                         int first_clock = 0) {
     if (!stats) return hb_fail("hb_schedule_plan: stats is NULL");
     if (nqt <= 0 || nbt <= 0 || workgroups <= 0 || d <= 0) return hb_fail("hb_schedule_plan: bad arguments");
     const int dp = (d + HB_KC - 1) / HB_KC * HB_KC;
@@ -272,7 +274,7 @@
     if (cq < 0 || cb < 0) hb_default_cluster(nqt, nbt, G, cq == -2, &cq, &cb);
     if (cq < 1 || cb < 1 || (long long)nqt * nbt < workgroups || cq * cb > HB_CLUSTER_MAX || G % (8 * cq * cb) != 0) { cq = 1; cb = 1; }
     const int panel = panel_tiles > 0 ? panel_tiles : hb_default_panel(nqt, G, (size_t)HB_BT * dp * 4, cq, cb);
-    hb_build_schedule(nqt, nbt, workgroups, panel, sc, cq, cb, phased, xcd_share && cq * cb > 1, xcd_w);
+    hb_build_schedule(nqt, nbt, workgroups, panel, sc, cq, cb, phased, xcd_share && cq * cb > 1, xcd_w, first_clock);
     stats[0] = sc.G; stats[1] = (int64_t)sc.segs.size(); stats[2] = sc.n_slots; stats[3] = sc.panel;
     stats[4] = sc.max_slots_per_qt; stats[5] = sc.nqt; stats[6] = sc.nbt; stats[7] = sc.cq * 16 + sc.cb;
     if (segs_out) {
@@ -294,12 +296,13 @@
     return schedule_plan(nqt, nbt, workgroups, panel_tiles, d, cluster_q, cluster_b, false, segs_out, max_segs, stats, sc);
 }
 
-extern "C" int hb_schedule_plan_phased(int nqt, int nbt, int workgroups, int panel_tiles, int d, int cluster_q, int cluster_b,
-                                       int* segs_out, int64_t max_segs, int64_t stats[8], int* clocks_out, int max_cuts, int* n_cuts,
-                                       int* bounds_out) {
+extern "C" int hb_schedule_plan_phased_from(int nqt, int nbt, int workgroups, int panel_tiles, int d, int cluster_q, int cluster_b, int first_clock,
+                                            int* segs_out, int64_t max_segs, int64_t stats[8], int* clocks_out, int max_cuts, int* n_cuts,
+                                            int* bounds_out) {
     if (!n_cuts) return hb_fail("hb_schedule_plan_phased: n_cuts is NULL");
+    if (first_clock < 0) return hb_fail("hb_schedule_plan_phased_from: negative first clock");
     hb_schedule sc;
-    if (schedule_plan(nqt, nbt, workgroups, panel_tiles, d, cluster_q, cluster_b, true, segs_out, max_segs, stats, sc)) return -1;
+    if (schedule_plan(nqt, nbt, workgroups, panel_tiles, d, cluster_q, cluster_b, true, segs_out, max_segs, stats, sc, false, nullptr, first_clock)) return -1;
     *n_cuts = (int)sc.phase_clock.size();
     for (int p = 0; p < *n_cuts && p < max_cuts; ++p) {
         if (clocks_out) clocks_out[p] = sc.phase_clock[p];
@@ -309,6 +312,12 @@
     return 0;
 }
 
+extern "C" int hb_schedule_plan_phased(int nqt, int nbt, int workgroups, int panel_tiles, int d, int cluster_q, int cluster_b,
+                                       int* segs_out, int64_t max_segs, int64_t stats[8], int* clocks_out, int max_cuts, int* n_cuts,
+                                       int* bounds_out) {
+    return hb_schedule_plan_phased_from(nqt, nbt, workgroups, panel_tiles, d, cluster_q, cluster_b, 0, segs_out, max_segs, stats, clocks_out, max_cuts, n_cuts, bounds_out);
+}
+
 extern "C" int hb_schedule_plan_weighted(int nqt, int nbt, int workgroups, int panel_tiles, int d, int cluster_q, int cluster_b, int shared,
                                          const double* xcd_w8, int* segs_out, int64_t max_segs, int64_t stats[8]) {
     hb_schedule sc;
diff --git a/open-hummingbird-eval_amd/csrc/hbird_schedule.h b/open-hummingbird-eval_amd/csrc/hbird_schedule.h
--- a/open-hummingbird-eval_amd/csrc/hbird_schedule.h
+++ b/open-hummingbird-eval_amd/csrc/hbird_schedule.h
@@ -45,7 +45,7 @@
 };
 
 void hb_build_schedule(int nqt, int nbt, int G, int panel_tiles, hb_schedule& out, int cq = 1, int cb = 1, bool phased = false,
-                       bool xcd_share = false, const double* xcd_w = nullptr);
+                       bool xcd_share = false, const double* xcd_w = nullptr, int first_clock = 0);
 int hb_default_panel(int nqt, int G, size_t tile_bytes, int cq = 1, int cb = 1);
 void hb_default_cluster(int nqt, int nbt, int G, bool fp32_kernel, int* cq, int* cb);
 
diff --git a/open-hummingbird-eval_amd/hbird_mi/_lib.py b/open-hummingbird-eval_amd/hbird_mi/_lib.py
--- a/open-hummingbird-eval_amd/hbird_mi/_lib.py
+++ b/open-hummingbird-eval_amd/hbird_mi/_lib.py
@@ -104,6 +104,9 @@
                                        c_uint64, c_uint64, c_uint64, c_uint64, POINTER(c_int)]),
     "hb_knn_plan_replay": (c_int, [POINTER(c_int64), c_int, POINTER(c_int64), c_int]),
     "hb_set_layout_form": (c_int, [c_int]),
+    "hb_query_tiles_f16": (c_int, [c_void_p, c_int64, c_int, c_int, c_void_p, c_int64, c_void_p]),
+    "hb_schedule_plan_phased_from": (c_int, [c_int, c_int, c_int, c_int, c_int, c_int, c_int, c_int, c_void_p, c_int64, POINTER(c_int64),
+                                             c_void_p, c_int, POINTER(c_int), c_void_p]),
     "hb_index_set_rerank_copy": (c_int, [c_void_p, c_int]),
     "hb_index_rerank_copy_bytes": (c_int, [c_void_p, POINTER(c_int64)]),
     "hb_index_schedule_info": (c_int, [c_void_p, POINTER(c_int64)]),
```

After: 77760. No clear change (-0.2%).
